# brudfors/UniRes

Hardware: AMD Instinct MI355X
Metric: cg_iters_per_sec (higher is better)
Workload: dtype f32; 1 GPU; cfg3_256c3_thick6z; channels=3, cg_iters_per_channel=20, cg_mode=fixed-iteration (tol=0), identity preconditioner, step=one y-update of one subject: C x (RHS + 20 CG iterations), channel_streams=True, channel_streams_setting=auto, parallelism=one subject per GPU, no data-path collective

## Files before the change

include/unires_hip.h:

```cpp
#ifndef UNIRES_HIP_H
#define UNIRES_HIP_H

#include <stdint.h>

#ifdef __cplusplus
extern "C" {
#endif

#define UNIRES_HIP_ABI_VERSION 1
#define UNIRES_MAX_TAPS 32

enum unires_status {
  UNIRES_OK = 0,
  UNIRES_ERR_NULL = 1,
  UNIRES_ERR_DIM = 2,
  UNIRES_ERR_ARG = 3,
  UNIRES_ERR_HIP = 4,
  UNIRES_ERR_ALLOC = 5,
  UNIRES_ERR_UNSUPPORTED = 6
};

enum unires_operator { UNIRES_OP_A = 0, UNIRES_OP_AT = 1, UNIRES_OP_ATA = 2 };

enum unires_regime {
  UNIRES_REGIME_IDENTITY = 0,
  UNIRES_REGIME_DENOISE = 1,
  UNIRES_REGIME_SUPERRES = 2
};

enum unires_cg_stop {
  UNIRES_STOP_RESIDUAL = 0,
  UNIRES_STOP_MAXGAIN = 1,
  UNIRES_STOP_MAXGAIN_RECURRED = 2,
  UNIRES_STOP_MAXGAIN_GUARDED = 3
};

enum unires_precond {
  UNIRES_PRECOND_IDENTITY = 0,
  UNIRES_PRECOND_JACOBI = 1,
  UNIRES_PRECOND_FFT = 2
};

const char *unires_last_error(void);
int unires_abi_version(void);


int unires_pull3d_affine(const float *src, const int32_t sdim[3], const float M[12], float *dst,
                         const int32_t gdim[3], float fov_tol, void *stream);

int unires_warp_label(const float *label, const int32_t ldim[3], const float M[12], float *dst,
                      const int32_t gdim[3], float fov_tol, void *stream);

int unires_pull3d_nearest(const float *src, const int32_t sdim[3], const float M[12], float *dst,
                          const int32_t gdim[3], float fov_tol, void *stream);

int unires_noise_hist(int32_t n_obs, const float *const *ptrs, const int64_t *sizes, const int32_t *ct,
                      uint32_t *counts, float *range, void *stream);

int unires_noise_fit(int32_t n_obs, const uint32_t *counts, const float *range, int32_t max_iter,
                     double *out, void *stream);

int unires_coreg_quantise(int32_t n_obs, const float *const *ptrs, const int64_t *sizes,
                          uint8_t *const *outs, uint32_t *counts, float *params, void *stream);

typedef struct {
  const uint8_t *G;
  const uint8_t *F;
  int32_t dim_g[3];
  int32_t dim_f[3];
  float M[12];
  float step[3];
} unires_coreg_job_t;

int unires_coreg_hist(int32_t n_jobs, const unires_coreg_job_t *jobs, uint64_t *hist, void *stream);

int unires_coreg_cost(int32_t n, const uint64_t *hist, int32_t cost_fun, double fwhm, double *work,
                      double *cost, void *stream);

int unires_pull_grad3d_affine(const float *src, const int32_t sdim[3], const float M[12],
                              float *dst3, const int32_t gdim[3], float fov_tol, void *stream);

int unires_push3d_affine(const float *src, const int32_t gdim[3], const float M[12], float *dst,
                         const int32_t ddim[3], float alpha, float fov_tol, int accumulate,
                         void *stream);

int unires_conv_down3d(const float *src, const int32_t sdim[3], const float *const taps[3],
                       const int32_t ntaps[3], const int32_t stride[3], float *dst,
                       const int32_t ddim[3], float scl, int32_t scl_dim, void *stream);

int unires_conv_up3d(const float *src, const int32_t sdim[3], const float *const taps[3],
                     const int32_t ntaps[3], const int32_t stride[3], float *dst,
                     const int32_t ddim[3], float scl, int32_t scl_dim, void *stream);

int unires_grad_fwd_zero(const float *src, const int32_t dim[3], const float vx[3], float *dst3,
                         void *stream);

int unires_div_fwd_zero(const float *src3, const int32_t dim[3], const float vx[3], float *dst,
                        void *stream);

int unires_dtd(const float *src, const int32_t dim[3], const float vx[3], float a, float c,
               float *dst, void *stream);

#define UNIRES_DIFF_FORWARD 0
#define UNIRES_DIFF_BACKWARD 1
#define UNIRES_DIFF_CENTRAL 2

int unires_grad_which(const float *src, const int32_t dim[3], const float vx[3], int32_t which,
                      float *dst3, void *stream);
int unires_div_which(const float *src3, const int32_t dim[3], const float vx[3], int32_t which,
                     float *dst, void *stream);
int unires_dtd_which(const float *src, const int32_t dim[3], const float vx[3], int32_t which, float a,
                     float c, float *dst, void *stream);


typedef struct unires_repeat {
  int32_t dim_x[3];
  int32_t dim_g[3];
  float M[12];
  int32_t ratio[3];
  int32_t ntaps[3];
  const float *taps[3];
  float scl;
  int32_t dim_thick;
  float tau;
} unires_repeat_t;

typedef struct unires_plan unires_plan_t;

int unires_plan_create(unires_plan_t **plan, const int32_t dim_y[3], const float vx_y[3],
                       int32_t regime, int32_t n_repeats, const unires_repeat_t *repeats,
                       float fov_tol);
int unires_plan_destroy(unires_plan_t *plan);
int unires_plan_set_repeat(unires_plan_t *plan, int32_t n, const unires_repeat_t *repeat);
int unires_plan_set_concurrency(unires_plan_t *plan, int32_t n_concurrent);
int unires_plan_set_diff(unires_plan_t *plan, int32_t which);
int unires_plan_set_missing(unires_plan_t *plan, int32_t n, const float *x, void *stream);
int unires_plan_set_slice_weights(unires_plan_t *plan, int32_t n, int32_t axis, const float *u_dev, void *stream);
int64_t unires_plan_workspace_bytes(const unires_plan_t *plan);
int unires_plan_repeat_info(const unires_plan_t *plan, int32_t n, int32_t info[8]);
int unires_orient_of(const float M[12], int32_t perm[3], int32_t flip[3]);
int unires_plan_time_matvecs(unires_plan_t *plan, int32_t on);
int unires_plan_matvec_time(unires_plan_t *plan, int32_t *launches, double *total_us);
int unires_plan_cg_ring(unires_plan_t *plan, int32_t k, int32_t *last);
int unires_plan_cg_ends(unires_plan_t *plan, int32_t *trimmed, int32_t *start_fused);

int unires_proj_apply(unires_plan_t *plan, int32_t n, int32_t op, const float *in, float *out,
                      void *stream);

int unires_ata_matvec(unires_plan_t *plan, float rho, float lam, const float *p, float *q,
                      double *dot_dev, void *stream);

int unires_rhs_assemble(unires_plan_t *plan, const float *const *x_ptrs, const float *w_c,
                        const float *z_c, float rho, float lam, float *b, void *stream);

int unires_atx_assemble(unires_plan_t *plan, const float *const *x_ptrs, float *atx,
                        void *stream);

int unires_rhs_from_atx(unires_plan_t *plan, const float *atx, const float *w_c,
                        const float *z_c, float rho, float lam, float *b, void *stream);

int unires_precond_build(unires_plan_t *plan, int32_t precond_mode, float rho, float lam,
                         float *m_out, void *stream);

int unires_precond_apply(unires_plan_t *plan, const float *in, float *out, void *stream);

int unires_cg_solve(unires_plan_t *plan, float rho, float lam, const float *b, float *x,
                    int32_t max_iter, double tol, int32_t stop_mode, int32_t precond_mode,
                    int32_t *iters_out, double *obj_trace, void *stream);

int unires_cg_solve_many(int32_t n, unires_plan_t *const *plans, const float *rho, const float *lam,
                         const float *const *b, float *const *x, int32_t max_iter, double tol,
                         int32_t stop_mode, int32_t precond_mode, int32_t *iters_out,
                         double *obj_trace, void *const *streams);


int unires_zw_update(const float *const *y_ptrs, const float *lam, int32_t n_channels,
                     const int32_t dim[3], const float vx[3], float rho, float alpha, float *z,
                     float *w, float *jtv, void *stream);

int unires_nll_prior(const float *const *y_ptrs, const float *lam, int32_t n_channels,
                     const int32_t dim[3], const float vx[3], double *out_dev, void *stream);

int unires_zw_update_which(const float *const *y_ptrs, const float *lam, int32_t n_channels,
                           const int32_t dim[3], const float vx[3], int32_t which, float rho, float alpha,
                           float *z, float *w, float *jtv, void *stream);
int unires_nll_prior_which(const float *const *y_ptrs, const float *lam, int32_t n_channels,
                           const int32_t dim[3], const float vx[3], int32_t which, double *out_dev,
                           void *stream);

int unires_masked_sse(const float *x, const float *ay, int64_t n, double *out_dev, void *stream);

int unires_slice_sums(const float *x, const float *ay, const int32_t dim[3], int32_t dim_thick, double *out_dev,
                      void *stream);

int unires_rigid_sums(const float *gr3, const float *diff, const float *ctc, const int32_t dim[3],
                      const float d_rigid[72], double *out_dev, void *stream);

int unires_clean_fov(float *y, const int32_t dim_y[3], const float M[12], const int32_t dim_x[3],
                     void *stream);

int unires_scaling_sums(const float *x, const float *ay, const int32_t dim[3], int32_t dim_thick,
                        double *out_dev, void *stream);

typedef struct unires_mark unires_mark_t;
int unires_mark_create(unires_mark_t **out);
int unires_mark_destroy(unires_mark_t *mark);
int unires_mark_signal(unires_mark_t *mark, uint64_t value, void *stream);
int unires_mark_read(const unires_mark_t *mark, uint64_t *value);

#ifdef __cplusplus
}
#endif
#endif
```

unires_amd/_lib.py:

```python
import ctypes as C
import os

_HERE = os.path.dirname(os.path.abspath(__file__))
LIB_PATH = os.environ.get('UNIRES_LIB') or os.path.join(_HERE, 'libunires_hip.so')

UNIRES_MAX_TAPS = 32
OP = {'A': 0, 'At': 1, 'AtA': 2}
REGIME_IDENTITY, REGIME_DENOISE, REGIME_SUPERRES = 0, 1, 2
STOP = {'e': 0, 'max_gain': 3, 'max_gain_guarded': 3, 'max_gain_fresh': 1, 'max_gain_recurred': 2}
PRECOND = {'none': 0, 'identity': 0, 'jacobi': 1, 'fft': 2}

c_i32x3 = C.c_int32 * 3
c_f32x3 = C.c_float * 3
c_f32x12 = C.c_float * 12
c_fptrx3 = C.POINTER(C.c_float) * 3


class Repeat(C.Structure):
    _fields_ = [('dim_x', c_i32x3), ('dim_g', c_i32x3), ('M', c_f32x12), ('ratio', c_i32x3),
                ('ntaps', c_i32x3), ('taps', c_fptrx3), ('scl', C.c_float),
                ('dim_thick', C.c_int32), ('tau', C.c_float)]


SIGNATURES = {
    'unires_last_error': (C.c_char_p, []),
    'unires_abi_version': (C.c_int, []),
    'unires_pull3d_affine': (C.c_int, [C.c_void_p, c_i32x3, c_f32x12, C.c_void_p, c_i32x3,
                                       C.c_float, C.c_void_p]),
    'unires_warp_label': (C.c_int, [C.c_void_p, c_i32x3, c_f32x12, C.c_void_p, c_i32x3,
                                    C.c_float, C.c_void_p]),
    'unires_pull3d_nearest': (C.c_int, [C.c_void_p, c_i32x3, c_f32x12, C.c_void_p, c_i32x3,
                                        C.c_float, C.c_void_p]),
    'unires_noise_hist': (C.c_int, [C.c_int32, C.POINTER(C.c_void_p), C.POINTER(C.c_int64),
                                    C.POINTER(C.c_int32), C.c_void_p, C.c_void_p, C.c_void_p]),
    'unires_noise_fit': (C.c_int, [C.c_int32, C.c_void_p, C.c_void_p, C.c_int32, C.c_void_p,
                                   C.c_void_p]),
    'unires_coreg_quantise': (C.c_int, [C.c_int32, C.POINTER(C.c_void_p), C.POINTER(C.c_int64),
                                        C.POINTER(C.c_void_p), C.c_void_p, C.c_void_p, C.c_void_p]),
    'unires_coreg_hist': (C.c_int, [C.c_int32, C.c_void_p, C.c_void_p, C.c_void_p]),
    'unires_coreg_cost': (C.c_int, [C.c_int32, C.c_void_p, C.c_int32, C.c_double, C.c_void_p,
                                    C.c_void_p, C.c_void_p]),
    'unires_pull_grad3d_affine': (C.c_int, [C.c_void_p, c_i32x3, c_f32x12, C.c_void_p, c_i32x3,
                                            C.c_float, C.c_void_p]),
    'unires_push3d_affine': (C.c_int, [C.c_void_p, c_i32x3, c_f32x12, C.c_void_p, c_i32x3,
                                       C.c_float, C.c_float, C.c_int, C.c_void_p]),
    'unires_conv_down3d': (C.c_int, [C.c_void_p, c_i32x3, c_fptrx3, c_i32x3, c_i32x3, C.c_void_p,
                                     c_i32x3, C.c_float, C.c_int32, C.c_void_p]),
    'unires_conv_up3d': (C.c_int, [C.c_void_p, c_i32x3, c_fptrx3, c_i32x3, c_i32x3, C.c_void_p,
                                   c_i32x3, C.c_float, C.c_int32, C.c_void_p]),
    'unires_grad_fwd_zero': (C.c_int, [C.c_void_p, c_i32x3, c_f32x3, C.c_void_p, C.c_void_p]),
    'unires_div_fwd_zero': (C.c_int, [C.c_void_p, c_i32x3, c_f32x3, C.c_void_p, C.c_void_p]),
    'unires_dtd': (C.c_int, [C.c_void_p, c_i32x3, c_f32x3, C.c_float, C.c_float, C.c_void_p,
                             C.c_void_p]),
    'unires_grad_which': (C.c_int, [C.c_void_p, c_i32x3, c_f32x3, C.c_int32, C.c_void_p, C.c_void_p]),
    'unires_div_which': (C.c_int, [C.c_void_p, c_i32x3, c_f32x3, C.c_int32, C.c_void_p, C.c_void_p]),
    'unires_dtd_which': (C.c_int, [C.c_void_p, c_i32x3, c_f32x3, C.c_int32, C.c_float, C.c_float, C.c_void_p,
                                   C.c_void_p]),
    'unires_plan_create': (C.c_int, [C.POINTER(C.c_void_p), c_i32x3, c_f32x3, C.c_int32,
                                     C.c_int32, C.POINTER(Repeat), C.c_float]),
    'unires_plan_destroy': (C.c_int, [C.c_void_p]),
    'unires_plan_set_repeat': (C.c_int, [C.c_void_p, C.c_int32, C.POINTER(Repeat)]),
    'unires_plan_set_concurrency': (C.c_int, [C.c_void_p, C.c_int32]),
    'unires_plan_set_diff': (C.c_int, [C.c_void_p, C.c_int32]),
    'unires_plan_set_missing': (C.c_int, [C.c_void_p, C.c_int32, C.c_void_p, C.c_void_p]),
    'unires_plan_set_slice_weights': (C.c_int, [C.c_void_p, C.c_int32, C.c_int32, C.c_void_p, C.c_void_p]),
    'unires_plan_workspace_bytes': (C.c_int64, [C.c_void_p]),
    'unires_orient_of': (C.c_int, [c_f32x12, c_i32x3, c_i32x3]),
    'unires_plan_repeat_info': (C.c_int, [C.c_void_p, C.c_int32, C.c_int32 * 8]),
    'unires_plan_time_matvecs': (C.c_int, [C.c_void_p, C.c_int32]),
    'unires_plan_matvec_time': (C.c_int, [C.c_void_p, C.POINTER(C.c_int32), C.POINTER(C.c_double)]),
    'unires_plan_cg_ring': (C.c_int, [C.c_void_p, C.c_int32, C.POINTER(C.c_int32)]),
    'unires_plan_cg_ends': (C.c_int, [C.c_void_p, C.POINTER(C.c_int32), C.POINTER(C.c_int32)]),
    'unires_proj_apply': (C.c_int, [C.c_void_p, C.c_int32, C.c_int32, C.c_void_p, C.c_void_p,
                                    C.c_void_p]),
    'unires_ata_matvec': (C.c_int, [C.c_void_p, C.c_float, C.c_float, C.c_void_p, C.c_void_p,
                                    C.c_void_p, C.c_void_p]),
    'unires_rhs_assemble': (C.c_int, [C.c_void_p, C.POINTER(C.c_void_p), C.c_void_p, C.c_void_p,
                                      C.c_float, C.c_float, C.c_void_p, C.c_void_p]),
    'unires_atx_assemble': (C.c_int, [C.c_void_p, C.POINTER(C.c_void_p), C.c_void_p, C.c_void_p]),
    'unires_rhs_from_atx': (C.c_int, [C.c_void_p, C.c_void_p, C.c_void_p, C.c_void_p, C.c_float,
                                      C.c_float, C.c_void_p, C.c_void_p]),
    'unires_precond_build': (C.c_int, [C.c_void_p, C.c_int32, C.c_float, C.c_float, C.c_void_p,
                                       C.c_void_p]),
    'unires_precond_apply': (C.c_int, [C.c_void_p, C.c_void_p, C.c_void_p, C.c_void_p]),
    'unires_cg_solve': (C.c_int, [C.c_void_p, C.c_float, C.c_float, C.c_void_p, C.c_void_p,
                                  C.c_int32, C.c_double, C.c_int32, C.c_int32,
                                  C.POINTER(C.c_int32), C.POINTER(C.c_double), C.c_void_p]),
    'unires_cg_solve_many': (C.c_int, [C.c_int32, C.POINTER(C.c_void_p), C.POINTER(C.c_float),
                                       C.POINTER(C.c_float), C.POINTER(C.c_void_p), C.POINTER(C.c_void_p),
                                       C.c_int32, C.c_double, C.c_int32, C.c_int32, C.POINTER(C.c_int32),
                                       C.POINTER(C.c_double), C.POINTER(C.c_void_p)]),
    'unires_zw_update': (C.c_int, [C.POINTER(C.c_void_p), C.POINTER(C.c_float), C.c_int32, c_i32x3,
                                   c_f32x3, C.c_float, C.c_float, C.c_void_p, C.c_void_p,
                                   C.c_void_p, C.c_void_p]),
    'unires_nll_prior': (C.c_int, [C.POINTER(C.c_void_p), C.POINTER(C.c_float), C.c_int32, c_i32x3,
                                   c_f32x3, C.c_void_p, C.c_void_p]),
    'unires_zw_update_which': (C.c_int, [C.POINTER(C.c_void_p), C.POINTER(C.c_float), C.c_int32, c_i32x3,
                                         c_f32x3, C.c_int32, C.c_float, C.c_float, C.c_void_p, C.c_void_p,
                                         C.c_void_p, C.c_void_p]),
    'unires_nll_prior_which': (C.c_int, [C.POINTER(C.c_void_p), C.POINTER(C.c_float), C.c_int32, c_i32x3,
                                         c_f32x3, C.c_int32, C.c_void_p, C.c_void_p]),
    'unires_scaling_sums': (C.c_int, [C.c_void_p, C.c_void_p, c_i32x3, C.c_int32, C.c_void_p,
                                      C.c_void_p]),
    'unires_rigid_sums': (C.c_int, [C.c_void_p, C.c_void_p, C.c_void_p, c_i32x3, C.c_float * 72,
                                    C.c_void_p, C.c_void_p]),
    'unires_clean_fov': (C.c_int, [C.c_void_p, c_i32x3, c_f32x12, c_i32x3, C.c_void_p]),
    'unires_masked_sse': (C.c_int, [C.c_void_p, C.c_void_p, C.c_int64, C.c_void_p, C.c_void_p]),
    'unires_slice_sums': (C.c_int, [C.c_void_p, C.c_void_p, c_i32x3, C.c_int32, C.c_void_p, C.c_void_p]),
    'unires_mark_create': (C.c_int, [C.POINTER(C.c_void_p)]),
    'unires_mark_destroy': (C.c_int, [C.c_void_p]),
    'unires_mark_signal': (C.c_int, [C.c_void_p, C.c_uint64, C.c_void_p]),
    'unires_mark_read': (C.c_int, [C.c_void_p, C.POINTER(C.c_uint64)]),
}

DIFF = {'forward': 0, 'backward': 1, 'central': 2}


def diff_code(which, arg='diff'):
    try:
        return DIFF[which]
    except (KeyError, TypeError):
        raise ValueError("%s must be 'forward', 'backward' or 'central', not %r" % (arg, which)) from None


_lib = None

_EXC = {1: ValueError, 2: ValueError, 3: ValueError, 4: RuntimeError, 5: MemoryError,
        6: NotImplementedError}


def load():
    global _lib
    if _lib is not None:
        return _lib
    if not os.path.exists(LIB_PATH):
        raise RuntimeError(
            'unires_amd: %s is missing. Build it with `python -c "import __graft_entry__ as g; '
            'g.build()"` (hipcc --offload-arch=gfx950). There is no CPU fallback.' % LIB_PATH)
    lib = C.CDLL(LIB_PATH)
    for name, (res, args) in SIGNATURES.items():
        fn = getattr(lib, name)
        fn.restype = res
        fn.argtypes = args
    if lib.unires_abi_version() != 1:
        raise RuntimeError('unires_amd: ABI version mismatch')
    _lib = lib
    return lib


def check(status):
    if status != 0:
        msg = load().unires_last_error().decode()
        raise _EXC.get(status, RuntimeError)(msg)


def i3(v):
    return c_i32x3(*[int(t) for t in v])


def f3(v):
    return c_f32x3(*[float(t) for t in v])


def f12(v):
    return c_f32x12(*[float(t) for t in v])
```

unires_amd/_plan.py:

```python
import ctypes as C

import numpy as np
import torch

from . import _lib
from ._lib import (REGIME_DENOISE, REGIME_IDENTITY, REGIME_SUPERRES, Repeat, check, f3, i3)
from ._ops import FOV_TOL, _ptr, _stream, _vol, on_device
from .spatial import _m12, voxel_size


def proj_matrix(po, method):
    if method == 'super-resolution':
        return torch.linalg.solve(po.mat_y, po.rigid.mm(po.mat_yx)), tuple(po.dim_yx)
    if method == 'denoising':
        return torch.linalg.solve(po.mat_y, po.rigid.mm(po.mat_x)), tuple(po.dim_x)
    raise ValueError('Undefined method')


def regime_of(method, do_proj):
    if method not in ('denoising', 'super-resolution'):
        raise ValueError('Undefined method')
    if not do_proj:
        return REGIME_IDENTITY
    return REGIME_SUPERRES if method == 'super-resolution' else REGIME_DENOISE
# ... 81 lines not shown
        check(self.lib.unires_plan_repeat_info(self._h, int(n), info))
        v = list(info)
        return dict(perm=tuple(v[:3]), flip=tuple((v[3] >> j) & 1 for j in range(3)), pull2=bool(v[4]),
                    splat2_axis=None if v[5] == 0 else v[5] - 2, shift=bool(v[6] & 1), separable=bool(v[7]),
                    fused=bool(v[6] & 2), masked=bool(v[6] & 4), weighted=bool(v[6] & 8))

    @on_device
    def time_matvecs(self, on=True):
        check(self.lib.unires_plan_time_matvecs(self._h, 2 if on == 2 else (1 if on else 0)))

    def cg_ring(self, k=0):
        last = C.c_int32(0)
        check(self.lib.unires_plan_cg_ring(self._h, int(k), C.byref(last)))
        return int(last.value)

    @on_device
    def matvec_time(self):
        n, us = C.c_int32(0), C.c_double(0.0)
        check(self.lib.unires_plan_matvec_time(self._h, C.byref(n), C.byref(us)))
        return int(n.value), float(us.value)

    @on_device
    def set_repeat(self, n, po, tau):
        keep = []
        r = _repeat_desc(po, tau, self.method, self.regime, keep)
        check(self.lib.unires_plan_set_repeat(self._h, n, C.byref(r)))

    @on_device
    def set_missing(self, n, dat):
        import weakref
        self._missing[n] = None
        if dat is None:
            check(self.lib.unires_plan_set_missing(self._h, int(n), None, _stream()))
            return
        d = _vol(dat, 'x')[0]
        if tuple(d.shape) != tuple(self.dims_x[n]):
            raise ValueError('unires_amd: observation shape mismatch')
        check(self.lib.unires_plan_set_missing(self._h, int(n), _ptr(d), _stream()))
        self._missing[n] = (weakref.ref(dat), dat._version)

    def sync_missing(self, x_dats):
        for n in range(self.n_repeats):
            if x_dats is None:
                if self._missing[n] is not None:
                    self.set_missing(n, None)
                continue
            t, key = x_dats[n], self._missing[n]
            if key is not None and key[0]() is t and key[1] == t._version:
                continue
            self.set_missing(n, t)

    @on_device
    def set_slice_weights(self, n, axis, w):
        import weakref
        n, axis = int(n), int(axis)
        if not 0 <= n < self.n_repeats:
            raise ValueError('unires_amd: repeat index out of range')
        if axis not in (0, 1, 2):
            raise ValueError('unires_amd: slice axis must be 0, 1 or 2')
        if w is not None and (not w.is_cuda or w.dtype != torch.float32
                              or tuple(w.shape) != (int(self.dims_x[n][axis]),)):
            raise ValueError('unires_amd: slice weights must be a float32 device tensor of shape (%d,)'
                             % int(self.dims_x[n][axis]))
        self._slice_w[n] = None
        self._atx = None
        if w is None:
            check(self.lib.unires_plan_set_slice_weights(self._h, n, axis, None, _stream()))
            return
        wc = w.contiguous()
        check(self.lib.unires_plan_set_slice_weights(self._h, int(n), axis, _ptr(wc), _stream()))
        self._slice_w[n] = (weakref.ref(w), w._version, axis)

    def sync_slice_weights(self, ws):
        for n in range(self.n_repeats):
            want = None if ws is None else ws[n]
            key = self._slice_w[n]
            if want is None:
                if key is not None:
                    self.set_slice_weights(n, key[2], None)
                continue
            axis, t = want
            if key is not None and key[0]() is t and key[1] == t._version and key[2] == int(axis):
                continue
            self.set_slice_weights(n, axis, t)

    def _slice_key(self):
        return tuple(None if k is None else (id(k[0]()), k[1]) for k in self._slice_w)

    def set_concurrency(self, n):
        n = max(1, int(n))
        if n != self._concurrency:
            check(self.lib.unires_plan_set_concurrency(self._h, n))
            self._concurrency = n

    def set_diff(self, diff):
        code = _lib.diff_code(diff, 'diff')
        if diff != self.diff:
            with torch.cuda.device(self.device):
                check(self.lib.unires_plan_set_diff(self._h, code))
            self.diff = diff

    def _y(self, t, name):
        v, _ = _vol(t, name)
        if tuple(v.shape) != self.dim_y:
            raise ValueError('unires_amd: %s has shape %s, expected %s'
                             % (name, tuple(v.shape), self.dim_y))
        return v

    @on_device
    def proj_apply(self, n, operator, dat):
        if operator not in _lib.OP:
            raise ValueError('Undefined operator')
        d, lead = _vol(dat)
        out_dim = self.dims_x[n] if operator == 'A' else self.dim_y
        in_dim = self.dims_x[n] if operator == 'At' else self.dim_y
        if tuple(d.shape) != tuple(in_dim):
            raise ValueError('unires_amd: input has shape %s, expected %s'
                             % (tuple(d.shape), tuple(in_dim)))
        out = torch.empty(out_dim, dtype=torch.float32, device=d.device)
        check(self.lib.unires_proj_apply(self._h, n, _lib.OP[operator], _ptr(d), _ptr(out),
                                         _stream()))
        return out.reshape(lead + tuple(out_dim))

    @on_device
    def matvec(self, p, rho, lam, out=None, dot=None):
        p = self._y(p, 'p')
        if out is None:
            out = torch.empty_like(p)
        check(self.lib.unires_ata_matvec(self._h, float(rho), float(lam), _ptr(p), _ptr(out),
                                         _ptr(dot) if dot is not None else None, _stream()))
        return out

    @on_device
    def rhs(self, x_dats, w_c, z_c, rho, lam, out=None):
        xs = [_vol(t, 'x')[0] for t in x_dats]
        for t, dx in zip(xs, self.dims_x):
            if tuple(t.shape) != tuple(dx):
                raise ValueError('unires_amd: observation shape mismatch')
        if len(xs) != self.n_repeats:
            raise ValueError('unires_amd: need one observation per repeat')
        for t in (w_c, z_c):
            if tuple(t.shape) != (3,) + self.dim_y or not t.is_cuda or t.dtype != torch.float32:
                raise ValueError('unires_amd: w/z must be (3,X,Y,Z) float32 device tensors')
        w_c, z_c = w_c.contiguous(), z_c.contiguous()
        if out is None:
            out = torch.empty(self.dim_y, dtype=torch.float32, device=w_c.device)
        ptrs = (C.c_void_p * len(xs))(*[t.data_ptr() for t in xs])
        check(self.lib.unires_rhs_assemble(self._h, ptrs, _ptr(w_c), _ptr(z_c), float(rho),
                                           float(lam), _ptr(out), _stream()))
        return out

    @on_device
    def rhs_cached(self, x_dats, w_c, z_c, rho, lam, out):
        xs = [_vol(t, 'x')[0] for t in x_dats]
        import weakref
        copied = any(v is not t and v.data_ptr() != t.data_ptr() for v, t in zip(xs, x_dats))
        key = None if copied else (tuple((id(t), t._version) for t in x_dats), self._slice_key())
        cache = getattr(self, '_atx', None)
        alive = cache is not None and all(r() is t for r, t in zip(cache[2], x_dats)) \
            and len(cache[2]) == len(x_dats)
        if cache is None or key is None or not alive or cache[0] != key:
            atx = cache[1] if cache is not None else torch.empty(self.dim_y, dtype=torch.float32,
                                                                 device=xs[0].device)
            ptrs = (C.c_void_p * len(xs))(*[t.data_ptr() for t in xs])
            check(self.lib.unires_atx_assemble(self._h, ptrs, _ptr(atx), _stream()))
            refs = [] if key is None else [weakref.ref(t) for t in x_dats]
            self._atx = cache = (key, atx, refs)
        w_c, z_c = w_c.contiguous(), z_c.contiguous()
        check(self.lib.unires_rhs_from_atx(self._h, _ptr(cache[1]), _ptr(w_c), _ptr(z_c),
                                           float(rho), float(lam), _ptr(out), _stream()))
        return out

    @on_device
    def precond_build(self, rho, lam, mode='jacobi', out=None):
        if mode not in _lib.PRECOND:
            raise ValueError('Undefined preconditioner')
        if out is not None:
            out = self._y(out, 'out')
        check(self.lib.unires_precond_build(self._h, _lib.PRECOND[mode], float(rho), float(lam),
                                            _ptr(out) if out is not None else None, _stream()))
        return out

    @on_device
    def precond_apply(self, v, out=None):
        v = self._y(v, 'v')
        if out is None:
            out = torch.empty_like(v)
        check(self.lib.unires_precond_apply(self._h, _ptr(v), _ptr(out), _stream()))
        return out

    @on_device
    def cg(self, b, x, rho, lam, max_iter=20, tolerance=1e-3, stop='max_gain', sync=True,
           precond='none'):
        if precond not in _lib.PRECOND:
            raise ValueError('Undefined preconditioner')
        pm = _lib.PRECOND[precond]
        b = self._y(b, 'b')
        if not x.is_contiguous():
            raise ValueError('unires_amd: cg updates x in place and needs it contiguous')
        self._y(x, 'x')
        s = stop if stop in _lib.STOP else stop[0].lower()
        mode = _lib.STOP[s] if s in _lib.STOP else (0 if s == 'e' else 3)
        max_iter = int(max_iter)
        if sync:
            it = C.c_int32(0)
            obj = (C.c_double * (min(max_iter, 4096) + 1))()
            check(self.lib.unires_cg_solve(self._h, float(rho), float(lam), _ptr(b), _ptr(x),
                                           int(max_iter), float(tolerance), mode, pm, C.byref(it),
                                           obj, _stream()))
            trace = _trace(list(obj), it.value) if tolerance else None
            return it.value, trace
        check(self.lib.unires_cg_solve(self._h, float(rho), float(lam), _ptr(b), _ptr(x),
                                       int(max_iter), float(tolerance), mode, pm, None, None,
                                       _stream()))
        return None


def _trace(ring, it):
    n = len(ring)
    if it < n:
        return ring[:it + 1]
    start = (it + 1) % n
    return ring[start:] + ring[:start]


def cg_many(plans, bs, xs, rho, lams, streams, max_iter=20, tolerance=1e-3, stop='max_gain', precond='none',
            sync=False):
    if precond not in _lib.PRECOND:
        raise ValueError('Undefined preconditioner')
    n = len(plans)
    lib = plans[0].lib
    s = stop if stop in _lib.STOP else stop[0].lower()
    mode = _lib.STOP[s] if s in _lib.STOP else (0 if s == 'e' else 3)
    for pl, b, x in zip(plans, bs, xs):
        pl._y(b, 'b')
        if not x.is_contiguous():
            raise ValueError('unires_amd: cg updates x in place and needs it contiguous')
        pl._y(x, 'x')
    max_iter = int(max_iter)
    nobj = min(max_iter, 4096) + 1
    it = (C.c_int32 * n)() if sync else None
    obj = (C.c_double * (n * nobj))() if sync else None
    with torch.cuda.device(plans[0].device):
        check(lib.unires_cg_solve_many(
            n, (C.c_void_p * n)(*[pl._h.value for pl in plans]), (C.c_float * n)(*[float(rho)] * n),
            (C.c_float * n)(*[float(v) for v in lams]), (C.c_void_p * n)(*[b.data_ptr() for b in bs]),
            (C.c_void_p * n)(*[x.data_ptr() for x in xs]), max_iter, float(tolerance), mode,
            _lib.PRECOND[precond], it, obj, (C.c_void_p * n)(*[st.cuda_stream for st in streams])))
    if not sync:
        return None
    return [(it[c], _trace(list(obj[c * nobj:(c + 1) * nobj]), it[c]) if tolerance else None) for c in range(n)]
```

unires_amd/_update.py:

```python
import ctypes as C

import torch

from . import _lib
from ._lib import check, f3, i3
from ._ops import _ptr, _stream, on_device
from ._host import Pacer
from ._plan import cg_many
from ._project import _channel_plan, _proj, _slice_axis
from .spatial import voxel_size


_PACERS = {}


def _admm_aux(y, sett):
    dim = (len(y), 3) + tuple(y[0].dim)
    z = torch.zeros(dim, dtype=torch.float32, device=sett.device)
    w = torch.zeros(dim, dtype=torch.float32, device=sett.device)
    return z, w


def _step_size(x, y, sett, verbose=False):
    rho = sett.rho
    if any(xn.ct for xc in x for xn in xc):
        rho = 1.0
    if rho is not None:
        return torch.tensor(rho, dtype=torch.float32)
    all_lam = torch.tensor([float(yc.lam) for yc in y], dtype=torch.float32)
    all_tau = torch.tensor([float(xn.tau) for xc in x for xn in xc], dtype=torch.float32)
    return sett.rho_scl * torch.sqrt(torch.mean(all_tau)) / torch.mean(all_lam)


def _diff(sett):
    diff = getattr(sett, 'diff', 'forward')
    _lib.diff_code(diff, 'sett.diff')
    return diff


def _mask_zeros(sett):
    return bool(getattr(sett, 'mask_zeros', False))


def _slice_robust(sett):
    return bool(getattr(sett, 'slice_robust', False))


class _Precond:

    def __init__(self, plan, M, mode):
        self.plan, self.M, self.mode = plan, M, mode

    def __call__(self, v):
        return v if self.M is None else v / self.M


@on_device
def _precond(x, y, rho, sett):
    if len(x) != 1:
        raise ValueError('CG pre-conditioning only supports one repeat per contrast.')
    plan = _channel_plan(x, y, sett.method, sett.do_proj, voxel_size(y.mat).float(), diff=_diff(sett),
                         mask_zeros=_mask_zeros(sett), weights=True)
    M = torch.empty(tuple(y.dim), dtype=torch.float32, device=y.dat.device)
    plan.precond_build(float(rho), float(y.lam), mode='jacobi', out=M)
    return _Precond(plan, M, 'jacobi')


@on_device
def _update_y(x, y, z, w, rho, tmp, sett, info=None):
    vx_y = voxel_size(y[0].mat).float()
    rho = float(rho)
    sync = info is not None
    C = len(x)
    concurrent = C > 1 and not sync and channel_streams_on(sett, y[0].dat)
    pre = getattr(sett, 'cgs_precond', 'none')
    if not concurrent:
        for c in range(C):
            plan = _channel_plan(x[c], y[c], sett.method, sett.do_proj, vx_y, diff=_diff(sett),
                                 mask_zeros=_mask_zeros(sett), weights=True)
            plan.set_concurrency(1)
            lam = float(y[c].lam)
            if getattr(sett, 'cache_atx', True) and not sync:
                plan.rhs_cached([xn.dat for xn in x[c]], w[c], z[c], rho, lam, out=tmp)
            else:
                plan.rhs([xn.dat for xn in x[c]], w[c], z[c], rho, lam, out=tmp)
            if pre in ('jacobi', 'fft'):
                plan.precond_build(rho, lam, mode=pre)
            res = plan.cg(tmp, y[c].dat, rho, lam, max_iter=sett.cgs_max_iter,
                          tolerance=sett.cgs_tol, stop=sett.cgs_stop, sync=sync, precond=pre)
            if sync:
                info.append(res)
        return y
    main = torch.cuda.current_stream()
    fetched = [_channel_plan(x[c], y[c], sett.method, sett.do_proj, vx_y, diff=_diff(sett),
                             mask_zeros=_mask_zeros(sett), weights=True) for c in range(C)]
    ready = torch.cuda.Event()
    ready.record(main)
    streams = _side_streams(y[0].dat.device, C)
    plans, bs = [], []
    for c in range(C):
        plan = fetched[c]
        plan.set_concurrency(C)
        lam = float(y[c].lam)
        b = tmp if c == 0 else plan.rhs_buffer(tmp)
        with torch.cuda.stream(streams[c]):
            streams[c].wait_event(ready)
            if getattr(sett, 'cache_atx', True):
                plan.rhs_cached([xn.dat for xn in x[c]], w[c], z[c], rho, lam, out=b)
            else:
                plan.rhs([xn.dat for xn in x[c]], w[c], z[c], rho, lam, out=b)
            if pre in ('jacobi', 'fft'):
                plan.precond_build(rho, lam, mode=pre)
        plans.append(plan)
        bs.append(b)
    cg_many(plans, bs, [yc.dat for yc in y], rho, [float(yc.lam) for yc in y], streams,
            max_iter=sett.cgs_max_iter, tolerance=sett.cgs_tol, stop=sett.cgs_stop, precond=pre)
    for c in range(C):
        main.wait_stream(streams[c])
    return y


CHANNEL_STREAMS_MAX_VOXELS = None


def channel_streams_on(sett, dat):
    cs = getattr(sett, 'channel_streams', 'auto')
    if cs == 'auto':
        return CHANNEL_STREAMS_MAX_VOXELS is None or dat.numel() < CHANNEL_STREAMS_MAX_VOXELS
    return bool(cs)


_STREAMS = {}


def _side_streams(device, n):
    key = (device.type, device.index)
    pool = _STREAMS.setdefault(key, [])
    while len(pool) < n:
        pool.append(torch.cuda.Stream(device=device))
    return pool[:n]


def _chan_args(y):
    for yc in y:
        if not yc.dat.is_cuda or yc.dat.dtype != torch.float32 or not yc.dat.is_contiguous():
            raise RuntimeError('unires_amd: y[c].dat must be contiguous float32 CUDA/HIP tensors')
    ptrs = (C.c_void_p * len(y))(*[yc.dat.data_ptr() for yc in y])
    lams = (C.c_float * len(y))(*[float(yc.lam) for yc in y])
    return ptrs, lams


@on_device
def _update_zw(y, z, w, rho, tmp, sett):
    for t in (z, w):
        if not t.is_cuda or t.dtype != torch.float32 or not t.is_contiguous() \
                or tuple(t.shape) != (len(y), 3) + tuple(y[0].dim):
            raise ValueError('unires_amd: z/w must be contiguous (C,3,X,Y,Z) float32 device tensors')
    if not tmp.is_contiguous() or tuple(tmp.shape) != tuple(y[0].dim):
        raise ValueError('unires_amd: tmp must be a contiguous (X,Y,Z) tensor')
    vx = [float(v) for v in voxel_size(y[0].mat).tolist()]
    ptrs, lams = _chan_args(y)
    diff = _lib.diff_code(_diff(sett), 'sett.diff')
    check(_lib.load().unires_zw_update_which(ptrs, lams, len(y), i3(y[0].dim), f3(vx), diff, float(rho),
                                             float(sett.alpha), _ptr(z), _ptr(w), _ptr(tmp), _stream()))
    return z, w, tmp


@on_device
def _slice_sums(x, y, sett):
    lib = _lib.load()
    out = {}
    for c in range(len(x)):
        for n, xn in enumerate(x[c]):
            if getattr(xn, 'slice_w', None) is None:
                continue
            Ay = _proj('A', y[c].dat, x[c], y[c], n=n, method=sett.method, do=sett.do_proj)
            xd = xn.dat.contiguous()
            a = _slice_axis(xn)
            sums = torch.empty(2 * int(xd.shape[a]), dtype=torch.float64, device=xd.device)
            check(lib.unires_slice_sums(_ptr(xd), _ptr(Ay), i3(xd.shape), a, _ptr(sums), _stream()))
            out[(c, n)] = sums
    return out


def slice_rule(sums, k):
    S = sums.numel() // 2
    sse, cnt = sums[:S], sums[S:]
    has = cnt > 0
    m = sse / cnt.clamp(min=1.0)
    K = has.sum()
    inf = torch.full_like(m, float('inf'))
    ranked = torch.where(has, m, inf).sort().values
    sig2 = ranked.gather(0, ((K + 1) // 2 - 1).clamp(min=0).reshape(1))[0]
    thr = (float(k) * float(k)) * sig2
    one = torch.ones_like(m)
    u = torch.where(has & (m > thr), thr / m, one)
    return torch.where((K > 0) & (sig2 > 0), u, one)


@on_device
def _update_slice_weights(x, y, sett, sums=None):
    sums = _slice_sums(x, y, sett) if sums is None else sums
    k = float(getattr(sett, 'slice_k', 3.0))
    for (c, n), s in sums.items():
        x[c][n].slice_w.copy_(slice_rule(s, k))
    return x


@on_device
def _compute_nll(x, y, sett, rho, sum_dtype=torch.float64, slice_sums=None):
    dev = y[0].dat.device
    if slice_sums is None:
        slice_sums = _slice_sums(x, y, sett)
    lib = _lib.load()
    vx = [float(v) for v in voxel_size(y[0].mat).tolist()]
    nll_xy = torch.zeros((), dtype=torch.float64, device=dev)
    sse = torch.zeros((), dtype=torch.float64, device=dev)
    for c in range(len(x)):
        for n in range(len(x[c])):
            if (c, n) in slice_sums:
                w, s = x[c][n].slice_w, slice_sums[(c, n)]
                nll_xy = nll_xy + 0.5 * float(x[c][n].tau) * (w.double() * s[:w.numel()]).sum()
                continue
            Ay = _proj('A', y[c].dat, x[c], y[c], n=n, method=sett.method, do=sett.do_proj)
            xd = x[c][n].dat.contiguous()
            check(lib.unires_masked_sse(_ptr(xd), _ptr(Ay), xd.numel(), _ptr(sse), _stream()))
            nll_xy = nll_xy + 0.5 * float(x[c][n].tau) * sse
    ptrs, lams = _chan_args(y)
    nll_y = torch.zeros((), dtype=torch.float64, device=dev)
    diff = _lib.diff_code(_diff(sett), 'sett.diff')
    check(lib.unires_nll_prior_which(ptrs, lams, len(y), i3(y[0].dim), f3(vx), diff, _ptr(nll_y), _stream()))
    return nll_xy + nll_y, nll_xy, nll_y


@on_device
def _update_scaling(x, y, sett, max_niter_gn=1, num_linesearch=4, verbose=0):
    from ._project import _apply_scaling
    if sett.method != 'super-resolution':
        raise ValueError('_update_scaling needs the super-resolution projection '
                         '(slice profile + slice scaling)')
    lib = _lib.load()
    dev = y[0].dat.device
    sll = torch.zeros((), dtype=torch.float64, device=dev)
    sums = torch.empty(5, dtype=torch.float64, device=dev)
    for c in range(len(x)):
        for n_x in range(len(x[c])):
            xn = x[c][n_x]
            if xn.ct:
                continue
            po = xn.po
            dim_thick, tau, scl = int(po.dim_thick), float(xn.tau), float(po.scl)
            plan = _channel_plan(x[c], y[c], sett.method, sett.do_proj)
            dat_x = xn.dat.contiguous()
            dat_y = plan.proj_apply(n_x, 'A', y[c].dat)

            def evaluate(ay):
                check(lib.unires_scaling_sums(_ptr(dat_x), _ptr(ay), i3(dat_x.shape), dim_thick,
                                              _ptr(sums), _stream()))
                return sums.tolist()

            ll = 0.0
            for _ in range(max_niter_gn):
                s = evaluate(dat_y)
                ll = 0.5 * tau * s[0]
                gr = tau * (s[1] - s[2])
                hes = tau * (s[3] + s[4])
                update = float(torch.tensor(gr, dtype=torch.float64) / torch.tensor(hes, dtype=torch.float64))
                old_scl, old_ll, armijo = scl, ll, 1.0
                if num_linesearch == 0:
# ... 36 lines not shown
```

unires_amd/csrc/api.hip:

```cpp
#include <float.h>
#include <math.h>
#include <string.h>

#include <map>
#include <mutex>
#include <new>

#include "admm.hpp"
#include "api_internal.hpp"
#include "conv.hpp"
#include "coreg.hpp"
#include "noise.hpp"
#include "pull.hpp"
#include "stencil.hpp"

using namespace unires;

thread_local std::string unires::g_err;

int unires::make_taps(const float *const taps[3], const int32_t ntaps[3], const int32_t stride[3], Taps &T) {
  memset(&T, 0, sizeof(T));
  for (int d = 0; d < 3; ++d) {
    if (ntaps[d] < 1 || ntaps[d] > UNIRES_MAX_TAPS)
      return fail(UNIRES_ERR_UNSUPPORTED, "ntaps must be in [1, UNIRES_MAX_TAPS]");
// ... 162 lines not shown
    int32_t ng[3];
    if (coreg_grid(J[o], ng) > (int64_t)INT32_MAX) return fail(UNIRES_ERR_DIM, "more than 2^31 - 1 sample points");
  }
  hipStream_t st = (hipStream_t)stream;
  HIP_TRY(hipMemsetAsync(hist, 0, (size_t)n_jobs * kCoregBins * kCoregBins * sizeof(uint64_t), st));
  for (int32_t o = 0; o < n_jobs; o += kCoregMaxJobs) {
    const int n = std::min<int32_t>(kCoregMaxJobs, n_jobs - o);
    launch_coreg_hist(n, J + o, hist + (size_t)o * kCoregBins * kCoregBins, st);
    CHECK_LAUNCH();
  }
  return UNIRES_OK;
}

extern "C" int unires_coreg_cost(int32_t n, const uint64_t *hist, int32_t cost_fun, double fwhm, double *work,
                                 double *cost, void *stream) {
  if (!hist || !work || !cost) return fail(UNIRES_ERR_NULL, "null argument");
  if (n < 1) return fail(UNIRES_ERR_ARG, "n must be >= 1");
  if (cost_fun < 0 || cost_fun > 2) return fail(UNIRES_ERR_ARG, "cost_fun must be 0 (nmi), 1 (mi) or 2 (ecc)");
  if (!(fwhm >= 0.0 && fwhm <= 16.0)) return fail(UNIRES_ERR_ARG, "fwhm must be in [0, 16]");
  const int R = (int)lround(2.0 * fwhm);
  double taps[2 * kCoregMaxTapRadius + 1];
  const double s = pow(fwhm / sqrt(8.0 * log(2.0)), 2) + DBL_EPSILON, w1 = 1.0 / sqrt(2.0 * s);
  double sum = 0.0;
  for (int k = -R; k <= R; ++k) {
    const double v = 0.5 * (erf(w1 * (k + 0.5)) - erf(w1 * (k - 0.5)));
    taps[k + R] = v > 0.0 ? v : 0.0;
    sum += taps[k + R];
  }
  for (int k = 0; k <= 2 * R; ++k) taps[k] /= sum;
  launch_coreg_cost(n, hist, cost_fun, taps, R, work, cost, (hipStream_t)stream);
  CHECK_LAUNCH();
  return UNIRES_OK;
}

extern "C" int unires_pull_grad3d_affine(const float *src, const int32_t sdim[3], const float M[12],
                                         float *dst3, const int32_t gdim[3], float fov_tol,
                                         void *stream) {
  if (!src || !dst3 || !sdim || !gdim || !M) return fail(UNIRES_ERR_NULL, "null argument");
  if (!dims_ok(sdim) || !dims_ok(gdim)) return fail(UNIRES_ERR_DIM, "bad dimensions");
  Affine A;
  memcpy(A.m, M, sizeof(A.m));
  launch_pull_grad(src, mk(sdim), A, dst3, mk(gdim), fov_tol, (hipStream_t)stream);
  CHECK_LAUNCH();
  return UNIRES_OK;
}

extern "C" int unires_push3d_affine(const float *src, const int32_t gdim[3], const float M[12],
                                    float *dst, const int32_t ddim[3], float alpha, float fov_tol,
                                    int accumulate, void *stream) {
  if (!src || !dst || !ddim || !gdim || !M) return fail(UNIRES_ERR_NULL, "null argument");
  if (!dims_ok(ddim) || !dims_ok(gdim)) return fail(UNIRES_ERR_DIM, "bad dimensions");
  Affine A;
  memcpy(A.m, M, sizeof(A.m));
  Affine Ainv;
  if (!invert_affine(A, Ainv)) return fail(UNIRES_ERR_ARG, "singular affine");
  PushSrc ps;
  memset(&ps, 0, sizeof(ps));
  ps.data = src;
  ps.gd = mk(gdim);
  ps.S = kNoScaling;
  PushEpilogue ep;
  ep.accumulate = accumulate ? 1 : 0;
  SplatSafety safe;
  splat_safety(A, safe.row_sep, safe.use_atomics);
  if (push_mode() == PushMode::kTile ||
      launch_splat(ps, A, Ainv, safe, alpha, fov_tol, ep, dst, mk(ddim), nullptr, (hipStream_t)stream))
    (void)launch_push_tile(ps, A, Ainv, safe, alpha, fov_tol, ep, dst, mk(ddim), nullptr,
                           (hipStream_t)stream);
  CHECK_LAUNCH();
  return UNIRES_OK;
}

extern "C" int unires_conv_down3d(const float *src, const int32_t sdim[3],
                                  const float *const taps[3], const int32_t ntaps[3],
                                  const int32_t stride[3], float *dst, const int32_t ddim[3],
                                  float scl, int32_t scl_dim, void *stream) {
  if (!src || !dst || !sdim || !ddim || !taps || !ntaps || !stride)
    return fail(UNIRES_ERR_NULL, "null argument");
  if (!dims_ok(sdim) || !dims_ok(ddim)) return fail(UNIRES_ERR_DIM, "bad dimensions");
  if (scl != 0.f && (scl_dim < 0 || scl_dim > 2)) return fail(UNIRES_ERR_ARG, "bad scl_dim");
  Taps T;
  int rc = make_taps(taps, ntaps, stride, T);
  if (rc) return rc;
  if ((rc = check_conv_dims(mk(sdim), mk(ddim), T))) return rc;
  launch_conv_down(src, mk(sdim), T, make_scaling(scl, scl_dim), dst, mk(ddim), nullptr,
                   (hipStream_t)stream);
  CHECK_LAUNCH();
  return UNIRES_OK;
}

extern "C" int unires_conv_up3d(const float *src, const int32_t sdim[3],
                                const float *const taps[3], const int32_t ntaps[3],
                                const int32_t stride[3], float *dst, const int32_t ddim[3],
                                float scl, int32_t scl_dim, void *stream) {
  if (!src || !dst || !sdim || !ddim || !taps || !ntaps || !stride)
    return fail(UNIRES_ERR_NULL, "null argument");
  if (!dims_ok(sdim) || !dims_ok(ddim)) return fail(UNIRES_ERR_DIM, "bad dimensions");
  if (scl != 0.f && (scl_dim < 0 || scl_dim > 2)) return fail(UNIRES_ERR_ARG, "bad scl_dim");
  Taps T;
  int rc = make_taps(taps, ntaps, stride, T);
  if (rc) return rc;
  if ((rc = check_conv_dims(mk(ddim), mk(sdim), T))) return rc;
  launch_conv_up(src, mk(sdim), T, make_scaling(scl, scl_dim), dst, mk(ddim), (hipStream_t)stream);
  CHECK_LAUNCH();
  return UNIRES_OK;
}

extern "C" int unires_grad_which(const float *src, const int32_t dim[3], const float vx[3], int32_t which,
                                 float *dst3, void *stream) {
  if (!src || !dst3 || !dim) return fail(UNIRES_ERR_NULL, "null argument");
  if (!dims_ok(dim)) return fail(UNIRES_ERR_DIM, "bad dimensions");
  if (!vx_ok(vx)) return fail(UNIRES_ERR_ARG, "voxel size must be positive");
  if (!diff_ok(which)) return fail(UNIRES_ERR_ARG, "which: forward (0), backward (1) or central (2)");
  launch_grad(src, mk(dim), vx, dst3, (hipStream_t)stream, which);
  CHECK_LAUNCH();
  return UNIRES_OK;
}
extern "C" int unires_grad_fwd_zero(const float *src, const int32_t dim[3], const float vx[3],
                                    float *dst3, void *stream) {
  return unires_grad_which(src, dim, vx, UNIRES_DIFF_FORWARD, dst3, stream);
}

extern "C" int unires_div_which(const float *src3, const int32_t dim[3], const float vx[3], int32_t which,
                                float *dst, void *stream) {
  if (!src3 || !dst || !dim) return fail(UNIRES_ERR_NULL, "null argument");
  if (!dims_ok(dim)) return fail(UNIRES_ERR_DIM, "bad dimensions");
  if (!vx_ok(vx)) return fail(UNIRES_ERR_ARG, "voxel size must be positive");
  if (!diff_ok(which)) return fail(UNIRES_ERR_ARG, "which: forward (0), backward (1) or central (2)");
  launch_div(src3, nullptr, 1.f, 0.f, mk(dim), vx, 1.f, nullptr, dst, (hipStream_t)stream, which);
  CHECK_LAUNCH();
  return UNIRES_OK;
}
extern "C" int unires_div_fwd_zero(const float *src3, const int32_t dim[3], const float vx[3],
                                   float *dst, void *stream) {
  return unires_div_which(src3, dim, vx, UNIRES_DIFF_FORWARD, dst, stream);
}

extern "C" int unires_dtd_which(const float *src, const int32_t dim[3], const float vx[3], int32_t which,
                                float a, float c, float *dst, void *stream) {
  if (!src || !dst || !dim) return fail(UNIRES_ERR_NULL, "null argument");
  if (!dims_ok(dim)) return fail(UNIRES_ERR_DIM, "bad dimensions");
  if (!vx_ok(vx)) return fail(UNIRES_ERR_ARG, "voxel size must be positive");
  if (!diff_ok(which)) return fail(UNIRES_ERR_ARG, "which: forward (0), backward (1) or central (2)");
  if (src == dst) return fail(UNIRES_ERR_ARG, "dtd cannot run in place");
  launch_dtd(src, mk(dim), vx, a, c, dst, nullptr, nullptr, nullptr, (hipStream_t)stream, which);
  CHECK_LAUNCH();
  return UNIRES_OK;
}
extern "C" int unires_dtd(const float *src, const int32_t dim[3], const float vx[3], float a,
                          float c, float *dst, void *stream) {
  return unires_dtd_which(src, dim, vx, UNIRES_DIFF_FORWARD, a, c, dst, stream);
}

static int check_channels(const float *const *y_ptrs, const float *lam, int32_t n) {
  if (!y_ptrs || !lam) return fail(UNIRES_ERR_NULL, "null argument");
  if (n < 1 || n > 4096) return fail(UNIRES_ERR_ARG, "channel count out of range");
  for (int c = 0; c < n; ++c)
    if (!y_ptrs[c]) return fail(UNIRES_ERR_NULL, "null channel pointer");
  return UNIRES_OK;
}

extern "C" int unires_zw_update_which(const float *const *y_ptrs, const float *lam, int32_t n_channels,
                                      const int32_t dim[3], const float vx[3], int32_t which, float rho,
                                      float alpha, float *z, float *w, float *jtv, void *stream) {
  int rc = check_channels(y_ptrs, lam, n_channels);
  if (rc) return rc;
  if (!diff_ok(which)) return fail(UNIRES_ERR_ARG, "which: forward (0), backward (1) or central (2)");
  if (!z || !w || !jtv || !dim) return fail(UNIRES_ERR_NULL, "null argument");
  if (!dims_ok(dim)) return fail(UNIRES_ERR_DIM, "bad dimensions");
  if (!vx_ok(vx)) return fail(UNIRES_ERR_ARG, "voxel size must be positive");
  if (!(rho > 0.f)) return fail(UNIRES_ERR_ARG, "rho must be positive");
  hipStream_t st = (hipStream_t)stream;
  const Dim3i d = mk(dim);
  launch_jtv_scale(y_ptrs, lam, n_channels, w, z, d, vx, rho, alpha, jtv, nullptr, nullptr, 0, st, which);
  const size_t n = d.numel();
  for (int c = 0; c < n_channels; ++c)
    launch_zw_update(y_ptrs[c], lam[c], jtv, z + (size_t)c * 3 * n, w + (size_t)c * 3 * n, d, vx,
                     rho, alpha, st, which);
  CHECK_LAUNCH();
  return UNIRES_OK;
}

extern "C" int unires_zw_update(const float *const *y_ptrs, const float *lam, int32_t n_channels,
                                const int32_t dim[3], const float vx[3], float rho, float alpha,
                                float *z, float *w, float *jtv, void *stream) {
  return unires_zw_update_which(y_ptrs, lam, n_channels, dim, vx, UNIRES_DIFF_FORWARD, rho, alpha, z, w, jtv, stream);
}

extern "C" int unires_nll_prior_which(const float *const *y_ptrs, const float *lam, int32_t n_channels,
                                      const int32_t dim[3], const float vx[3], int32_t which, double *out_dev,
                                      void *stream) {
  int rc = check_channels(y_ptrs, lam, n_channels);
  if (rc) return rc;
  if (!diff_ok(which)) return fail(UNIRES_ERR_ARG, "which: forward (0), backward (1) or central (2)");
  if (!out_dev || !dim) return fail(UNIRES_ERR_NULL, "null argument");
  if (!dims_ok(dim)) return fail(UNIRES_ERR_DIM, "bad dimensions");
  if (!vx_ok(vx)) return fail(UNIRES_ERR_ARG, "voxel size must be positive");
  hipStream_t st = (hipStream_t)stream;
  HIP_TRY(hipMemsetAsync(out_dev, 0, sizeof(double), st));
  float *acc = nullptr;
  if (n_channels > 8) {
    static std::mutex mu;
    static std::map<int, std::pair<float *, size_t>> scratch;
    int dev = 0;
    HIP_TRY(hipGetDevice(&dev));
    const size_t need = mk(dim).numel() * sizeof(float);
    std::lock_guard<std::mutex> lock(mu);
    auto &slot = scratch[dev];
    if (slot.second < need) {
      if (slot.first) {
        HIP_TRY(hipDeviceSynchronize());
        (void)hipFree(slot.first);
        slot = {nullptr, 0};
      }
      HIP_TRY(hipMalloc((void **)&slot.first, need));
      slot.second = need;
    }
    acc = slot.first;
  }
  double *part = nullptr;
  if ((rc = reduce_scratch(st, (size_t)jtv_scale_blocks(mk(dim)), &part))) return rc;
  launch_jtv_scale(y_ptrs, lam, n_channels, nullptr, nullptr, mk(dim), vx, 1.f, 1.f, acc, part, out_dev, 1, st, which);
  CHECK_LAUNCH();
  return UNIRES_OK;
}

extern "C" int unires_nll_prior(const float *const *y_ptrs, const float *lam, int32_t n_channels,
                                const int32_t dim[3], const float vx[3], double *out_dev,
                                void *stream) {
  return unires_nll_prior_which(y_ptrs, lam, n_channels, dim, vx, UNIRES_DIFF_FORWARD, out_dev, stream);
}

extern "C" int unires_scaling_sums(const float *x, const float *ay, const int32_t dim[3],
                                   int32_t dim_thick, double *out_dev, void *stream) {
  if (!x || !ay || !dim || !out_dev) return fail(UNIRES_ERR_NULL, "null argument");
  if (!dims_ok(dim)) return fail(UNIRES_ERR_DIM, "bad dims");
  if (dim_thick < 0 || dim_thick > 2) return fail(UNIRES_ERR_ARG, "bad dim_thick");
  hipStream_t st = (hipStream_t)stream;
  double *part = nullptr;
  if (int rc = reduce_scratch(st, 5 * (size_t)scaling_sums_blocks(mk(dim)), &part)) return rc;
  launch_scaling_sums(x, ay, mk(dim), dim_thick, part, out_dev, st);
  CHECK_LAUNCH();
  return UNIRES_OK;
}

extern "C" int unires_rigid_sums(const float *gr3, const float *diff, const float *ctc,
                                 const int32_t dim[3], const float d_rigid[72], double *out_dev,
                                 void *stream) {
  if (!gr3 || !diff || !dim || !d_rigid || !out_dev) return fail(UNIRES_ERR_NULL, "null argument");
  if (!dims_ok(dim)) return fail(UNIRES_ERR_DIM, "bad dims");
  hipStream_t st = (hipStream_t)stream;
  float D[6][12];
  memcpy(D, d_rigid, sizeof(D));
  double *part = nullptr;
  if (int rc = reduce_scratch(st, 27 * (size_t)rigid_sums_blocks(mk(dim)), &part)) return rc;
  launch_rigid_sums(gr3, diff, ctc, mk(dim), D, part, out_dev, st);
  CHECK_LAUNCH();
  return UNIRES_OK;
}

extern "C" int unires_clean_fov(float *y, const int32_t dim_y[3], const float M[12],
                                const int32_t dim_x[3], void *stream) {
  if (!y || !dim_y || !M || !dim_x) return fail(UNIRES_ERR_NULL, "null argument");
  if (!dims_ok(dim_y) || !dims_ok(dim_x)) return fail(UNIRES_ERR_DIM, "bad dims");
  Affine A;
  memcpy(A.m, M, sizeof(A.m));
  launch_clean_fov(y, mk(dim_y), A, mk(dim_x), (hipStream_t)stream);
  CHECK_LAUNCH();
  return UNIRES_OK;
}

extern "C" int unires_masked_sse(const float *x, const float *ay, int64_t n, double *out_dev,
                                 void *stream) {
  if (!x || !ay || !out_dev) return fail(UNIRES_ERR_NULL, "null argument");
  if (n < 1) return fail(UNIRES_ERR_DIM, "bad length");
  hipStream_t st = (hipStream_t)stream;
  double *part = nullptr;
  if (int rc = reduce_scratch(st, (size_t)masked_sse_blocks((size_t)n), &part)) return rc;
  launch_masked_sse(x, ay, (size_t)n, part, out_dev, st);
  CHECK_LAUNCH();
  return UNIRES_OK;
}

extern "C" int unires_slice_sums(const float *x, const float *ay, const int32_t dim[3], int32_t dim_thick,
                                 double *out_dev, void *stream) {
  if (!x || !ay || !dim || !out_dev) return fail(UNIRES_ERR_NULL, "null argument");
  if (!dims_ok(dim)) return fail(UNIRES_ERR_DIM, "bad dims");
  if (dim_thick < 0 || dim_thick > 2) return fail(UNIRES_ERR_ARG, "bad dim_thick");
  hipStream_t st = (hipStream_t)stream;
  double *part = nullptr;
  const size_t cols = 2 * (size_t)dim[dim_thick];
  if (int rc = reduce_scratch(st, cols * (size_t)slice_sums_parts(mk(dim), dim_thick), &part)) return rc;
  launch_slice_sums(x, ay, mk(dim), dim_thick, part, out_dev, st);
  CHECK_LAUNCH();
  return UNIRES_OK;
}

struct unires_mark {
  unsigned long long *host = nullptr;
  unsigned long long *dev = nullptr;
};

__global__ void k_mark(unsigned long long *w, unsigned long long v) {
  __hip_atomic_store(w, v, __ATOMIC_RELAXED, __HIP_MEMORY_SCOPE_SYSTEM);
}

// ... 41 lines not shown
```

unires_amd/csrc/api_cg.hip:

```cpp
#include <time.h>

#include <functional>

#include "api_internal.hpp"

using namespace unires;

static bool cg_start_fused_on() {
  static const bool on = !(getenv("UNIRES_CG_START_FUSED") && getenv("UNIRES_CG_START_FUSED")[0] == '0');
  return on;
}

static int cg_enqueue_start(unires_plan *pl, const CgSolve &s, unsigned long long *hostw, hipStream_t st) {
  const size_t ny = pl->dy.numel();
  const bool check = s.tol != 0.0;
  CgState *S = pl->state;
  const int gv = vec_num_blocks(ny);
  HIP_TRY(hipMemsetAsync(&S->done, 0, sizeof(int), st));
  const bool want_obj0 = check && s.stop != UNIRES_STOP_RESIDUAL;
  StartResidual res = {s.b, pl->r, pl->p, s.M, pl->part0, want_obj0 ? pl->part1 : nullptr, false};
  const bool ask = cg_start_fused_on() && !s.fft;
  int g0 = matvec(pl, s.rho, s.lam, s.x, pl->ap, nullptr, nullptr, st, nullptr, ask ? &res : nullptr);
  pl->last_fused = ask && res.served;
  if (!(ask && res.served)) {
    launch_residual_init(s.b, pl->ap, s.x, pl->r, pl->p, ny, pl->part0, want_obj0 ? pl->part1 : nullptr, s.M, st);
    g0 = gv;
  }
  if (s.fft) {
    if (fftpre_apply(pl->fft, pl->r, pl->fft.z, st)) return fail(UNIRES_ERR_HIP, "hipFFT execution failed");
    HIP_TRY(hipMemcpyAsync(pl->p, pl->fft.z, ny * sizeof(float), hipMemcpyDeviceToDevice, st));
    launch_dot(pl->r, pl->fft.z, ny, pl->part0, nullptr, st);
  }
  launch_sc_init(S, pl->part0, pl->part1, g0, s.stop, check ? 1 : 0, hostw, st);
  return UNIRES_OK;
}

static float *ring_slot(unires_plan *pl, int j) {
  return j == 0 ? pl->p : pl->ring + (size_t)(j - 1) * (align_up(pl->dy.numel() * 4) / 4);
}

static bool cg_trim_on() {
  static const bool on = !(getenv("UNIRES_CG_TRIM") && getenv("UNIRES_CG_TRIM")[0] == '0');
  return on;
}

static int cg_enqueue_iters(unires_plan *pl, const CgSolve &s, int k_first, int count, bool dev_k,
                            unsigned long long *hostw, hipStream_t st) {
  const size_t ny = pl->dy.numel();
  const bool check = s.tol != 0.0;
  const int ring = s.ring;
  CgState *S = pl->state;
  const int *done = &S->done;
  const int gv = vec_num_blocks(ny);
  if (ring > 1 && (check || s.fft || dev_k || ring > kMaxRing || ring - 1 > pl->ring_slots))
    return fail(UNIRES_ERR_ARG, "deferred iterate update outside its scope");
  const bool trim = cg_trim_on() && !check && !s.fft && !dev_k && k_first == 1 && count == s.max_iter;
  pl->last_trim = trim && count > 0;
  RingPtrs rp = {};
  for (int j = 0; j < ring && ring > 1; ++j) rp.p[j] = ring_slot(pl, j);
  for (int k = k_first; k < k_first + count; ++k) {
    const int kk = dev_k ? -1 : k;
    const int slot = ring > 1 ? (k - k_first) % ring : 0;
    float *p = ring > 1 ? ring_slot(pl, slot) : pl->p;
    hipEvent_t ev0 = nullptr, ev1 = nullptr;
    if (pl->timing && hipEventCreate(&ev0) == hipSuccess) {
      if (hipEventCreate(&ev1) == hipSuccess) {
        (void)hipEventRecord(ev0, st);
      } else {
        (void)hipEventDestroy(ev0);
        ev0 = nullptr;
      }
    }
    if (pl->twice) (void)matvec(pl, s.rho, s.lam, p, pl->ap, pl->part0, done, st);
    const int g = matvec(pl, s.rho, s.lam, p, pl->ap, pl->part0, done, st);
    if (ev0 && ev1) {
      (void)hipEventRecord(ev1, st);
      if (pl->tev.size() >= 65536) {
        (void)hipEventDestroy(pl->tev.front().first), (void)hipEventDestroy(pl->tev.front().second);
        pl->tev.erase(pl->tev.begin());
      }
      pl->tev.emplace_back(ev0, ev1);
    }
    const bool guarded = check && s.stop == UNIRES_STOP_MAXGAIN_GUARDED;
    const bool recur = check && (s.stop == UNIRES_STOP_MAXGAIN_RECURRED || guarded);
    int obj_kind = 0;
    if (check && s.stop == UNIRES_STOP_RESIDUAL) obj_kind = 1;
    if (recur) obj_kind = 2;
    const bool lazy_x = obj_kind == 0;
    if (trim && k == k_first + count - 1) {
      launch_sc_alpha(S, pl->part0, g, st, k);
      if (ring > 1)
        launch_update_x_flush(S, rp, slot + 1, ny, s.x, st);
      else
        launch_update_x(S, p, ny, s.x, st);
      break;
    }
    launch_sc_alpha(S, pl->part0, g, st);
    launch_update_xr(S, p, pl->ap, lazy_x ? nullptr : s.x, pl->r, s.b, ny, pl->part0,
                     recur ? pl->part1 : nullptr, s.M, st);
    if (s.fft) {
      if (fftpre_apply(pl->fft, pl->r, pl->fft.z, st)) return fail(UNIRES_ERR_HIP, "hipFFT execution failed");
      launch_dot(pl->r, pl->fft.z, ny, pl->part0, done, st);
    }
    if (guarded)
      launch_sc_beta_guarded(S, pl->part0, pl->part1, gv, kk, s.tol, hostw, st);
    else
      launch_sc_beta(S, pl->part0, pl->part1, gv, kk, obj_kind, s.tol, obj_kind ? hostw : nullptr, st);
    if (ring > 1 && (slot == ring - 1 || k == k_first + count - 1))
      launch_update_p_flush(S, pl->r, rp, slot + 1, ring_slot(pl, (slot + 1) % ring), ny, s.M, s.x, st);
    else if (ring > 1)
      launch_update_p_ring(S, pl->r, p, ring_slot(pl, slot + 1), slot, ny, s.M, st);
    else
      launch_update_p(S, s.fft ? pl->fft.z : pl->r, pl->p, ny, s.M, lazy_x ? s.x : nullptr, st);
    if (check && s.stop == UNIRES_STOP_MAXGAIN) {
      const int go = matvec(pl, s.rho, s.lam, s.x, pl->ax, pl->part1, done, st, s.b);
      launch_sc_obj(S, pl->part1, go, kk, s.tol, hostw, st);
    }
    if (guarded) {
      const int go = matvec(pl, s.rho, s.lam, s.x, pl->ax, pl->part1, &S->skip_fresh, st, s.b);
      launch_sc_obj_guarded(S, pl->part1, go, kk, s.tol, hostw, st);
    }
  }
  return UNIRES_OK;
}

static int cg_enqueue(unires_plan *pl, const CgSolve &s, hipStream_t st) {
  const int rc = cg_enqueue_start(pl, s, nullptr, st);
  if (rc) return rc;
  return cg_enqueue_iters(pl, s, 1, s.max_iter, false, nullptr, st);
}

static int cg_ring_prepare(unires_plan *pl, hipStream_t st) {
  static const int env_k = [] {
    const char *e = getenv("UNIRES_CG_RING");
    return e ? atoi(e) : 8;
  }();
  int want = pl->ring_req > 0 ? pl->ring_req : env_k;
  want = std::max(1, std::min(want, kMaxRing));
  if (want <= 1) return 1;
  if (!pl->ring_tried) {
    if (stream_capturing(st)) return 1;
    pl->ring_tried = true;
    const size_t slot = align_up(pl->dy.numel() * 4);
    size_t budget = 0;
    if (const char *e = getenv("UNIRES_CG_RING_MB")) {
      budget = (size_t)std::max(0.0, atof(e) * 1048576.0);
    } else {
      size_t free_b = 0, total_b = 0;
      if (hipMemGetInfo(&free_b, &total_b) == hipSuccess) budget = free_b / 8;
      (void)hipGetLastError();
    }
    const int n = (int)std::min<size_t>((size_t)(want - 1), budget / slot);
    if (n < 1) return 1;
    if (hipMalloc((void **)&pl->ring, (size_t)n * slot) != hipSuccess) {
      (void)hipGetLastError();
      pl->ring = nullptr;
      return 1;
    }
    pl->ring_slots = n;
  }
  return std::min(want, pl->ring_slots + 1);
}

struct CgRun {
  unires_plan *pl = nullptr;
  CgSolve s;
  hipStream_t st = nullptr;
  int enqueued = 0;
  unsigned gen = 0;
  bool finished = false;
  bool use_graph = false;
};

static void cg_resync_gen(unires_plan *pl) {
  (void)hipDeviceSynchronize();
  (void)hipGetLastError();
  unsigned g = pl->cg_gen;
  if (pl->state && hipMemcpy(&g, &pl->state->gen, sizeof(g), hipMemcpyDeviceToHost) == hipSuccess) pl->cg_gen = g;
  (void)hipGetLastError();
}

static int cg_chunk_env() {
  static const int v = [] {
    const char *e = getenv("UNIRES_CG_CHUNK");
    return e ? atoi(e) : 2;
  }();
  return v;
}
static int cg_chunk_size() { return std::max(1, std::min(cg_chunk_env(), 64)); }

static int capture_graph(hipStream_t st, hipGraphExec_t *exec, const std::function<int()> &body) {
  *exec = nullptr;
  if (hipStreamBeginCapture(st, hipStreamCaptureModeThreadLocal) != hipSuccess) {
    (void)hipGetLastError();
    return -1;
  }
  const int rc = body();
  hipGraph_t graph = nullptr;
  const hipError_t ce = hipStreamEndCapture(st, &graph);
  if (rc) {
    if (graph) (void)hipGraphDestroy(graph);
    return rc;
  }
  if (ce != hipSuccess || !graph) return fail(UNIRES_ERR_HIP, "hipStreamEndCapture failed");
  const hipError_t ge = hipGraphInstantiate(exec, graph, nullptr, nullptr, 0);
  (void)hipGraphDestroy(graph);
  if (ge != hipSuccess) {
    *exec = nullptr;
    return fail(UNIRES_ERR_HIP, "hipGraphInstantiate failed");
  }
  return UNIRES_OK;
}

static int cg_run_enqueue_chunk(CgRun &R) {
  unires_plan *pl = R.pl;
  const int n = std::min(R.s.chunk, R.s.max_iter - R.enqueued);
  if (n <= 0) return UNIRES_OK;
  if (R.use_graph && n == R.s.chunk && pl->cg_chunk_exec) {
    HIP_TRY(hipGraphLaunch(pl->cg_chunk_exec, R.st));
  } else {
    const int rc = cg_enqueue_iters(pl, R.s, R.enqueued + 1, n, true, pl->progress_dev, R.st);
    if (rc) return rc;
  }
  R.enqueued += n;
  return UNIRES_OK;
}

static int cg_run_start_impl(CgRun &R) {
  unires_plan *pl = R.pl;
  if (!pl->progress) {
    HIP_TRY(hipHostMalloc((void **)&pl->progress, 64, hipHostMallocMapped));
    *pl->progress = 0ull;
    HIP_TRY(hipHostGetDevicePointer((void **)&pl->progress_dev, (void *)pl->progress, 0));
  }
  R.gen = ++pl->cg_gen;
  R.enqueued = 0;
  R.finished = false;
  CgSolve key = R.s;
  key.max_iter = 0;
  key.pre = R.s.M ? UNIRES_PRECOND_JACOBI : UNIRES_PRECOND_IDENTITY;
  if (R.use_graph && !(pl->cg_start_exec && pl->cg_chunk_exec && pl->cg_chunk_key.same_graph(key))) {
    drop_cg_chunk_graphs(pl);
    int rc = capture_graph(R.st, &pl->cg_start_exec, [&] { return cg_enqueue_start(pl, R.s, pl->progress_dev, R.st); });
    if (rc > 0) return rc;
    if (rc == 0)
      rc = capture_graph(R.st, &pl->cg_chunk_exec, [&] {
        return cg_enqueue_iters(pl, R.s, 1, R.s.chunk, true, pl->progress_dev, R.st);
      });
    if (rc > 0) return rc;
    if (rc < 0 || !pl->cg_start_exec || !pl->cg_chunk_exec) {
      drop_cg_chunk_graphs(pl);
      R.use_graph = false;
    } else {
      pl->cg_chunk_key = key;
      pl->chunk_fused = pl->last_fused;
    }
  }
  pl->last_trim = 0;
  if (R.use_graph) {
    pl->last_fused = pl->chunk_fused;
    HIP_TRY(hipGraphLaunch(pl->cg_start_exec, R.st));
  } else {
    const int rc = cg_enqueue_start(pl, R.s, pl->progress_dev, R.st);
    if (rc) return rc;
  }
  int rc = cg_run_enqueue_chunk(R);
  if (!rc) rc = cg_run_enqueue_chunk(R);
  if (rc) return rc;
  if (R.enqueued >= R.s.max_iter) R.finished = true;
  pl->last_trim = 0;
  return UNIRES_OK;
}

static int cg_run_start(CgRun &R) {
  const int rc = cg_run_start_impl(R);
  if (rc) cg_resync_gen(R.pl);
  return rc;
}

static int cg_run_poll(CgRun &R) {
  if (R.finished) return UNIRES_OK;
  const unsigned long long w = __atomic_load_n(R.pl->progress, __ATOMIC_ACQUIRE);
  if ((unsigned)(w >> 32) != R.gen) return UNIRES_OK;
  if (w & 0x80000000ull) {
    R.finished = true;
    return UNIRES_OK;
  }
  const int iters = (int)(w & 0x7fffffffull);
  while (!R.finished && iters >= R.enqueued - R.s.chunk) {
    const int rc = cg_run_enqueue_chunk(R);
    if (rc) return rc;
    if (R.enqueued >= R.s.max_iter) R.finished = true;
  }
  return UNIRES_OK;
}

static int cg_runs_drive(std::vector<CgRun> &runs) {
  unsigned spins = 0;
  for (;;) {
    bool all = true;
    for (CgRun &R : runs) {
      if (R.finished) continue;
      const int rc = cg_run_poll(R);
      if (rc) return rc;
      all = all && R.finished;
    }
    if (all) return UNIRES_OK;
    if (++spins > 256) {
      const struct timespec nap = {0, 50000};
      (void)nanosleep(&nap, nullptr);
    }
    if ((spins <= 256 && (spins & 0xff) == 0) || (spins > 256 && (spins & 0x1ff) == 0)) {
      for (CgRun &R : runs) {
        if (R.finished) continue;
        const hipError_t q = hipStreamQuery(R.st);
        if (q == hipSuccess) {
          const int before = R.enqueued;
          const int rc = cg_run_poll(R);
          if (rc) return rc;
          if (!R.finished && R.enqueued == before)
            return fail(UNIRES_ERR_HIP, "chunked CG: the stream drained without the expected progress");
        } else if (q != hipErrorNotReady) {
          g_err = std::string("chunked CG: ") + hipGetErrorString(q);
          return UNIRES_ERR_HIP;
        }
      }
    }
  }
}

static int cg_check_args(unires_plan *plan, float rho, float lam, const float *b, float *x, int32_t max_iter,
                         double tol, int32_t stop_mode, int32_t precond_mode) {
  if (!plan || !b || !x) return fail(UNIRES_ERR_NULL, "null argument");
  if (b == x) return fail(UNIRES_ERR_ARG, "b and x must not alias");
  if (max_iter < 0) return fail(UNIRES_ERR_ARG, "max_iter out of range");
  if (max_iter > kMaxCgIter && !(tol > 0.0))
    return fail(UNIRES_ERR_ARG, "max_iter beyond 4096 needs a tolerance (the solve is then enqueued in chunks)");
  if (stop_mode < 0 || stop_mode > 3) return fail(UNIRES_ERR_ARG, "bad stop mode");
  if (precond_mode < UNIRES_PRECOND_IDENTITY || precond_mode > UNIRES_PRECOND_FFT)
    return fail(UNIRES_ERR_UNSUPPORTED, "preconditioner modes: identity (0), Jacobi (1), FFT (2)");
  if (precond_mode != UNIRES_PRECOND_IDENTITY &&
      (!plan->prec_ready || plan->prec_mode != precond_mode || plan->prec_rho != rho ||
       plan->prec_lam != lam))
    return fail(UNIRES_ERR_ARG, "call unires_precond_build with this mode, rho and lam first");
  if (!(tol >= 0.0)) return fail(UNIRES_ERR_ARG, "tolerance must be >= 0");
  return UNIRES_OK;
}

static bool cg_graphs_on() {
  static const bool on = !(getenv("UNIRES_CG_GRAPH") && getenv("UNIRES_CG_GRAPH")[0] == '0');
  return on;
}

static bool cg_chunked(double tol, int max_iter) {
  const bool off = cg_chunk_env() == 0;
  return tol != 0.0 && max_iter > 0 && (!off || max_iter > kMaxCgIter);
}

static CgSolve cg_describe(const unires_plan *pl, float rho, float lam, const float *b, float *x, int max_iter,
                           double tol, int stop_mode, int precond_mode) {
  CgSolve s;
  s.b = b, s.x = x, s.rho = rho, s.lam = lam, s.max_iter = max_iter, s.stop = stop_mode, s.pre = precond_mode;
  s.tol = tol;
  s.M = precond_mode == UNIRES_PRECOND_JACOBI ? pl->precM : nullptr;
  s.fft = precond_mode == UNIRES_PRECOND_FFT;
  return s;
}

static CgRun cg_make_run(unires_plan *pl, CgSolve s, hipStream_t st) {
  CgRun R;
  R.pl = pl, R.s = s, R.st = st;
  R.s.chunk = cg_chunk_size();
  R.use_graph = cg_graphs_on() && !s.fft && !pl->timing;
  return R;
}

static int cg_read_back(unires_plan *pl, int max_iter, double tol, int32_t *iters_out, double *obj_trace,
                        hipStream_t st) {
  CgState *S = pl->state;
  int it = 0;
  HIP_TRY(hipMemcpyAsync(&it, &S->iters, sizeof(int), hipMemcpyDeviceToHost, st));
  if (obj_trace && tol != 0.0)
    HIP_TRY(hipMemcpyAsync(obj_trace, S->obj, sizeof(double) * (size_t)(std::min(max_iter, kMaxCgIter) + 1),
                           hipMemcpyDeviceToHost, st));
  HIP_TRY(hipStreamSynchronize(st));
  *iters_out = it;
  return UNIRES_OK;
}

extern "C" int unires_cg_solve(unires_plan_t *plan, float rho, float lam, const float *b, float *x,
                               int32_t max_iter, double tol, int32_t stop_mode,
                               int32_t precond_mode, int32_t *iters_out, double *obj_trace,
                               void *stream) {
  int rc = cg_check_args(plan, rho, lam, b, x, max_iter, tol, stop_mode, precond_mode);
  if (rc) return rc;
  hipStream_t st = (hipStream_t)stream;
  unires_plan *pl = plan;
  CgSolve s = cg_describe(pl, rho, lam, b, x, max_iter, tol, stop_mode, precond_mode);
  mark_use(pl, st);

  if (stream_capturing(st) && tol != 0.0 && max_iter > kMaxCgIter)
    return fail(UNIRES_ERR_ARG, "a solve with a tolerance and more than 4096 iterations cannot join a stream capture "
                                "(it is fed to the device chunk by chunk, following its progress)");
  if (cg_chunked(tol, max_iter) && !(stream_capturing(st) && max_iter <= kMaxCgIter)) {
    pl->last_ring = 1;
    std::vector<CgRun> runs(1, cg_make_run(pl, s, st));
    if ((rc = cg_run_start(runs[0]))) return rc;
    if ((rc = cg_runs_drive(runs))) return rc;
    mark_use(pl, st);
    CHECK_LAUNCH();
    return iters_out ? cg_read_back(pl, max_iter, tol, iters_out, obj_trace, st) : UNIRES_OK;
  }
  ++pl->cg_gen;
  s.ring = tol == 0.0 && !s.fft && max_iter > 0 ? cg_ring_prepare(pl, st) : 1;
  pl->last_ring = s.ring;

  const bool graphable = cg_graphs_on() && !s.fft && max_iter > 0 && !pl->timing;
  if (graphable && pl->cg_exec && pl->cg_key.same_graph(s)) {
    pl->last_trim = pl->graph_trim, pl->last_fused = pl->graph_fused;
    HIP_TRY(hipGraphLaunch(pl->cg_exec, st));
  } else {
    if (graphable && pl->cg_exec) drop_cg_graph(pl);
    rc = graphable ? capture_graph(st, &pl->cg_exec, [&] { return cg_enqueue(pl, s, st); }) : -1;
    if (rc > 0) {
      cg_resync_gen(pl);
      return rc;
    }
    if (rc == 0) {
      pl->cg_key = s;
      pl->graph_trim = pl->last_trim, pl->graph_fused = pl->last_fused;
      if (hipGraphLaunch(pl->cg_exec, st) != hipSuccess) {
        cg_resync_gen(pl);
        return fail(UNIRES_ERR_HIP, "hipGraphLaunch failed");
      }
    } else if ((rc = cg_enqueue(pl, s, st))) {
      cg_resync_gen(pl);
      return rc;
    }
  }
  mark_use(pl, st);
  CHECK_LAUNCH();
  return iters_out ? cg_read_back(pl, max_iter, tol, iters_out, obj_trace, st) : UNIRES_OK;
}

extern "C" int unires_cg_solve_many(int32_t n, unires_plan_t *const *plans, const float *rho, const float *lam,
                                    const float *const *b, float *const *x, int32_t max_iter, double tol,
                                    int32_t stop_mode, int32_t precond_mode, int32_t *iters_out,
                                    double *obj_trace, void *const *streams) {
  if (n < 1 || !plans || !rho || !lam || !b || !x || !streams) return fail(UNIRES_ERR_NULL, "null argument");
  for (int c = 0; c < n; ++c) {
    const int rc = cg_check_args(plans[c], rho[c], lam[c], b[c], x[c], max_iter, tol, stop_mode, precond_mode);
    if (rc) return rc;
    for (int d = 0; d < c; ++d)
      if (plans[d] == plans[c]) return fail(UNIRES_ERR_ARG, "one plan per solve");
  }
  bool capturing = false;
  for (int c = 0; c < n; ++c) capturing = capturing || stream_capturing((hipStream_t)streams[c]);
  if (capturing && tol != 0.0 && max_iter > kMaxCgIter)
    return fail(UNIRES_ERR_ARG, "a solve with a tolerance and more than 4096 iterations cannot join a stream capture "
                                "(it is fed to the device chunk by chunk, following its progress)");
  for (int c = 0; c < n; ++c) mark_use(plans[c], (hipStream_t)streams[c]);
  if (!cg_chunked(tol, max_iter) || (capturing && max_iter <= kMaxCgIter)) {
    for (int c = 0; c < n; ++c) {
      const int rc = unires_cg_solve(plans[c], rho[c], lam[c], b[c], x[c], max_iter, tol, stop_mode, precond_mode,
                                     nullptr, nullptr, streams[c]);
      if (rc) return rc;
    }
  } else {
    std::vector<CgRun> runs;
    for (int c = 0; c < n; ++c) plans[c]->last_ring = 1;
    for (int c = 0; c < n; ++c)
      runs.push_back(cg_make_run(plans[c], cg_describe(plans[c], rho[c], lam[c], b[c], x[c], max_iter, tol, stop_mode,
                                                       precond_mode), (hipStream_t)streams[c]));
    for (CgRun &R : runs) {
      const int rc = cg_run_start(R);
      if (rc) return rc;
    }
    const int rc = cg_runs_drive(runs);
    if (rc) return rc;
    for (int c = 0; c < n; ++c) mark_use(plans[c], (hipStream_t)streams[c]);
    CHECK_LAUNCH();
  }
  if (iters_out)
    for (int c = 0; c < n; ++c) {
      const int rc = cg_read_back(plans[c], max_iter, tol, iters_out + c,
                                  obj_trace ? obj_trace + (size_t)c * (std::min(max_iter, kMaxCgIter) + 1) : nullptr,
                                  (hipStream_t)streams[c]);
      if (rc) return rc;
    }
  return UNIRES_OK;
}
```

unires_amd/csrc/api_internal.hpp:

```cpp
#pragma once
#include <math.h>
#include <stdlib.h>
#include <string.h>

#include <algorithm>
#include <string>
#include <utility>
#include <vector>

#include "../../include/unires_hip.h"
#include "ata1.hpp"
#include "cg.hpp"
#include "fftpre.hpp"
#include "fused.hpp"
#include "mask.hpp"
#include "orient.hpp"
#include "pull2.hpp"
#include "shift.hpp"
#include "slice.hpp"
#include "splat2.hpp"

namespace unires {

extern thread_local std::string g_err;

inline int fail(int code, const char *msg) {
  g_err = msg;
  return code;
}

#define HIP_TRY(expr)                                                               \
  do {                                                                              \
    hipError_t e_ = (expr);                                                         \
    if (e_ != hipSuccess) {                                                         \
      unires::g_err = std::string(#expr) + ": " + hipGetErrorString(e_);            \
      return UNIRES_ERR_HIP;                                                        \
    }                                                                               \
  } while (0)

#define CHECK_LAUNCH()                                                              \
  do {                                                                              \
    hipError_t e_ = hipGetLastError();                                              \
    if (e_ != hipSuccess) {                                                         \
      unires::g_err = std::string("kernel launch: ") + hipGetErrorString(e_);       \
      return UNIRES_ERR_HIP;                                                        \
    }                                                                               \
  } while (0)

inline bool dims_ok(const int32_t d[3]) {
  return d[0] > 0 && d[1] > 0 && d[2] > 0 && d[0] <= 65535 &&
         (long long)d[0] * d[1] * d[2] < (1ll << 40);
}
inline bool vx_ok(const float vx[3]) { return vx && vx[0] > 0 && vx[1] > 0 && vx[2] > 0; }
inline Dim3i mk(const int32_t d[3]) { return Dim3i{d[0], d[1], d[2]}; }
inline size_t align_up(size_t v) { return (v + 255) & ~(size_t)255; }

int make_taps(const float *const taps[3], const int32_t ntaps[3], const int32_t stride[3], Taps &T);
int check_conv_dims(const Dim3i &hi, const Dim3i &lo, const Taps &T);
bool invert_affine(const Affine &A, Affine &out);

inline Scaling make_scaling(float scl, int dim) {
  if (scl == 0.f) return kNoScaling;
  return Scaling{expf(scl), expf(-scl), dim};
}

enum class PushMode { kDefault, kTile, kNoSchedule };
inline PushMode push_mode() {
  static const PushMode mode = [] {
    const char *e = getenv("UNIRES_PUSH");
    return !e ? PushMode::kDefault : !strcmp(e, "tile") ? PushMode::kTile : PushMode::kNoSchedule;
  }();
  return mode;
}

struct RepeatDesc {
  Orient orient;
  bool oriented = false;
  Dim3i dim_xu;
  Dim3i dim_x, dim_g;
  Affine A;
  Taps T;
  float scl;
  int dim_thick;
  float tau;
  Dim3i dim_gf;
  Affine Af, Afinv;
  Taps Tf;
  SplatSafety safe;
  bool sep = false;
  bool sep0 = false;
  bool hyb = false;
  bool hybf = false;
  Taps Tz, Txy;
  Dim3i dim_h;
};

struct RepeatTables {
  SplatSched sched;
  float *ctab_dev[2] = {nullptr, nullptr};
  int ctab_n = 0, ctab_cap = 0;
  unsigned ctab_step = 1, src_stride = 1;
  float *xytab_dev[2] = {nullptr, nullptr};
  int xytab_cap[2] = {0, 0};
  PullPlan pplan;
  ShiftPlan shift;
  F1Sched f1;
};

struct RepeatMask {
  bool masked = false;
  uint8_t *mask_u = nullptr, *mask_c = nullptr;
  size_t mask_cap = 0;
};

struct RepeatWeights {
  bool weighted = false;
  float *w_dev = nullptr;
  int w_axis = 0;
  size_t w_cap = 0;
};

struct Repeat : RepeatDesc, RepeatTables, RepeatMask, RepeatWeights {
  const uint8_t *mask() const { return oriented ? mask_c : mask_u; }
  bool mid() const { return masked || weighted; }
  int w_caxis() const {
    for (int j = 0; j < 3; ++j)
      if (orient.perm[j] == w_axis) return j;
    return w_axis;
  }
  bool w_flip() const { return orient.flip[w_caxis()] != 0; }
};

struct CgSolve {
  const float *b = nullptr;
  float *x = nullptr;
  float rho = 0.f, lam = 0.f;
  int max_iter = -1, stop = -1, pre = -1;
  double tol = -1.0;
  int ring = 1;
  int chunk = 0;
  const float *M = nullptr;
  bool fft = false;
  bool same_graph(const CgSolve &o) const {
    return b == o.b && x == o.x && rho == o.rho && lam == o.lam && max_iter == o.max_iter && stop == o.stop &&
           pre == o.pre && ring == o.ring && chunk == o.chunk && tol == o.tol;
  }
};

}

struct unires_plan {
  unires::Dim3i dy;
  float vx[3];
  int regime;
  float fov_tol;
  int diff = UNIRES_DIFF_FORWARD;
  std::vector<unires::Repeat> reps;
  char *ws = nullptr;
  size_t ws_bytes = 0;
  float *r = nullptr, *p = nullptr, *ap = nullptr, *ax = nullptr;
  bool timing = false;
  bool twice = false;
  std::vector<std::pair<hipEvent_t, hipEvent_t>> tev;
  float *gbuf = nullptr;
  float *gbuf2 = nullptr;
  float *xbuf = nullptr;
  float *xperm = nullptr;
  double *part0 = nullptr, *part1 = nullptr;
  unires::CgState *state = nullptr;
  size_t cap_g = 0, cap_x = 0;
  unires::CgSolve cg_key;
  hipGraphExec_t cg_exec = nullptr;
  unires::CgSolve cg_chunk_key;
  hipGraphExec_t cg_start_exec = nullptr, cg_chunk_exec = nullptr;
  unsigned long long *progress = nullptr, *progress_dev = nullptr;
  unsigned cg_gen = 0;
  float *precM = nullptr;
  float *ring = nullptr;
  int ring_slots = 0;
  bool ring_tried = false;
  int ring_req = 0;
  int last_ring = 1;
  int last_trim = 0, last_fused = 0, graph_trim = 0, graph_fused = 0, chunk_fused = 0;
  unires::FftPre fft;
  float prec_rho = 0.f, prec_lam = 0.f;
  int prec_mode = UNIRES_PRECOND_IDENTITY;
  bool prec_ready = false;
  hipEvent_t last_use = nullptr;
  std::vector<hipStream_t> use_streams;
  bool captured_use = false;
  int concurrency = 1;
  int cap_s2 = 0, cap_f1 = 0;
};

namespace unires {

bool stream_capturing(hipStream_t st);
void mark_use(unires_plan *pl, hipStream_t st);
void await_use(unires_plan *pl);
void drop_cg_chunk_graphs(unires_plan *pl);
void drop_cg_graph(unires_plan *pl);

struct StartResidual {
  const float *b;
  float *r, *p;
  const float *M;
  double *partials;
  double *obj_partials;
  bool served;
};
int matvec(unires_plan *pl, float rho, float lam, const float *p, float *q, double *part, const int *done,
           hipStream_t st, const float *objb = nullptr, StartResidual *res = nullptr);

}
```

unires_amd/csrc/api_operator.hip:

```cpp
#include "aligned.hpp"
#include "api_internal.hpp"
#include "conv.hpp"
#include "pull.hpp"
#include "stencil.hpp"

using namespace unires;

static PushSrc push_src(const Repeat &R, const float *data, bool convup, float scl) {
  PushSrc src;
  src.data = data;
  src.convup = convup ? 1 : 0;
  src.xd = R.dim_x;
  src.gd = convup ? R.dim_gf : R.dim_g;
  src.T = R.Tf;
  src.S = make_scaling(scl, R.dim_thick);
  return src;
}

static Scaling scaling_z(const Scaling &S) { return S.dim == 2 ? S : kNoScaling; }
static Scaling scaling_xy(const Scaling &S) { return S.dim == 2 ? kNoScaling : S; }

static void forward(unires_plan *pl, const Repeat &R, const float *in, const Scaling &S, float *out,
                    const int *done, hipStream_t st) {
  if (pl->regime == UNIRES_REGIME_DENOISE) {
// ... 219 lines not shown
}

int unires::matvec(unires_plan *pl, float rho, float lam, const float *p, float *q, double *part, const int *done,
                   hipStream_t st, const float *objb, StartResidual *res) {
  if (res) res->served = false;
  const float c = rho * (lam * lam);
  float wr[3], wq[3];
  for (int d = 0; d < 3; ++d) {
    const float v2 = pl->vx[d] * pl->vx[d];
    wr[d] = c * (1.f / v2), wq[d] = c / v2;
  }
  if (pl->regime == UNIRES_REGIME_IDENTITY) {
    float a0 = 0.f;
    for (const Repeat &R : pl->reps) a0 += R.tau;
    return stencil_close(pl, c, wr, wq, a0, false, p, q, part, done, st, objb);
  }
  const bool fwd = !diff_nonforward(pl->diff);
  const float zero[3] = {0.f, 0.f, 0.f};
  const float *kw = fwd ? wr : zero;
  double *kpart = fwd ? part : nullptr;
  const float *kobjb = fwd ? objb : nullptr;
  const size_t nrep = pl->reps.size();
  const auto one_kernel = [&]() -> int {
    const Repeat &R = pl->reps[0];
    if (nrep != 1 || no_aligned() || R.mid()) return -1;
    const auto shift = [&] {
      return launch_ata_shift(R.shift, p, q, pl->dy, R.Af, R.tau, 0.f, kw[0], kw[1], kw[2], kpart, kobjb, done, st);
    };
    if (shift_fast(R.shift, pl->dy) && !shift()) return kpart ? shift_blocks(pl->dy) : 0;
    if (!launch_ata_aligned(p, q, pl->dy, R.dim_gf, R.dim_x, R.Tf, make_scaling(2.f * R.scl, R.dim_thick), R.Af, R.tau,
                            0.f, kw[0], kw[1], kw[2], kpart, kobjb, done, st))
      return kpart ? aligned_blocks(pl->dy) : 0;
    if (!shift()) return kpart ? shift_blocks(pl->dy) : 0;
    return -1;
  };
  const bool ask = res && fwd && !part && !objb;
  int npart = one_kernel();
  if (npart < 0) {
    npart = 0;
    for (size_t n = 0; n < nrep; ++n) {
      const Repeat &R = pl->reps[n];
      PushEpilogue ep;
      ep.accumulate = n > 0;
      if (fwd) {
        ep.p = p;
        if (n == 0) ep.cx = wq[0], ep.cy = wq[1], ep.cz = wq[2];
        if (n + 1 == nrep) ep.partials = part, ep.objb = objb;
        if (n + 1 == nrep && ask)
          ep.partials = res->partials, ep.res_obj = res->obj_partials, ep.res_b = res->b, ep.res_r = res->r,
          ep.res_p = res->p, ep.res_M = res->M;
      }
      npart = ata_apply(pl, R, p, R.tau, ep, true, q, done, st, n + 1 == nrep && ask ? &res->served : nullptr);
    }
  }
  return fwd ? npart : stencil_close(pl, c, wr, wq, 0.f, true, p, q, part, done, st, objb);
}

extern "C" int unires_ata_matvec(unires_plan_t *plan, float rho, float lam, const float *p,
                                 float *q, double *dot_dev, void *stream) {
  if (!plan || !p || !q) return fail(UNIRES_ERR_NULL, "null argument");
  if (p == q) return fail(UNIRES_ERR_ARG, "matvec cannot run in place");
  hipStream_t st = (hipStream_t)stream;
  mark_use(plan, st);
  const int g = matvec(plan, rho, lam, p, q, dot_dev ? plan->part0 : nullptr, nullptr, st);
  if (dot_dev) launch_sum_to(plan->part0, g, dot_dev, st);
  CHECK_LAUNCH();
  return UNIRES_OK;
}

extern "C" int unires_precond_build(unires_plan_t *plan, int32_t precond_mode, float rho,
                                    float lam, float *m_out, void *stream) {
  if (!plan) return fail(UNIRES_ERR_NULL, "null plan");
  if (precond_mode == UNIRES_PRECOND_IDENTITY) {
    plan->prec_ready = false;
    return UNIRES_OK;
  }
  if (plan->prec_ready && plan->prec_mode == precond_mode && plan->prec_rho == rho && plan->prec_lam == lam &&
      !m_out)
    return UNIRES_OK;
  if (precond_mode != UNIRES_PRECOND_JACOBI && precond_mode != UNIRES_PRECOND_FFT)
    return fail(UNIRES_ERR_UNSUPPORTED, "preconditioner modes: identity (0), Jacobi (1), FFT (2)");
  hipStream_t st = (hipStream_t)stream;
  mark_use(plan, st);
  const size_t ny = plan->dy.numel();
  if (precond_mode == UNIRES_PRECOND_FFT) {
    if (int rc = fftpre_setup(plan->fft, plan->dy, plan->diff))
      return fail(rc == 2 ? UNIRES_ERR_ALLOC : UNIRES_ERR_HIP, "hipFFT plan / buffer creation failed");
    FftPre &F = plan->fft;
    double a = 0.0;
    if (plan->regime == UNIRES_REGIME_IDENTITY) {
      for (const Repeat &R : plan->reps) a += R.tau;
    } else {
      launch_fill(1.f, plan->ax, ny, st);
      for (size_t n = 0; n < plan->reps.size(); ++n) {
        const Repeat &R = plan->reps[n];
        const PushSrc src = ata_forward(plan, R, plan->ax, nullptr, st);
        PushEpilogue ep;
        ep.accumulate = n > 0;
        push_any(plan, src, R, R.tau, ep, F.z, nullptr, st);
      }
      launch_dot(F.z, plan->ax, ny, plan->part0, nullptr, st);
      launch_sum_to(plan->part0, vec_num_blocks(ny), &plan->state->rz, st);
      HIP_TRY(hipMemcpyAsync(&a, &plan->state->rz, sizeof(double), hipMemcpyDeviceToHost, st));
      HIP_TRY(hipStreamSynchronize(st));
      a /= (double)ny;
    }
    if (!(a > 0.0)) return fail(UNIRES_ERR_ARG, "data term has an empty diagonal");
    F.a = (float)a;
    for (int d = 0; d < 3; ++d) F.c[d] = rho * (lam * lam) / (plan->vx[d] * plan->vx[d]);
    if (m_out) return fail(UNIRES_ERR_ARG, "m_out is only defined for the Jacobi diagonal");
    CHECK_LAUNCH();
    plan->prec_rho = rho, plan->prec_lam = lam, plan->prec_mode = precond_mode, plan->prec_ready = true;
    return UNIRES_OK;
  }
  if (plan->reps.size() != 1)
    return fail(UNIRES_ERR_ARG, "CG pre-conditioning only supports one repeat per contrast.");
  if (!plan->precM) HIP_TRY(hipMalloc((void **)&plan->precM, ny * sizeof(float)));
  const Repeat &R = plan->reps[0];
  float c = 0.f;
  for (int d = 0; d < 3; ++d) c += 1.f / (plan->vx[d] * plan->vx[d]);
  c = 2.f * rho * (lam * lam) * c;
  if (plan->regime == UNIRES_REGIME_IDENTITY) {
    launch_fill(R.tau + c, plan->precM, ny, st);
  } else {
    launch_fill(1.f, plan->ax, ny, st);
    const PushSrc src = ata_forward(plan, R, plan->ax, nullptr, st);
    push_any(plan, src, R, 1.f, PushEpilogue(), plan->precM, nullptr, st);
    launch_scale_shift(R.tau, c, plan->precM, ny, st);
  }
  if (m_out)
    HIP_TRY(hipMemcpyAsync(m_out, plan->precM, ny * sizeof(float), hipMemcpyDeviceToDevice, st));
  CHECK_LAUNCH();
  plan->prec_rho = rho, plan->prec_lam = lam, plan->prec_mode = precond_mode, plan->prec_ready = true;
  return UNIRES_OK;
}

extern "C" int unires_precond_apply(unires_plan_t *plan, const float *in, float *out, void *stream) {
  if (!plan || !in || !out) return fail(UNIRES_ERR_NULL, "null argument");
  if (in == out) return fail(UNIRES_ERR_ARG, "precond_apply cannot run in place");
  hipStream_t st = (hipStream_t)stream;
  mark_use(plan, st);
  const size_t ny = plan->dy.numel();
  if (!plan->prec_ready || plan->prec_mode == UNIRES_PRECOND_IDENTITY) {
    HIP_TRY(hipMemcpyAsync(out, in, ny * sizeof(float), hipMemcpyDeviceToDevice, st));
  } else if (plan->prec_mode == UNIRES_PRECOND_FFT) {
    if (fftpre_apply(plan->fft, in, out, st)) return fail(UNIRES_ERR_HIP, "hipFFT execution failed");
  } else {
    launch_div(in, plan->precM, out, ny, st);
  }
  CHECK_LAUNCH();
  return UNIRES_OK;
}

extern "C" int unires_rhs_assemble(unires_plan_t *plan, const float *const *x_ptrs,
                                   const float *w_c, const float *z_c, float rho, float lam,
                                   float *b, void *stream) {
  if (!plan || !x_ptrs || !w_c || !z_c || !b) return fail(UNIRES_ERR_NULL, "null argument");
  for (size_t n = 0; n < plan->reps.size(); ++n)
    if (!x_ptrs[n]) return fail(UNIRES_ERR_NULL, "null observation pointer");
  hipStream_t st = (hipStream_t)stream;
  mark_use(plan, st);
  launch_div(w_c, z_c, 1.f, -rho, plan->dy, plan->vx, -lam, nullptr, b, st, plan->diff);
  for (size_t n = 0; n < plan->reps.size(); ++n)
    at_accumulate(plan, plan->reps[n], x_ptrs[n], b, plan->reps[n].tau, true, st, true);
  CHECK_LAUNCH();
  return UNIRES_OK;
}

extern "C" int unires_atx_assemble(unires_plan_t *plan, const float *const *x_ptrs, float *atx,
                                   void *stream) {
  if (!plan || !x_ptrs || !atx) return fail(UNIRES_ERR_NULL, "null argument");
  for (size_t n = 0; n < plan->reps.size(); ++n)
    if (!x_ptrs[n]) return fail(UNIRES_ERR_NULL, "null observation pointer");
  hipStream_t st = (hipStream_t)stream;
  mark_use(plan, st);
  if (plan->regime == UNIRES_REGIME_IDENTITY)
    HIP_TRY(hipMemsetAsync(atx, 0, plan->dy.numel() * sizeof(float), st));
  for (size_t n = 0; n < plan->reps.size(); ++n)
    at_accumulate(plan, plan->reps[n], x_ptrs[n], atx, plan->reps[n].tau,
                  n > 0 || plan->regime == UNIRES_REGIME_IDENTITY, st, true);
  CHECK_LAUNCH();
  return UNIRES_OK;
}

extern "C" int unires_rhs_from_atx(unires_plan_t *plan, const float *atx, const float *w_c,
                                   const float *z_c, float rho, float lam, float *b,
                                   void *stream) {
  if (!plan || !atx || !w_c || !z_c || !b) return fail(UNIRES_ERR_NULL, "null argument");
  launch_div(w_c, z_c, 1.f, -rho, plan->dy, plan->vx, -lam, atx, b, (hipStream_t)stream, plan->diff);
  CHECK_LAUNCH();
  return UNIRES_OK;
}
```

unires_amd/csrc/api_plan.hip:

```cpp
#include <stdio.h>
#include <time.h>

#include <new>

#include "api_internal.hpp"

using namespace unires;

static void drop_timing(unires_plan *pl) {
  for (auto &e : pl->tev) (void)hipEventDestroy(e.first), (void)hipEventDestroy(e.second);
  pl->tev.clear();
}

bool unires::stream_capturing(hipStream_t st) {
  hipStreamCaptureStatus cs = hipStreamCaptureStatusNone;
  if (hipStreamIsCapturing(st, &cs) != hipSuccess) {
    (void)hipGetLastError();
    return false;
  }
  return cs != hipStreamCaptureStatusNone;
}

void unires::mark_use(unires_plan *pl, hipStream_t st) {
  if (stream_capturing(st)) {
// ... 298 lines not shown
static void free_tables(RepeatTables &R) {
  splat2_free(R.sched);
  pull2_free(R.pplan);
  shift_free(R.shift);
  ata1_free(R.f1);
  for (int v = 0; v < 2; ++v) {
    if (R.ctab_dev[v]) (void)hipFree(R.ctab_dev[v]), R.ctab_dev[v] = nullptr;
    if (R.xytab_dev[v]) (void)hipFree(R.xytab_dev[v]), R.xytab_dev[v] = nullptr;
    R.xytab_cap[v] = 0;
  }
  R.ctab_n = R.ctab_cap = 0;
}

static void free_mask(RepeatMask &R) {
  if (R.mask_u) (void)hipFree(R.mask_u);
  if (R.mask_c) (void)hipFree(R.mask_c);
  R.mask_u = R.mask_c = nullptr;
  R.mask_cap = 0, R.masked = false;
}

static void free_weights(RepeatWeights &R) {
  if (R.w_dev) (void)hipFree(R.w_dev);
  R.w_dev = nullptr;
  R.w_cap = 0, R.weighted = false;
}

static int canonical_mask(Repeat &R, hipStream_t st) {
  if (!R.masked || !R.oriented) return UNIRES_OK;
  if (!R.mask_c && hipMalloc((void **)&R.mask_c, R.mask_cap) != hipSuccess) {
    R.mask_c = nullptr;
    return fail(UNIRES_ERR_ALLOC, "hipMalloc mask");
  }
  launch_mask_permute(R.mask_u, R.orient, R.dim_xu, R.mask_c, st);
  return UNIRES_OK;
}

extern "C" int unires_plan_create(unires_plan_t **plan, const int32_t dim_y[3],
                                  const float vx_y[3], int32_t regime, int32_t n_repeats,
                                  const unires_repeat_t *repeats, float fov_tol) {
  if (!plan || !dim_y) return fail(UNIRES_ERR_NULL, "null argument");
  *plan = nullptr;
  if (!dims_ok(dim_y)) return fail(UNIRES_ERR_DIM, "bad dim_y");
  if (!vx_ok(vx_y)) return fail(UNIRES_ERR_ARG, "voxel size must be positive");
  if (regime < 0 || regime > 2) return fail(UNIRES_ERR_ARG, "Undefined method");
  if (n_repeats < 1 || !repeats) return fail(UNIRES_ERR_ARG, "need at least one repeat");
  unires_plan *pl = new (std::nothrow) unires_plan();
  if (!pl) return fail(UNIRES_ERR_ALLOC, "host allocation failed");
  pl->dy = mk(dim_y);
  memcpy(pl->vx, vx_y, sizeof(pl->vx));
  pl->regime = regime;
  pl->fov_tol = fov_tol;
  pl->reps.resize(n_repeats);
  bool need_sep = false;
  for (int n = 0; n < n_repeats; ++n) {
    if (int rc = fill_repeat(pl, &repeats[n], pl->reps[n])) {
      unires_plan_destroy(pl);
      return rc;
    }
    if (regime != UNIRES_REGIME_IDENTITY) {
      pl->cap_g = std::max(pl->cap_g, pl->reps[n].dim_g.numel());
      pl->cap_x = std::max(pl->cap_x, pl->reps[n].dim_x.numel());
    }
    need_sep = need_sep || (regime == UNIRES_REGIME_SUPERRES && (pl->reps[n].sep || pl->reps[n].hyb));
  }
  const size_t ny = pl->dy.numel();
  size_t off = 0;
  auto carve = [&](size_t bytes) {
    size_t o = off;
    off += align_up(bytes);
    return o;
  };
  const size_t o_r = carve(ny * 4), o_p = carve(ny * 4), o_ap = carve(ny * 4), o_ax = carve(ny * 4);
  const size_t o_g = carve(pl->cap_g * 4), o_x = carve(pl->cap_x * 4), o_xp = carve(pl->cap_x * 4);
  const size_t o_g2 = carve(need_sep ? pl->cap_g * 4 : 0);
  const size_t o_p0 = carve(kMaxPartials * 8), o_p1 = carve(kMaxPartials * 8);
  const size_t o_st = carve(sizeof(CgState));
  pl->ws_bytes = off;
  hipError_t e = hipMalloc((void **)&pl->ws, pl->ws_bytes);
  if (e != hipSuccess) {
    g_err = std::string("hipMalloc workspace: ") + hipGetErrorString(e);
    pl->ws = nullptr;
    unires_plan_destroy(pl);
    return UNIRES_ERR_ALLOC;
  }
  pl->r = (float *)(pl->ws + o_r);
  pl->p = (float *)(pl->ws + o_p);
  pl->ap = (float *)(pl->ws + o_ap);
  pl->ax = (float *)(pl->ws + o_ax);
  pl->gbuf = (float *)(pl->ws + o_g);
  pl->xbuf = (float *)(pl->ws + o_x);
  pl->xperm = (float *)(pl->ws + o_xp);
  pl->gbuf2 = need_sep ? (float *)(pl->ws + o_g2) : nullptr;
  pl->part0 = (double *)(pl->ws + o_p0);
  pl->part1 = (double *)(pl->ws + o_p1);
  pl->state = (CgState *)(pl->ws + o_st);
  e = hipMemset(pl->state, 0, sizeof(CgState));
  if (e != hipSuccess) {
    g_err = std::string("hipMemset: ") + hipGetErrorString(e);
    unires_plan_destroy(pl);
    return UNIRES_ERR_HIP;
  }
  for (Repeat &R : pl->reps)
    if (int rc = build_repeat_kernels(pl, R)) {
      unires_plan_destroy(pl);
      return rc;
    }
  *plan = pl;
  return UNIRES_OK;
}

extern "C" int unires_plan_destroy(unires_plan_t *plan) {
  if (!plan) return UNIRES_OK;
  if (plan->ws) (void)hipFree(plan->ws);
  if (plan->precM) (void)hipFree(plan->precM);
  if (plan->ring) (void)hipFree(plan->ring);
  if (plan->cg_exec) (void)hipGraphExecDestroy(plan->cg_exec);
  if (plan->cg_start_exec) (void)hipGraphExecDestroy(plan->cg_start_exec);
  if (plan->cg_chunk_exec) (void)hipGraphExecDestroy(plan->cg_chunk_exec);
  if (plan->progress) (void)hipHostFree(plan->progress);
  if (plan->last_use) (void)hipEventDestroy(plan->last_use);
  drop_timing(plan);
  fftpre_destroy(plan->fft);
  for (Repeat &R : plan->reps) free_tables(R), free_mask(R), free_weights(R);
  delete plan;
  return UNIRES_OK;
}

extern "C" int unires_plan_time_matvecs(unires_plan_t *plan, int32_t on) {
  if (!plan) return fail(UNIRES_ERR_NULL, "null argument");
  const bool twice = on == 2;
  if (twice != plan->twice) drop_cg_graph(plan);
  plan->twice = twice;
  plan->timing = on == 1;
  if (!plan->timing) drop_timing(plan);
  return UNIRES_OK;
}

extern "C" int unires_plan_cg_ring(unires_plan_t *plan, int32_t k, int32_t *last) {
  if (!plan) return fail(UNIRES_ERR_NULL, "null argument");
  if (k < 0) return fail(UNIRES_ERR_ARG, "ring size must be >= 0");
  if (k > 0) {
    const int v = std::min<int>(k, kMaxRing);
    if (v != plan->ring_req) drop_cg_graph(plan);
    plan->ring_req = v;
  }
  if (last) *last = plan->last_ring;
  return UNIRES_OK;
}

extern "C" int unires_plan_cg_ends(unires_plan_t *plan, int32_t *trimmed, int32_t *start_fused) {
  if (!plan) return fail(UNIRES_ERR_NULL, "null argument");
  if (trimmed) *trimmed = plan->last_trim;
  if (start_fused) *start_fused = plan->last_fused;
  return UNIRES_OK;
}

extern "C" int unires_plan_matvec_time(unires_plan_t *plan, int32_t *launches, double *total_us) {
  if (!plan || !launches || !total_us) return fail(UNIRES_ERR_NULL, "null argument");
  *launches = 0, *total_us = 0.0;
  for (auto &e : plan->tev) {
    float ms = 0.f;
    HIP_TRY(hipEventSynchronize(e.second));
    HIP_TRY(hipEventElapsedTime(&ms, e.first, e.second));
    *total_us += 1e3 * (double)ms;
    ++*launches;
  }
  drop_timing(plan);
  return UNIRES_OK;
}

static bool same_but_scaling(const RepeatDesc &a, const RepeatDesc &b) {
  auto taps_equal = [](const Taps &p, const Taps &q) {
    for (int d = 0; d < 3; ++d) {
      if (p.n[d] != q.n[d] || p.s[d] != q.s[d]) return false;
      for (int t = 0; t < p.n[d]; ++t)
        if (p.t[d][t] != q.t[d][t]) return false;
    }
    return true;
  };
  return !memcmp(&a.A, &b.A, sizeof(Affine)) && taps_equal(a.T, b.T) && !memcmp(&a.Af, &b.Af, sizeof(Affine)) &&
         taps_equal(a.Tf, b.Tf) && !memcmp(&a.dim_x, &b.dim_x, sizeof(Dim3i)) &&
         !memcmp(&a.dim_g, &b.dim_g, sizeof(Dim3i)) && !memcmp(&a.dim_gf, &b.dim_gf, sizeof(Dim3i)) &&
         !memcmp(&a.dim_xu, &b.dim_xu, sizeof(Dim3i)) && !memcmp(&a.orient, &b.orient, sizeof(Orient)) &&
         a.oriented == b.oriented && a.dim_thick == b.dim_thick && (a.scl != 0.f) == (b.scl != 0.f) &&
         a.sep0 == b.sep0;
}

extern "C" int unires_plan_set_repeat(unires_plan_t *plan, int32_t n,
                                      const unires_repeat_t *repeat) {
  if (!plan || !repeat) return fail(UNIRES_ERR_NULL, "null argument");
  if (n < 0 || n >= (int)plan->reps.size()) return fail(UNIRES_ERR_ARG, "repeat index");
  RepeatDesc tmp;
  int rc = fill_repeat(plan, repeat, tmp, plan->reps[n].mid());
  if (rc) return rc;
  if (plan->reps[n].masked && memcmp(&tmp.dim_xu, &plan->reps[n].dim_xu, sizeof(Dim3i)))
    return fail(UNIRES_ERR_DIM, "a masked repeat keeps its observation's dims (clear the mask first)");
  if (plan->reps[n].weighted && memcmp(&tmp.dim_xu, &plan->reps[n].dim_xu, sizeof(Dim3i)))
    return fail(UNIRES_ERR_DIM, "a weighted repeat keeps its observation's dims (clear the weights first)");
  if (plan->regime != UNIRES_REGIME_IDENTITY &&
      (tmp.dim_g.numel() > plan->cap_g || tmp.dim_x.numel() > plan->cap_x))
    return fail(UNIRES_ERR_DIM, "new repeat exceeds the plan's workspace");
  if (plan->regime == UNIRES_REGIME_SUPERRES && (tmp.sep || tmp.hyb) && !plan->gbuf2)
    return fail(UNIRES_ERR_DIM, "new repeat needs the separable-conv scratch the plan was built without");
  await_use(plan);
  drop_cg_graph(plan);
  plan->prec_ready = false;
  Repeat &R = plan->reps[n];
  static const bool no_fast = getenv("UNIRES_SET_REPEAT_FULL") != nullptr;
  const bool same = !no_fast && same_but_scaling(tmp, R);
  static const bool verbose = getenv("UNIRES_SET_REPEAT_VERBOSE") != nullptr;
  if (verbose) fprintf(stderr, "[set_repeat] %s (scl %g -> %g)\n", same ? "scaling only" : "full rebuild", (double)R.scl, (double)tmp.scl);
  if (same) {
    R.scl = tmp.scl, R.tau = tmp.tau;
    rc = build_sched(plan, R, true);
    if (!rc) build_shift(plan, R);
    return rc;
  }
  static_cast<RepeatDesc &>(R) = tmp;
  R.ctab_n = 0;
  sched_set_thorough(false);
  rc = build_repeat_kernels(plan, R);
  sched_set_thorough(true);
  if (!rc && R.masked && R.oriented) {
    rc = canonical_mask(R, nullptr);
    if (!rc) HIP_TRY(hipStreamSynchronize(nullptr));
  }
  return rc;
}

static int refamily(unires_plan *pl, Repeat &R) {
  const bool hyb = R.hyb, hybf = R.hybf, sep = R.sep;
  choose_family(pl, R, R.mid());
  if (hyb == R.hyb && hybf == R.hybf && sep == R.sep) return UNIRES_OK;
  R.ctab_n = 0;
  return build_repeat_kernels(pl, R);
}

extern "C" int unires_plan_set_missing(unires_plan_t *plan, int32_t n, const float *x, void *stream) {
  if (!plan) return fail(UNIRES_ERR_NULL, "null plan");
  if (n < 0 || n >= (int)plan->reps.size()) return fail(UNIRES_ERR_ARG, "repeat index");
  if (plan->regime == UNIRES_REGIME_IDENTITY)
    return fail(UNIRES_ERR_UNSUPPORTED,
                "regime A = I has no x-space intermediate to mask: build the plan in the denoising regime with the "
                "identity affine");
  Repeat &R = plan->reps[n];
  if (!x && !R.masked) return UNIRES_OK;
  hipStream_t st = (hipStream_t)stream;
  await_use(plan);
  drop_cg_graph(plan);
  plan->prec_ready = false;
  const bool was = R.masked, was_mid = R.mid();
  if (x) {
    const size_t nx = R.dim_xu.numel();
    if (R.mask_cap < nx) {
      free_mask(R);
      if (was_mid != R.mid()) (void)refamily(plan, R);
      if (hipMalloc((void **)&R.mask_u, nx) != hipSuccess) {
        R.mask_u = nullptr;
        return fail(UNIRES_ERR_ALLOC, "hipMalloc mask");
      }
      R.mask_cap = nx;
    }
    if (R.oriented && !R.mask_c && hipMalloc((void **)&R.mask_c, R.mask_cap) != hipSuccess) {
      R.mask_c = nullptr;
      return fail(UNIRES_ERR_ALLOC, "hipMalloc mask");
    }
    mark_use(plan, st);
    launch_mask_build(x, Orient(), R.dim_xu, R.mask_u, st);
    R.masked = true;
    (void)canonical_mask(R, st);
  } else {
    R.masked = false;
  }
  if (was_mid != R.mid()) {
    if (int rc = refamily(plan, R)) {
      R.masked = was;
      (void)refamily(plan, R);
      return rc;
    }
  }
  CHECK_LAUNCH();
  return UNIRES_OK;
}

extern "C" int unires_plan_set_slice_weights(unires_plan_t *plan, int32_t n, int32_t axis, const float *u_dev,
                                             void *stream) {
  if (!plan) return fail(UNIRES_ERR_NULL, "null plan");
  if (n < 0 || n >= (int)plan->reps.size()) return fail(UNIRES_ERR_ARG, "repeat index");
  if (axis < 0 || axis > 2) return fail(UNIRES_ERR_ARG, "slice axis: 0, 1 or 2");
  if (plan->regime == UNIRES_REGIME_IDENTITY)
    return fail(UNIRES_ERR_UNSUPPORTED,
                "regime A = I has no x-space intermediate to weight: build the plan in the denoising regime with the "
                "identity affine");
  Repeat &R = plan->reps[n];
  if (!u_dev && !R.weighted) return UNIRES_OK;
  hipStream_t st = (hipStream_t)stream;
  const bool was = R.weighted, was_mid = R.mid();
  const int was_axis = R.w_axis;
  const bool values_only = u_dev && was && axis == R.w_axis;
  plan->prec_ready = false;
  if (!values_only) {
    await_use(plan);
    drop_cg_graph(plan);
  }
  if (u_dev) {
    const int du[3] = {R.dim_xu.x, R.dim_xu.y, R.dim_xu.z};
// ... 86 lines not shown
```

unires_amd/csrc/cg.hip:

```cpp
#include "cg.hpp"

namespace unires {

static inline int vec_blocks(size_t n) {
  size_t b = (n / 4 + kBlock - 1) / kBlock;
  if (b < 1) b = 1;
  const size_t cap = 4096;
  return (int)(b < cap ? b : cap);
}

#define GRID_STRIDE_VEC4(n)                                                   \
  const size_t n4 = (n) / 4;                                                  \
  const size_t stride = (size_t)gridDim.x * blockDim.x;                       \
  const size_t tid0 = (size_t)blockIdx.x * blockDim.x + threadIdx.x

__device__ __forceinline__ float4 ld4(const float *p, size_t i) {
  return reinterpret_cast<const float4 *>(p)[i];
}
__device__ __forceinline__ void st4(float *p, size_t i, float4 v) {
  reinterpret_cast<float4 *>(p)[i] = v;
}
typedef float f4v __attribute__((ext_vector_type(4)));
__device__ __forceinline__ float4 ld4_stream(const float *p, size_t i) {
#ifdef UNIRES_CG_X_PLAIN
  return ld4(p, i);
#else
  const f4v v = __builtin_nontemporal_load(reinterpret_cast<const f4v *>(p) + i);
  return make_float4(v.x, v.y, v.z, v.w);
#endif
}
__device__ __forceinline__ void st4_stream(float *p, size_t i, float4 v) {
#ifdef UNIRES_CG_X_PLAIN
  st4(p, i, v);
#else
  __builtin_nontemporal_store(f4v{v.x, v.y, v.z, v.w}, reinterpret_cast<f4v *>(p) + i);
#endif
}


__device__ __forceinline__ float4 zval4(float4 r, const float *__restrict__ M, size_t i) {
  if (!M) return r;
  const float4 m = ld4(M, i);
  return make_float4(__fdiv_rn(r.x, m.x), __fdiv_rn(r.y, m.y), __fdiv_rn(r.z, m.z),
                     __fdiv_rn(r.w, m.w));
}
__device__ __forceinline__ float zval1(float r, const float *__restrict__ M, size_t i) {
  return M ? __fdiv_rn(r, M[i]) : r;
}

__global__ void __launch_bounds__(kBlock)
    k_residual_init(const float *__restrict__ b, const float *__restrict__ ax,
                    const float *__restrict__ x, float *__restrict__ r, float *__restrict__ p,
                    size_t n, double *__restrict__ part_rr, double *__restrict__ part_obj,
                    const float *__restrict__ M) {
  GRID_STRIDE_VEC4(n);
  double rr = 0.0, ob = 0.0;
  for (size_t i = tid0; i < n4; i += stride) {
    const float4 vb = ld4(b, i), va = ld4(ax, i);
    float4 vr;
    vr.x = __fsub_rn(vb.x, va.x);
    vr.y = __fsub_rn(vb.y, va.y);
    vr.z = __fsub_rn(vb.z, va.z);
    vr.w = __fsub_rn(vb.w, va.w);
    st4(r, i, vr);
    const float4 vz = zval4(vr, M, i);
    st4(p, i, vz);
    rr += (double)__fmul_rn(vr.x, vz.x) + (double)__fmul_rn(vr.y, vz.y) +
          (double)__fmul_rn(vr.z, vz.z) + (double)__fmul_rn(vr.w, vz.w);
    if (part_obj) {
      const float4 vx = ld4(x, i);
      ob += (double)obj_term(va.x, vb.x, vx.x) + (double)obj_term(va.y, vb.y, vx.y) +
            (double)obj_term(va.z, vb.z, vx.z) + (double)obj_term(va.w, vb.w, vx.w);
    }
  }
  for (size_t i = n4 * 4 + tid0; i < n; i += stride) {
    const float vr = __fsub_rn(b[i], ax[i]);
    r[i] = vr;
    const float vz = zval1(vr, M, i);
    p[i] = vz;
    rr += (double)__fmul_rn(vr, vz);
    if (part_obj) ob += (double)obj_term(ax[i], b[i], x[i]);
  }
  const double t = block_sum(rr);
  if (threadIdx.x == 0) part_rr[blockIdx.x] = t;
  if (part_obj) {
    const double t2 = block_sum(ob);
    if (threadIdx.x == 0) part_obj[blockIdx.x] = t2;
  }
}

__global__ void __launch_bounds__(kBlock)
    k_dot(const float *__restrict__ a, const float *__restrict__ b, size_t n,
          double *__restrict__ part, const int *__restrict__ done) {
  if (done && *done) return;
  GRID_STRIDE_VEC4(n);
  double acc = 0.0;
  for (size_t i = tid0; i < n4; i += stride) {
    const float4 va = ld4(a, i), vb = ld4(b, i);
    acc += (double)__fmul_rn(va.x, vb.x) + (double)__fmul_rn(va.y, vb.y) +
           (double)__fmul_rn(va.z, vb.z) + (double)__fmul_rn(va.w, vb.w);
  }
  for (size_t i = n4 * 4 + tid0; i < n; i += stride) acc += (double)__fmul_rn(a[i], b[i]);
  const double t = block_sum(acc);
  if (threadIdx.x == 0) part[blockIdx.x] = t;
}

template <bool XUPD>
__global__ void __launch_bounds__(kBlock)
    k_update_xr(const CgState *__restrict__ st, const float *__restrict__ p,
                const float *__restrict__ ap, float *__restrict__ x, float *__restrict__ r,
                const float *__restrict__ b, size_t n, double *__restrict__ part_rr,
                double *__restrict__ part_obj, const float *__restrict__ M) {
  if (st->done) return;
  const float alpha = (float)st->alpha;
  GRID_STRIDE_VEC4(n);
  double rr = 0.0, ob = 0.0;
  for (size_t i = tid0; i < n4; i += stride) {
    const float4 va = ld4(ap, i);
    float4 vx = make_float4(0.f, 0.f, 0.f, 0.f), vr = ld4(r, i);
    if (XUPD) {
      const float4 vp = ld4(p, i);
      vx = ld4(x, i);
      vx.x = __fadd_rn(vx.x, __fmul_rn(alpha, vp.x));
      vx.y = __fadd_rn(vx.y, __fmul_rn(alpha, vp.y));
      vx.z = __fadd_rn(vx.z, __fmul_rn(alpha, vp.z));
      vx.w = __fadd_rn(vx.w, __fmul_rn(alpha, vp.w));
      st4(x, i, vx);
    }
    vr.x = __fsub_rn(vr.x, __fmul_rn(alpha, va.x));
    vr.y = __fsub_rn(vr.y, __fmul_rn(alpha, va.y));
    vr.z = __fsub_rn(vr.z, __fmul_rn(alpha, va.z));
    vr.w = __fsub_rn(vr.w, __fmul_rn(alpha, va.w));
    st4(r, i, vr);
    const float4 vz = zval4(vr, M, i);
    rr += (double)__fmul_rn(vr.x, vz.x) + (double)__fmul_rn(vr.y, vz.y) +
          (double)__fmul_rn(vr.z, vz.z) + (double)__fmul_rn(vr.w, vz.w);
    if (XUPD && part_obj) {
      const float4 vb = ld4(b, i);
      ob += (double)__fmul_rn(vx.x, __fadd_rn(vb.x, vr.x)) +
            (double)__fmul_rn(vx.y, __fadd_rn(vb.y, vr.y)) +
            (double)__fmul_rn(vx.z, __fadd_rn(vb.z, vr.z)) +
            (double)__fmul_rn(vx.w, __fadd_rn(vb.w, vr.w));
    }
  }
  for (size_t i = n4 * 4 + tid0; i < n; i += stride) {
    float vx = 0.f;
    if (XUPD) {
      vx = __fadd_rn(x[i], __fmul_rn(alpha, p[i]));
      x[i] = vx;
    }
    const float vr = __fsub_rn(r[i], __fmul_rn(alpha, ap[i]));
    r[i] = vr;
    rr += (double)__fmul_rn(vr, zval1(vr, M, i));
    if (XUPD && part_obj) ob += (double)__fmul_rn(vx, __fadd_rn(b[i], vr));
  }
  const double t = block_sum(rr);
  if (threadIdx.x == 0) part_rr[blockIdx.x] = t;
  if (XUPD && part_obj) {
    const double t2 = block_sum(ob);
    if (threadIdx.x == 0) part_obj[blockIdx.x] = t2;
  }
}

template <bool XUPD>
__global__ void __launch_bounds__(kBlock)
    k_update_p(const CgState *__restrict__ st, const float *__restrict__ r, float *__restrict__ p,
               size_t n, const float *__restrict__ M, float *__restrict__ x) {
  if (st->done) return;
  const float beta = (float)st->beta, alpha = (float)st->alpha;
  GRID_STRIDE_VEC4(n);
  for (size_t i = tid0; i < n4; i += stride) {
    const float4 vr = zval4(ld4(r, i), M, i);
    float4 vp = ld4(p, i);
    if (XUPD) {
      float4 vx = ld4_stream(x, i);
      vx.x = __fadd_rn(vx.x, __fmul_rn(alpha, vp.x));
      vx.y = __fadd_rn(vx.y, __fmul_rn(alpha, vp.y));
      vx.z = __fadd_rn(vx.z, __fmul_rn(alpha, vp.z));
      vx.w = __fadd_rn(vx.w, __fmul_rn(alpha, vp.w));
      st4_stream(x, i, vx);
    }
    vp.x = __fadd_rn(__fmul_rn(beta, vp.x), vr.x);
    vp.y = __fadd_rn(__fmul_rn(beta, vp.y), vr.y);
    vp.z = __fadd_rn(__fmul_rn(beta, vp.z), vr.z);
    vp.w = __fadd_rn(__fmul_rn(beta, vp.w), vr.w);
    st4(p, i, vp);
  }
  for (size_t i = n4 * 4 + tid0; i < n; i += stride) {
    const float vp = p[i];
    if (XUPD) x[i] = __fadd_rn(x[i], __fmul_rn(alpha, vp));
    p[i] = __fadd_rn(__fmul_rn(beta, vp), zval1(r[i], M, i));
  }
}


__global__ void __launch_bounds__(kBlock)
    k_update_p_ring(CgState *__restrict__ st, const float *__restrict__ r, const float *__restrict__ p_in,
                    float *__restrict__ p_out, int slot, size_t n, const float *__restrict__ M) {
  const int done = st->done;
  if (blockIdx.x == 0 && threadIdx.x == 0) st->ahist[slot] = st->alpha, st->committed[slot] = done ? 0 : 1;
  if (done) return;
  const float beta = (float)st->beta;
  GRID_STRIDE_VEC4(n);
  for (size_t i = tid0; i < n4; i += stride) {
    const float4 vz = zval4(ld4(r, i), M, i);
    float4 vp = ld4_stream(p_in, i);
    vp.x = __fadd_rn(__fmul_rn(beta, vp.x), vz.x);
    vp.y = __fadd_rn(__fmul_rn(beta, vp.y), vz.y);
    vp.z = __fadd_rn(__fmul_rn(beta, vp.z), vz.z);
    vp.w = __fadd_rn(__fmul_rn(beta, vp.w), vz.w);
    st4(p_out, i, vp);
  }
  for (size_t i = n4 * 4 + tid0; i < n; i += stride)
    p_out[i] = __fadd_rn(__fmul_rn(beta, p_in[i]), zval1(r[i], M, i));
}

template <bool PUPD>
__global__ void __launch_bounds__(kBlock)
    k_update_p_flush(CgState *__restrict__ st, const float *__restrict__ r, RingPtrs ring, int m, float *p_out,
                     size_t n, const float *__restrict__ M, float *__restrict__ x) {
  const int done = st->done;
  const float beta = PUPD ? (float)st->beta : 0.f;
  float a[kMaxRing];
  bool c[kMaxRing];
  bool any = false;
#pragma unroll
  for (int j = 0; j < kMaxRing; ++j) {
    c[j] = false, a[j] = 0.f;
    if (j < m - 1) c[j] = st->committed[j] != 0, a[j] = (float)st->ahist[j];
    if (j == m - 1) c[j] = !done, a[j] = (float)st->alpha;
    any = any || c[j];
  }
  if (!any) return;
  GRID_STRIDE_VEC4(n);
  for (size_t i = tid0; i < n4; i += stride) {
    float4 vz = make_float4(0.f, 0.f, 0.f, 0.f);
    if (PUPD && !done) vz = zval4(ld4(r, i), M, i);
    float4 vx = ld4_stream(x, i);
    float4 vp[kMaxRing];
#pragma unroll
    for (int j = 0; j < kMaxRing; ++j)
      if (c[j]) vp[j] = ld4_stream(ring.p[j], i);
#pragma unroll
    for (int j = 0; j < kMaxRing; ++j) {
      if (!c[j]) continue;
      vx.x = __fadd_rn(vx.x, __fmul_rn(a[j], vp[j].x));
      vx.y = __fadd_rn(vx.y, __fmul_rn(a[j], vp[j].y));
      vx.z = __fadd_rn(vx.z, __fmul_rn(a[j], vp[j].z));
      vx.w = __fadd_rn(vx.w, __fmul_rn(a[j], vp[j].w));
      if (PUPD && j == m - 1) {
        float4 b = vp[j];
        b.x = __fadd_rn(__fmul_rn(beta, b.x), vz.x);
        b.y = __fadd_rn(__fmul_rn(beta, b.y), vz.y);
        b.z = __fadd_rn(__fmul_rn(beta, b.z), vz.z);
        b.w = __fadd_rn(__fmul_rn(beta, b.w), vz.w);
        st4(p_out, i, b);
      }
    }
    st4_stream(x, i, vx);
  }
  for (size_t i = n4 * 4 + tid0; i < n; i += stride) {
    float vx = x[i], own = 0.f;
#pragma unroll
    for (int j = 0; j < kMaxRing; ++j) {
      if (!c[j]) continue;
      const float pj = ring.p[j][i];
      vx = __fadd_rn(vx, __fmul_rn(a[j], pj));
      if (j == m - 1) own = pj;
    }
    x[i] = vx;
    if (PUPD && !done) p_out[i] = __fadd_rn(__fmul_rn(beta, own), zval1(r[i], M, i));
  }
}

__global__ void __launch_bounds__(kBlock)
    k_update_x(const CgState *__restrict__ st, const float *__restrict__ p, size_t n, float *__restrict__ x) {
  if (st->done) return;
  const float alpha = (float)st->alpha;
  GRID_STRIDE_VEC4(n);
  for (size_t i = tid0; i < n4; i += stride) {
    const float4 vp = ld4_stream(p, i);
    float4 vx = ld4_stream(x, i);
    vx.x = __fadd_rn(vx.x, __fmul_rn(alpha, vp.x));
    vx.y = __fadd_rn(vx.y, __fmul_rn(alpha, vp.y));
    vx.z = __fadd_rn(vx.z, __fmul_rn(alpha, vp.z));
    vx.w = __fadd_rn(vx.w, __fmul_rn(alpha, vp.w));
    st4_stream(x, i, vx);
  }
  for (size_t i = n4 * 4 + tid0; i < n; i += stride) x[i] = __fadd_rn(x[i], __fmul_rn(alpha, p[i]));
}

__global__ void __launch_bounds__(kBlock)
    k_axpy(float a, const float *__restrict__ x, float *__restrict__ y, size_t n) {
  const size_t stride = (size_t)gridDim.x * blockDim.x;
  for (size_t i = (size_t)blockIdx.x * blockDim.x + threadIdx.x; i < n; i += stride)
    y[i] = fmaf(a, x[i], y[i]);
}

__device__ __forceinline__ double sum_partials(const double *part, int g) {
  double v = 0.0;
  int i = threadIdx.x;
  for (; i + 7 * kBlock < g; i += 8 * kBlock) {
    double t[8];
#pragma unroll
    for (int u = 0; u < 8; ++u) t[u] = part[i + u * kBlock];
// ... 44 lines not shown
  const double gain = (prev - obj) / (st->obj_max - st->obj_min);
  if (fabs(gain) < tol) st->done = 1;
  if (!isfinite(obj)) st->done = 1;
}

__global__ void __launch_bounds__(kBlock)
    k_sc_init(CgState *st, const double *part_rr, const double *part_obj, int g, int mode,
              int check, unsigned long long *hostw) {
  const double rr = sum_partials(part_rr, g);
  double ob = 0.0;
  if (check && mode != UNIRES_STOP_RESIDUAL) ob = sum_partials(part_obj, g);
  if (threadIdx.x == 0) {
    st->rz = rr;
    st->rzpp[0] = rr;
    st->rzpp[1] = rr;
    st->done = 0;
    st->iters = 0;
    st->alpha = 0.0;
    st->beta = 0.0;
    st->gen += 1u;
    if (check) record_obj(st, 0, mode == UNIRES_STOP_RESIDUAL ? sqrt(rr) : 0.5 * ob, 0.0);
    st->skip_fresh = 1, st->fresh_prev_ok = 1, st->rec_prev = 0.5 * ob, st->fresh_prev = 0.5 * ob, st->gain_rec = 0.0;
    publish(st, hostw);
  }
}

__global__ void __launch_bounds__(kBlock) k_sc_alpha(CgState *st, const double *part_pap, int g, int iters_end) {
  PartLoad L;
  part_issue(part_pap, g, L);
  const int done = st->done;
  const double rz = st->rz;
  const double pap = part_finish(part_pap, g, L);
  if (threadIdx.x == 0 && !done) {
    st->pAp = pap;
    st->alpha = rz / pap;
    if (iters_end > 0) st->iters = iters_end;
  }
}

__global__ void __launch_bounds__(kBlock)
    k_sc_beta(CgState *st, const double *part_rr, const double *part_obj, int g, int k,
              int obj_kind, double tol, unsigned long long *hostw) {
  PartLoad Lr, Lo;
  part_issue(part_rr, g, Lr);
  if (obj_kind == 2) part_issue(part_obj, g, Lo);
  const int done = st->done, iters = st->iters;
  const double rz0 = st->rz;
  if (k < 0) k = iters + 1;
  const double rr = part_finish(part_rr, g, Lr);
  double ob = 0.0;
  if (obj_kind == 2) ob = part_finish(part_obj, g, Lo);
  if (threadIdx.x == 0 && !done) {
    st->rz = rr;
    st->rzpp[k & 1] = rr;
    st->beta = rr / rz0;
    st->iters = k;
    if (obj_kind == 1) record_obj(st, k, sqrt(rr), tol);
    if (obj_kind == 2) record_obj(st, k, -0.5 * ob, tol);
    publish(st, hostw);
  }
}

__global__ void __launch_bounds__(kBlock)
    k_sc_obj(CgState *st, const double *part_obj, int g, int k, double tol, unsigned long long *hostw) {
  PartLoad L;
  part_issue(part_obj, g, L);
  const int done = st->done, iters = st->iters;
  if (k < 0) k = iters;
  const double ob = part_finish(part_obj, g, L);
  if (threadIdx.x == 0 && !done) {
    record_obj(st, k, 0.5 * ob, tol);
    publish(st, hostw);
  }
}

constexpr double kGuardHi = 4.0, kGuardLo = 0.5, kGuardNear = 1.5;
__global__ void __launch_bounds__(kBlock)
    k_sc_beta_guarded(CgState *st, const double *part_rr, const double *part_obj, int g, int k, double tol,
                      unsigned long long *hostw) {
  PartLoad Lr, Lo;
  part_issue(part_rr, g, Lr);
  part_issue(part_obj, g, Lo);
  const int done = st->done, iters = st->iters;
  const double rz0 = st->rz;
  if (k < 0) k = iters + 1;
  const double rr = part_finish(part_rr, g, Lr);
  const double ob = part_finish(part_obj, g, Lo);
  if (threadIdx.x == 0 && !done) {
    constexpr int kRing = kMaxCgIter + 1;
    st->rz = rr;
    st->rzpp[k & 1] = rr;
    st->beta = rr / rz0;
    st->iters = k;
    const double rec = -0.5 * ob;
    st->obj[k % kRing] = rec;
    st->obj_max = fmax(st->obj_max, rec);
    st->obj_min = fmin(st->obj_min, rec);
    const double gain = (st->rec_prev - rec) / (st->obj_max - st->obj_min);
    const double gain_before = fabs(st->gain_rec);
    st->gain_rec = gain;
    st->rec_prev = rec;
    double hi = kGuardHi;
    if (gain_before > 0.0 && isfinite(gain_before) && isfinite(gain)) {
      const double rho = fabs(gain) / gain_before;
      hi = fmin(kGuardHi, fmax(kGuardNear, kGuardNear / fmax(rho, 1e-6)));
    }
    const bool far = fabs(gain) >= hi * tol;
    const bool under = fabs(gain) < kGuardLo * tol;
    st->skip_fresh = (far || under) ? 1 : 0;
    if (far) st->fresh_prev_ok = 0;
    if (under) st->done = 1;
    if (!isfinite(rec)) st->done = 1, st->skip_fresh = 1;
    publish(st, hostw);
  }
}

__global__ void __launch_bounds__(kBlock)
    k_sc_obj_guarded(CgState *st, const double *part_obj, int g, int k, double tol, unsigned long long *hostw) {
  PartLoad L;
  part_issue(part_obj, g, L);
  const int done = st->done, skip = st->skip_fresh, iters = st->iters;
  if (k < 0) k = iters;
  const double ob = part_finish(part_obj, g, L);
  if (threadIdx.x == 0 && !done && !skip) {
    constexpr int kRing = kMaxCgIter + 1;
    const double fresh = 0.5 * ob;
    st->obj[k % kRing] = fresh;
    st->obj_max = fmax(st->obj_max, fresh);
    st->obj_min = fmin(st->obj_min, fresh);
    const double gain = st->fresh_prev_ok ? (st->fresh_prev - fresh) / (st->obj_max - st->obj_min) : st->gain_rec;
    st->fresh_prev = fresh, st->fresh_prev_ok = 1;
    if (fabs(gain) < tol || !isfinite(fresh)) st->done = 1, st->skip_fresh = 1;
    publish(st, hostw);
  }
}

__global__ void __launch_bounds__(kBlock) k_sum_to(const double *part, int g, double *out) {
  const double v = sum_partials(part, g);
  if (threadIdx.x == 0) *out = v;
}

int vec_num_blocks(size_t n) { return vec_blocks(n); }

void launch_residual_init(const float *b, const float *ax, const float *x, float *r, float *p,
                          size_t n, double *part_rr, double *part_obj, const float *M,
                          hipStream_t st) {
  hipLaunchKernelGGL(k_residual_init, dim3(vec_blocks(n)), dim3(kBlock), 0, st, b, ax, x, r, p, n,
                     part_rr, part_obj, M);
}
void launch_dot(const float *a, const float *b, size_t n, double *part, const int *done,
                hipStream_t st) {
  hipLaunchKernelGGL(k_dot, dim3(vec_blocks(n)), dim3(kBlock), 0, st, a, b, n, part, done);
}
void launch_update_xr(const CgState *s, const float *p, const float *ap, float *x, float *r,
                      const float *b, size_t n, double *part_rr, double *part_obj,
                      const float *M, hipStream_t st) {
  if (x)
    hipLaunchKernelGGL(k_update_xr<true>, dim3(vec_blocks(n)), dim3(kBlock), 0, st, s, p, ap, x, r, b,
                       n, part_rr, part_obj, M);
  else
    hipLaunchKernelGGL(k_update_xr<false>, dim3(vec_blocks(n)), dim3(kBlock), 0, st, s, p, ap, x, r,
                       b, n, part_rr, part_obj, M);
}
void launch_update_p(const CgState *s, const float *r, float *p, size_t n, const float *M, float *x,
                     hipStream_t st) {
  if (x)
    hipLaunchKernelGGL(k_update_p<true>, dim3(vec_blocks(n)), dim3(kBlock), 0, st, s, r, p, n, M, x);
  else
    hipLaunchKernelGGL(k_update_p<false>, dim3(vec_blocks(n)), dim3(kBlock), 0, st, s, r, p, n, M, x);
}
void launch_update_p_ring(CgState *s, const float *r, const float *p_in, float *p_out, int slot, size_t n,
                          const float *M, hipStream_t st) {
  hipLaunchKernelGGL(k_update_p_ring, dim3(vec_blocks(n)), dim3(kBlock), 0, st, s, r, p_in, p_out, slot, n, M);
}
void launch_update_p_flush(CgState *s, const float *r, const RingPtrs &ring, int m, float *p_out, size_t n,
                           const float *M, float *x, hipStream_t st) {
  hipLaunchKernelGGL(k_update_p_flush<true>, dim3(vec_blocks(n)), dim3(kBlock), 0, st, s, r, ring, m, p_out, n, M, x);
}
void launch_update_x_flush(CgState *s, const RingPtrs &ring, int m, size_t n, float *x, hipStream_t st) {
  hipLaunchKernelGGL(k_update_p_flush<false>, dim3(vec_blocks(n)), dim3(kBlock), 0, st, s, (const float *)nullptr, ring, m,
                     (float *)nullptr, n, (const float *)nullptr, x);
}
void launch_update_x(const CgState *s, const float *p, size_t n, float *x, hipStream_t st) {
  hipLaunchKernelGGL(k_update_x, dim3(vec_blocks(n)), dim3(kBlock), 0, st, s, p, n, x);
}
__global__ void __launch_bounds__(kBlock) k_scale_shift(float a, float c, float *__restrict__ y, size_t n) {
  const size_t stride = (size_t)gridDim.x * blockDim.x;
  for (size_t i = (size_t)blockIdx.x * blockDim.x + threadIdx.x; i < n; i += stride)
    y[i] = __fadd_rn(__fmul_rn(a, y[i]), c);
}
void launch_scale_shift(float a, float c, float *y, size_t n, hipStream_t st) {
  hipLaunchKernelGGL(k_scale_shift, dim3(vec_blocks(n) * 4 > 4096 ? 4096 : vec_blocks(n) * 4),
                     dim3(kBlock), 0, st, a, c, y, n);
}
__global__ void __launch_bounds__(kBlock) k_fill(float v, float *__restrict__ y, size_t n) {
  const size_t stride = (size_t)gridDim.x * blockDim.x;
  for (size_t i = (size_t)blockIdx.x * blockDim.x + threadIdx.x; i < n; i += stride) y[i] = v;
}
void launch_fill(float v, float *y, size_t n, hipStream_t st) {
  hipLaunchKernelGGL(k_fill, dim3(vec_blocks(n) * 4 > 4096 ? 4096 : vec_blocks(n) * 4), dim3(kBlock), 0,
                     st, v, y, n);
}
__global__ void __launch_bounds__(kBlock)
    k_divide(const float *__restrict__ a, const float *__restrict__ m, float *__restrict__ y, size_t n) {
  const size_t stride = (size_t)gridDim.x * blockDim.x;
  for (size_t i = (size_t)blockIdx.x * blockDim.x + threadIdx.x; i < n; i += stride)
    y[i] = __fdiv_rn(a[i], m[i]);
}
void launch_div(const float *a, const float *m, float *y, size_t n, hipStream_t st) {
  hipLaunchKernelGGL(k_divide, dim3(vec_blocks(n) * 4 > 4096 ? 4096 : vec_blocks(n) * 4), dim3(kBlock), 0,
                     st, a, m, y, n);
}
void launch_axpy(float a, const float *x, float *y, size_t n, hipStream_t st) {
  hipLaunchKernelGGL(k_axpy, dim3(vec_blocks(n) * 4 > 4096 ? 4096 : vec_blocks(n) * 4),
                     dim3(kBlock), 0, st, a, x, y, n);
}
void launch_sc_init(CgState *s, const double *part_rr, const double *part_obj, int g, int mode,
                    int check, unsigned long long *hostw, hipStream_t st) {
  hipLaunchKernelGGL(k_sc_init, dim3(1), dim3(kBlock), 0, st, s, part_rr, part_obj, g, mode,
                     check, hostw);
}
void launch_sc_alpha(CgState *s, const double *part, int g, hipStream_t st, int iters_end) {
  hipLaunchKernelGGL(k_sc_alpha, dim3(1), dim3(kBlock), 0, st, s, part, g, iters_end);
}
void launch_sc_beta(CgState *s, const double *part_rr, const double *part_obj, int g, int k,
                    int obj_kind, double tol, unsigned long long *hostw, hipStream_t st) {
  hipLaunchKernelGGL(k_sc_beta, dim3(1), dim3(kBlock), 0, st, s, part_rr, part_obj, g, k,
                     obj_kind, tol, hostw);
}
void launch_sc_obj(CgState *s, const double *part, int g, int k, double tol, unsigned long long *hostw,
                   hipStream_t st) {
  hipLaunchKernelGGL(k_sc_obj, dim3(1), dim3(kBlock), 0, st, s, part, g, k, tol, hostw);
}
void launch_sc_beta_guarded(CgState *s, const double *part_rr, const double *part_obj, int g, int k, double tol,
                            unsigned long long *hostw, hipStream_t st) {
  hipLaunchKernelGGL(k_sc_beta_guarded, dim3(1), dim3(kBlock), 0, st, s, part_rr, part_obj, g, k, tol, hostw);
}
void launch_sc_obj_guarded(CgState *s, const double *part, int g, int k, double tol, unsigned long long *hostw,
                           hipStream_t st) {
  hipLaunchKernelGGL(k_sc_obj_guarded, dim3(1), dim3(kBlock), 0, st, s, part, g, k, tol, hostw);
}
void launch_sum_to(const double *part, int g, double *out, hipStream_t st) {
  hipLaunchKernelGGL(k_sum_to, dim3(1), dim3(kBlock), 0, st, part, g, out);
}

}
```

unires_amd/csrc/cg.hpp:

```cpp
#pragma once
#include "common.hpp"

namespace unires {

constexpr int kMaxCgIter = 4096;
constexpr int kMaxRing = 8;

struct CgState {
  double rz, pAp, alpha, beta, obj_max, obj_min;
  int done, iters;
  unsigned gen, pad_;
  double rzpp[2];
  double obj[kMaxCgIter + 1];
  int skip_fresh;
  int fresh_prev_ok;
  double rec_prev, fresh_prev, gain_rec;
  double ahist[kMaxRing];
  int committed[kMaxRing];
};
struct RingPtrs {
  const float *p[kMaxRing];
};

__host__ __device__ inline unsigned long long cg_progress_word(unsigned gen, int done, int iters) {
  return ((unsigned long long)gen << 32) | (done ? 0x80000000ull : 0ull) | (unsigned)(iters & 0x7fffffff);
}

int vec_num_blocks(size_t n);
void launch_residual_init(const float *b, const float *ax, const float *x, float *r, float *p,
                          size_t n, double *part_rr, double *part_obj, const float *M,
                          hipStream_t st);
void launch_dot(const float *a, const float *b, size_t n, double *part, const int *done,
                hipStream_t st);
void launch_update_xr(const CgState *s, const float *p, const float *ap, float *x, float *r,
                      const float *b, size_t n, double *part_rr, double *part_obj, const float *M,
                      hipStream_t st);
void launch_update_p(const CgState *s, const float *r, float *p, size_t n, const float *M, float *x,
                     hipStream_t st);
void launch_update_p_ring(CgState *s, const float *r, const float *p_in, float *p_out, int slot, size_t n,
                          const float *M, hipStream_t st);
void launch_update_p_flush(CgState *s, const float *r, const RingPtrs &ring, int m, float *p_out, size_t n,
                           const float *M, float *x, hipStream_t st);
void launch_update_x_flush(CgState *s, const RingPtrs &ring, int m, size_t n, float *x, hipStream_t st);
void launch_update_x(const CgState *s, const float *p, size_t n, float *x, hipStream_t st);
void launch_scale_shift(float a, float c, float *y, size_t n, hipStream_t st);
void launch_fill(float v, float *y, size_t n, hipStream_t st);
void launch_div(const float *a, const float *m, float *y, size_t n, hipStream_t st);
void launch_axpy(float a, const float *x, float *y, size_t n, hipStream_t st);
void launch_sc_init(CgState *s, const double *part_rr, const double *part_obj, int g, int mode,
                    int check, unsigned long long *hostw, hipStream_t st);
void launch_sc_alpha(CgState *s, const double *part, int g, hipStream_t st, int iters_end = 0);
void launch_sc_beta(CgState *s, const double *part_rr, const double *part_obj, int g, int k,
                    int obj_kind, double tol, unsigned long long *hostw, hipStream_t st);
void launch_sc_obj(CgState *s, const double *part, int g, int k, double tol, unsigned long long *hostw,
                   hipStream_t st);
void launch_sc_beta_guarded(CgState *s, const double *part_rr, const double *part_obj, int g, int k, double tol,
                            unsigned long long *hostw, hipStream_t st);
void launch_sc_obj_guarded(CgState *s, const double *part, int g, int k, double tol, unsigned long long *hostw,
                           hipStream_t st);
void launch_sum_to(const double *part, int g, double *out, hipStream_t st);

}
```

unires_amd/csrc/stencil.hip:

```cpp
#include <stdlib.h>

#include <algorithm>

#include "stencil.hpp"

namespace unires {

#ifndef UNIRES_FLAT_VECS
#define UNIRES_FLAT_VECS 1
#endif
constexpr int kFlatVecs = UNIRES_FLAT_VECS;
constexpr int kFlatChunk = kBlock * 4 * kFlatVecs;

struct FlatArgs {
  const float *p;
  float *q;
  const float *objb;
  double *partials;
  unsigned n, nz, ny, nynz;
  float inv_nz, inv_ny;
  unsigned head;
  unsigned nvec;
  unsigned nchunk;
  float a0, cx, cy, cz;
// ... 325 lines not shown
      FlatVec L;
      L.cc = cur.cc, L.xm = prev.cc, L.xp = next.cc, L.ym = cur.ym, L.yp = cur.yp, L.ob = cur.ob, L.edge = cur.edge;
      if (M.dbg & 2) {
        const f4 o = cur.cc + prev.cc + next.cc + cur.ym + cur.yp;
        if (valid) __builtin_amdgcn_raw_buffer_store_b128(__builtin_bit_cast(u4, o), rq, bo, 0, kAuxNt);
        bo += pstep;
        return;
      }
      if (y_inside && vx > 0u && vx + 1u < M.nx)
        flat_vec<false, DOT, OBJ>(A, L, lane, bo >> 2, k0, j0, valid, rq, dot);
      else
        flat_vec<true, DOT, OBJ>(A, L, lane, bo >> 2, k0, j0, valid, rq, dot);
      bo += pstep;
    };
    Plane P0, P1, P2, P3;
    P0.cc = f4{0.f, 0.f, 0.f, 0.f};
    if (xa > 0u) P0.cc = ld4_fast(rp, bo - pstep);
    P1.cc = ld4_fast(rp, bo);
    load_rest(bo, xa == 0u, P1);
    P2.cc = ld4_fast(rp, bo + pstep);
    for (unsigned vx = xa; vx < xb; vx += 4u) {
      step(P0, P1, P2, P3, vx);
      if (vx + 1u < xb) step(P1, P2, P3, P0, vx + 1u);
      if (vx + 2u < xb) step(P2, P3, P0, P1, vx + 2u);
      if (vx + 3u < xb) step(P3, P0, P1, P2, vx + 3u);
      else break;
    }
  }
  if (tail_wg) {
    const unsigned tl = nynz - 4u * M.nvp, ntail = M.nx * tl;
    const Dim3i dd{(int)M.nx, (int)A.ny, (int)nz};
    for (unsigned i = tid; i < ntail; i += kBlock) {
      const unsigned x = i / tl, idx = x * nynz + 4u * M.nvp + (i - x * tl);
      const unsigned line = idx / nz, k = idx - line * nz, j = line - x * A.ny;
      float pc;
      const float st = dtd_at(A.p, idx, (int)x, (int)j, (int)k, dd, A.cx, A.cy, A.cz, pc);
      matvec_emit(A.q, idx, A.a0 * pc + st, pc, OBJ ? A.objb : nullptr, DOT, dot);
    }
  }
  if (DOT || OBJ) {
    const double tot = block_sum(dot);
    if (tid == 0) A.partials[blockIdx.x] = tot;
  }
}

static bool flat_m_geometry(Dim3i dd, FlatMArgs &M) {
  static const int mode = getenv("UNIRES_FLAT_MARCH") ? atoi(getenv("UNIRES_FLAT_MARCH")) : 0;
  if (mode == 0) return false;
  const unsigned long long nynz = (unsigned long long)dd.y * dd.z;
  if (nynz < 4u * kWave || dd.x < 4 || nynz >= (1u << 24)) return false;
  M.nx = (unsigned)dd.x, M.nvp = (unsigned)(nynz / 4u), M.ncw = (M.nvp + kWave - 1u) / kWave;
  static const int tasks = getenv("UNIRES_FLAT_TASKS") ? atoi(getenv("UNIRES_FLAT_TASKS")) : 2048;
  unsigned long long xr = mode > 0 ? (unsigned long long)mode : ((unsigned long long)M.nx * M.ncw + tasks - 1) / tasks;
  xr = std::max<unsigned long long>(mode > 0 ? 2 : 4, std::min<unsigned long long>(xr, M.nx));
  if (mode <= 0 && xr < M.nx && (xr * nynz * 4u) % (1u << 20) == 0) ++xr;
  M.xr = (unsigned)xr, M.nxr = (M.nx + M.xr - 1u) / M.xr;
  return true;
}

static int flat_m_blocks(const FlatMArgs &M) {
  const unsigned long long nb = ((unsigned long long)M.ncw * M.nxr + (kBlock / kWave) - 1) / (kBlock / kWave);
  return (int)std::min<unsigned long long>(nb, 4096) + 1;
}

static int flat_grid(unsigned nchunk) {
  static const unsigned cap = getenv("UNIRES_FLAT_BLOCKS") ? (unsigned)atoi(getenv("UNIRES_FLAT_BLOCKS")) : 4096u;
  if (nchunk < 1) return 1;
  const unsigned per = (nchunk + cap - 1) / cap;
  return (int)((nchunk + per - 1) / per);
}

int dtd_flat_blocks(Dim3i dd, int which) {
  FlatMArgs M;
  if (!diff_nonforward(which) && flat_m_geometry(dd, M)) return flat_m_blocks(M);
  const size_t n = dd.numel();
  return flat_grid((unsigned)((n / 4 * 4 + kFlatChunk - 1) / kFlatChunk));
}

static bool flat_args(const float *p, float *q, Dim3i dd, float a0, float cx, float cy, float cz, double *partials,
                      const float *objb, FlatArgs &A) {
  const size_t n = dd.numel();
  if (dd.z < 4 || n >= (1ull << 29) || n < 64 || (objb && !partials)) return false;
  if ((size_t)dd.z + kFlatChunk >= (1u << 24) || (size_t)dd.y + kFlatChunk >= (1u << 24)) return false;
  A.p = p, A.q = q, A.objb = objb, A.partials = partials;
  A.n = (unsigned)n, A.nz = (unsigned)dd.z, A.ny = (unsigned)dd.y, A.nynz = (unsigned)dd.y * (unsigned)dd.z;
  A.inv_nz = 1.f / (float)dd.z, A.inv_ny = 1.f / (float)dd.y;
  A.head = (unsigned)(((16u - (unsigned)((uintptr_t)q & 15u)) & 15u) / 4u);
  A.nvec = (A.n - A.head) / 4u;
  A.nchunk = (A.nvec * 4u + kFlatChunk - 1u) / (unsigned)kFlatChunk;
  A.a0 = a0, A.cx = cx, A.cy = cy, A.cz = cz;
  return true;
}

static void flat_ranges(FlatArgs &A, unsigned G) {
  A.nx = G >= 8u ? 8u : 1u, A.per_xcd = G / A.nx, A.rem = G % A.nx;
  for (unsigned x = 0, before = 0; x <= A.nx; ++x) {
    A.cb[x] = (unsigned)((unsigned long long)A.nchunk * before / G);
    before += A.per_xcd + (x < A.rem ? 1u : 0u);
  }
}

template <class L>
static void by_epilogue(const double *partials, const float *objb, L &&launch) {
  if (objb)
    launch(std::true_type(), std::true_type());
  else if (partials)
    launch(std::true_type(), std::false_type());
  else
    launch(std::false_type(), std::false_type());
}

int launch_dtd_flat(int which, bool accumulate, const float *p, float *q, Dim3i dd, float a0, float cx, float cy,
                    float cz, double *partials, const float *objb, const int *done, hipStream_t st) {
  const bool fwd = !diff_nonforward(which);
  FlatArgs A;
  if (!flat_args(p, q, dd, a0, cx, cy, cz, partials, objb, A) || (fwd && accumulate)) return 1;
  const dim3 block(kBlock);
  FlatMArgs M;
  if (fwd && flat_m_geometry(dd, M)) {
    M.F = A;
    static const int fdbg = getenv("UNIRES_FLAT_DBG") ? atoi(getenv("UNIRES_FLAT_DBG")) : 0;
    M.dbg = fdbg;
    const dim3 grid(flat_m_blocks(M));
    by_epilogue(partials, objb, [&](auto DOT, auto OBJ) {
      hipLaunchKernelGGL((k_dtd_flat_m<DOT(), OBJ()>), grid, block, 0, st, M, done);
    });
    return 0;
  }
  const unsigned G = (unsigned)dtd_flat_blocks(dd, which);
  flat_ranges(A, G);
  const dim3 grid(G);
  if (fwd) {
    by_epilogue(partials, objb, [&](auto DOT, auto OBJ) {
      hipLaunchKernelGGL((k_dtd_flat<DOT(), OBJ()>), grid, block, 0, st, A, done);
    });
    return 0;
  }
  by_diff(which, [&](auto Wc) {
    constexpr int W = decltype(Wc)::value;
    if constexpr (W != kDiffForward) {
      if (accumulate)
        by_epilogue(partials, objb, [&](auto DOT, auto OBJ) {
          hipLaunchKernelGGL((k_dtd_flat_w<W, true, DOT(), OBJ()>), grid, block, 0, st, A, done);
        });
      else
        by_epilogue(partials, objb, [&](auto DOT, auto OBJ) {
          hipLaunchKernelGGL((k_dtd_flat_w<W, false, DOT(), OBJ()>), grid, block, 0, st, A, done);
        });
    }
  });
  return 0;
}

}
```

unires_amd/csrc/stencil.hpp:

```cpp
#pragma once
#include "common.hpp"

namespace unires {

int dtd_flat_blocks(Dim3i dd, int which);
int launch_dtd_flat(int which, bool accumulate, const float *p, float *q, Dim3i dd, float a0, float cx, float cy,
                    float cz, double *partials, const float *objb, const int *done, hipStream_t st);

void launch_grad(const float *src, Dim3i d, const float vx[3], float *dst3, hipStream_t st, int which = kDiffForward);
void launch_div(const float *ua, const float *ub, float ca, float cb, Dim3i d, const float vx[3],
                float scale, const float *add, float *dst, hipStream_t st, int which = kDiffForward);
int dtd_num_blocks(Dim3i d);
void launch_dtd(const float *src, Dim3i d, const float vx[3], float a, float c, float *dst,
                double *partials, const float *objb, const int *done, hipStream_t st, int which = kDiffForward,
                bool accumulate = false);

}
```

Measured before the change: 5263 cg_iters/s.

## Fuse RHS assembly into CG start with one-pass divergence-residual kernel

Adds a combined RHS+CG solve entry point (single and multi-stream) used when the tolerance is zero. The RHS divergence of w/z, the optional A^T x add, the initial residual b - Ax0, preconditioning and the r·z dot are computed in one vectorised stencil kernel inside the CG start. This removes separate RHS launches, the b buffer write/read and the per-channel Python round trips. In exchange it needs a new code path with alignment and dim%4 constraints, and it falls back to separate kernels otherwise.

```diff
diff --git a/include/unires_hip.h b/include/unires_hip.h
--- a/include/unires_hip.h
+++ b/include/unires_hip.h
@@ -109,6 +109,10 @@
                       float *dst3, void *stream);
 int unires_div_which(const float *src3, const int32_t dim[3], const float vx[3], int32_t which,
                      float *dst, void *stream);
+int unires_rhs_residual(const float *ua, const float *ub, float ca, float cb, const int32_t dim[3],
+                        const float vx[3], int32_t which, float scale, const float *add, int32_t add_after, const float *q,
+                        const float *m, float *r, float *p, float *b, double *partials, int32_t one_pass,
+                        int32_t *n_partials, void *stream);
 int unires_dtd_which(const float *src, const int32_t dim[3], const float vx[3], int32_t which, float a,
                      float c, float *dst, void *stream);
 
@@ -143,6 +147,10 @@
 int unires_plan_matvec_time(unires_plan_t *plan, int32_t *launches, double *total_us);
 int unires_plan_cg_ring(unires_plan_t *plan, int32_t k, int32_t *last);
 int unires_plan_cg_ends(unires_plan_t *plan, int32_t *trimmed, int32_t *start_fused);
+#define UNIRES_START_SEPARATE 0
+#define UNIRES_START_PUSH 1
+#define UNIRES_START_RHS 2
+int unires_plan_cg_start(unires_plan_t *plan, int32_t *start, int32_t *r0_once);
 
 int unires_proj_apply(unires_plan_t *plan, int32_t n, int32_t op, const float *in, float *out,
                       void *stream);
@@ -172,6 +180,17 @@
                          const float *const *b, float *const *x, int32_t max_iter, double tol,
                          int32_t stop_mode, int32_t precond_mode, int32_t *iters_out,
                          double *obj_trace, void *const *streams);
+
+int unires_plan_rhs_cg_solve(unires_plan_t *plan, const float *const *x_ptrs, const float *atx, const float *w_c,
+                             const float *z_c, float rho, float lam, float *b, float *x, int32_t max_iter, double tol,
+                             int32_t stop_mode, int32_t precond_mode, int32_t *iters_out, double *obj_trace,
+                             void *stream);
+int unires_plan_rhs_cg_solve_many(int32_t n, unires_plan_t *const *plans, const float *const *const *x_ptrs,
+                                  const float *const *atx,
+                                  const float *const *w_c, const float *const *z_c, const float *rho,
+                                  const float *lam, float *const *b, float *const *x, int32_t max_iter,
+                                  double tol, int32_t stop_mode, int32_t precond_mode, int32_t *iters_out,
+                                  double *obj_trace, void *const *streams);
 
 
 int unires_zw_update(const float *const *y_ptrs, const float *lam, int32_t n_channels,
diff --git a/unires_amd/_lib.py b/unires_amd/_lib.py
--- a/unires_amd/_lib.py
+++ b/unires_amd/_lib.py
@@ -56,6 +56,10 @@
     'unires_div_which': (C.c_int, [C.c_void_p, c_i32x3, c_f32x3, C.c_int32, C.c_void_p, C.c_void_p]),
     'unires_dtd_which': (C.c_int, [C.c_void_p, c_i32x3, c_f32x3, C.c_int32, C.c_float, C.c_float, C.c_void_p,
                                    C.c_void_p]),
+    'unires_rhs_residual': (C.c_int, [C.c_void_p, C.c_void_p, C.c_float, C.c_float, c_i32x3, c_f32x3, C.c_int32,
+                                      C.c_float, C.c_void_p, C.c_int32, C.c_void_p, C.c_void_p, C.c_void_p,
+                                      C.c_void_p, C.c_void_p, C.c_void_p, C.c_int32, C.POINTER(C.c_int32),
+                                      C.c_void_p]),
     'unires_plan_create': (C.c_int, [C.POINTER(C.c_void_p), c_i32x3, c_f32x3, C.c_int32,
                                      C.c_int32, C.POINTER(Repeat), C.c_float]),
     'unires_plan_destroy': (C.c_int, [C.c_void_p]),
@@ -90,6 +94,16 @@
                                        C.POINTER(C.c_float), C.POINTER(C.c_void_p), C.POINTER(C.c_void_p),
                                        C.c_int32, C.c_double, C.c_int32, C.c_int32, C.POINTER(C.c_int32),
                                        C.POINTER(C.c_double), C.POINTER(C.c_void_p)]),
+    'unires_plan_cg_start': (C.c_int, [C.c_void_p, C.POINTER(C.c_int32), C.POINTER(C.c_int32)]),
+    'unires_plan_rhs_cg_solve': (C.c_int, [C.c_void_p, C.POINTER(C.c_void_p), C.c_void_p, C.c_void_p, C.c_void_p,
+                                           C.c_float, C.c_float,
+                                           C.c_void_p, C.c_void_p, C.c_int32, C.c_double, C.c_int32, C.c_int32,
+                                           C.POINTER(C.c_int32), C.POINTER(C.c_double), C.c_void_p]),
+    'unires_plan_rhs_cg_solve_many': (C.c_int, [C.c_int32, C.POINTER(C.c_void_p), C.POINTER(C.POINTER(C.c_void_p)),
+                                                C.POINTER(C.c_void_p), C.POINTER(C.c_void_p), C.POINTER(C.c_void_p), C.POINTER(C.c_float),
+                                                C.POINTER(C.c_float), C.POINTER(C.c_void_p), C.POINTER(C.c_void_p),
+                                                C.c_int32, C.c_double, C.c_int32, C.c_int32, C.POINTER(C.c_int32),
+                                                C.POINTER(C.c_double), C.POINTER(C.c_void_p)]),
     'unires_zw_update': (C.c_int, [C.POINTER(C.c_void_p), C.POINTER(C.c_float), C.c_int32, c_i32x3,
                                    c_f32x3, C.c_float, C.c_float, C.c_void_p, C.c_void_p,
                                    C.c_void_p, C.c_void_p]),
diff --git a/unires_amd/_plan.py b/unires_amd/_plan.py
--- a/unires_amd/_plan.py
+++ b/unires_amd/_plan.py
@@ -257,6 +257,14 @@
 
     @on_device
     def rhs_cached(self, x_dats, w_c, z_c, rho, lam, out):
+        atx = self.atx_cached(x_dats)
+        w_c, z_c = w_c.contiguous(), z_c.contiguous()
+        check(self.lib.unires_rhs_from_atx(self._h, _ptr(atx), _ptr(w_c), _ptr(z_c),
+                                           float(rho), float(lam), _ptr(out), _stream()))
+        return out
+
+    @on_device
+    def atx_cached(self, x_dats):
         xs = [_vol(t, 'x')[0] for t in x_dats]
         import weakref
         copied = any(v is not t and v.data_ptr() != t.data_ptr() for v, t in zip(xs, x_dats))
@@ -271,10 +279,44 @@
             check(self.lib.unires_atx_assemble(self._h, ptrs, _ptr(atx), _stream()))
             refs = [] if key is None else [weakref.ref(t) for t in x_dats]
             self._atx = cache = (key, atx, refs)
-        w_c, z_c = w_c.contiguous(), z_c.contiguous()
-        check(self.lib.unires_rhs_from_atx(self._h, _ptr(cache[1]), _ptr(w_c), _ptr(z_c),
-                                           float(rho), float(lam), _ptr(out), _stream()))
-        return out
+        return cache[1]
+
+    @on_device
+    def _observations(self, x_dats):
+        xs = [_vol(t, 'x')[0] for t in x_dats]
+        if len(xs) != self.n_repeats:
+            raise ValueError('unires_amd: need one observation per repeat')
+        for t, dx in zip(xs, self.dims_x):
+            if tuple(t.shape) != tuple(dx):
+                raise ValueError('unires_amd: observation shape mismatch')
+        return xs, (C.c_void_p * len(xs))(*[t.data_ptr() for t in xs])
+
+    @on_device
+    def rhs_cg(self, x_dats, w_c, z_c, rho, lam, b, x, max_iter=20, tolerance=0.0, stop='max_gain', sync=False,
+               precond='none', cached=True):
+        if precond not in _lib.PRECOND:
+            raise ValueError('Undefined preconditioner')
+        atx = self.atx_cached(x_dats) if cached else None
+        xs, xp = (None, None) if cached else self._observations(x_dats)
+        w_c, z_c, b = _wz(self, w_c), _wz(self, z_c), self._y(b, 'b')
+        if not x.is_contiguous() or not b.is_contiguous():
+            raise ValueError('unires_amd: cg updates x in place and needs it and b contiguous')
+        self._y(x, 'x')
+        max_iter = int(max_iter)
+        it = C.c_int32(0) if sync else None
+        obj = (C.c_double * (min(max_iter, 4096) + 1))() if sync else None
+        check(self.lib.unires_plan_rhs_cg_solve(self._h, xp, _ptr(atx) if cached else None, _ptr(w_c), _ptr(z_c),
+                                                float(rho), float(lam),
+                                                _ptr(b), _ptr(x), max_iter, float(tolerance), _stop_mode(stop),
+                                                _lib.PRECOND[precond], C.byref(it) if sync else None, obj, _stream()))
+        if not sync:
+            return None
+        return it.value, (_trace(list(obj), it.value) if tolerance else None)
+
+    def cg_start(self):
+        s, o = C.c_int32(-1), C.c_int32(-1)
+        check(self.lib.unires_plan_cg_start(self._h, C.byref(s), C.byref(o)))
+        return int(s.value), bool(o.value)
 
     @on_device
     def precond_build(self, rho, lam, mode='jacobi', out=None):
@@ -319,6 +361,48 @@
                                        int(max_iter), float(tolerance), mode, pm, None, None,
                                        _stream()))
         return None
+
+
+def _stop_mode(stop):
+    s = stop if stop in _lib.STOP else stop[0].lower()
+    return _lib.STOP[s] if s in _lib.STOP else (0 if s == 'e' else 3)
+
+
+def _wz(plan, t):
+    if tuple(t.shape) != (3,) + plan.dim_y or not t.is_cuda or t.dtype != torch.float32:
+        raise ValueError('unires_amd: w/z must be (3,X,Y,Z) float32 device tensors')
+    return t.contiguous()
+
+
+def rhs_cg_many(plans, x_dats, ws, zs, bs, xs, rho, lams, streams, max_iter=20, tolerance=0.0, stop='max_gain',
+                precond='none', cached=True):
+    if precond not in _lib.PRECOND:
+        raise ValueError('Undefined preconditioner')
+    n = len(plans)
+    lib = plans[0].lib
+    atx, obs, keep = [], [], []
+    for c, pl in enumerate(plans):
+        if cached:
+            with torch.cuda.stream(streams[c]):
+                atx.append(pl.atx_cached(x_dats[c]))
+        else:
+            obs.append(pl._observations(x_dats[c]))
+        keep.append((_wz(pl, ws[c]), _wz(pl, zs[c])))
+        pl._y(bs[c], 'b')
+        pl._y(xs[c], 'x')
+        if not xs[c].is_contiguous() or not bs[c].is_contiguous():
+            raise ValueError('unires_amd: cg updates x in place and needs it and b contiguous')
+    vp = C.c_void_p * n
+    with torch.cuda.device(plans[0].device):
+        check(lib.unires_plan_rhs_cg_solve_many(
+            n, vp(*[pl._h.value for pl in plans]),
+            None if cached else (C.POINTER(C.c_void_p) * n)(*[C.cast(xp, C.POINTER(C.c_void_p)) for _, xp in obs]),
+            vp(*[t.data_ptr() for t in atx]) if cached else None,
+            vp(*[w.data_ptr() for w, _ in keep]), vp(*[z.data_ptr() for _, z in keep]),
+            (C.c_float * n)(*[float(rho)] * n), (C.c_float * n)(*[float(v) for v in lams]),
+            vp(*[b.data_ptr() for b in bs]), vp(*[x.data_ptr() for x in xs]), int(max_iter), float(tolerance),
+            _stop_mode(stop), _lib.PRECOND[precond], None, None, vp(*[st.cuda_stream for st in streams])))
+    return None
 
 
 def _trace(ring, it):
diff --git a/unires_amd/_update.py b/unires_amd/_update.py
--- a/unires_amd/_update.py
+++ b/unires_amd/_update.py
@@ -6,7 +6,7 @@
 from ._lib import check, f3, i3
 from ._ops import _ptr, _stream, on_device
 from ._host import Pacer
-from ._plan import cg_many
+from ._plan import cg_many, rhs_cg_many
 from ._project import _channel_plan, _proj, _slice_axis
 from .spatial import voxel_size
 
@@ -74,12 +74,20 @@
     C = len(x)
     concurrent = C > 1 and not sync and channel_streams_on(sett, y[0].dat)
     pre = getattr(sett, 'cgs_precond', 'none')
+    one_call = sett.cgs_tol == 0
+    cached = bool(getattr(sett, 'cache_atx', True))
     if not concurrent:
         for c in range(C):
             plan = _channel_plan(x[c], y[c], sett.method, sett.do_proj, vx_y, diff=_diff(sett),
                                  mask_zeros=_mask_zeros(sett), weights=True)
             plan.set_concurrency(1)
             lam = float(y[c].lam)
+            if one_call and not sync:
+                if pre in ('jacobi', 'fft'):
+                    plan.precond_build(rho, lam, mode=pre)
+                plan.rhs_cg([xn.dat for xn in x[c]], w[c], z[c], rho, lam, tmp, y[c].dat, max_iter=sett.cgs_max_iter,
+                            tolerance=sett.cgs_tol, stop=sett.cgs_stop, precond=pre, cached=cached)
+                continue
             if getattr(sett, 'cache_atx', True) and not sync:
                 plan.rhs_cached([xn.dat for xn in x[c]], w[c], z[c], rho, lam, out=tmp)
             else:
@@ -105,7 +113,10 @@
         b = tmp if c == 0 else plan.rhs_buffer(tmp)
         with torch.cuda.stream(streams[c]):
             streams[c].wait_event(ready)
-            if getattr(sett, 'cache_atx', True):
+            if one_call:
+                if cached:
+                    plan.atx_cached([xn.dat for xn in x[c]])
+            elif getattr(sett, 'cache_atx', True):
                 plan.rhs_cached([xn.dat for xn in x[c]], w[c], z[c], rho, lam, out=b)
             else:
                 plan.rhs([xn.dat for xn in x[c]], w[c], z[c], rho, lam, out=b)
@@ -113,8 +124,13 @@
                 plan.precond_build(rho, lam, mode=pre)
         plans.append(plan)
         bs.append(b)
-    cg_many(plans, bs, [yc.dat for yc in y], rho, [float(yc.lam) for yc in y], streams,
-            max_iter=sett.cgs_max_iter, tolerance=sett.cgs_tol, stop=sett.cgs_stop, precond=pre)
+    if one_call:
+        rhs_cg_many(plans, [[xn.dat for xn in xc] for xc in x], list(w), list(z), bs, [yc.dat for yc in y], rho,
+                    [float(yc.lam) for yc in y], streams, max_iter=sett.cgs_max_iter, tolerance=sett.cgs_tol,
+                    stop=sett.cgs_stop, precond=pre, cached=cached)
+    else:
+        cg_many(plans, bs, [yc.dat for yc in y], rho, [float(yc.lam) for yc in y], streams,
+                max_iter=sett.cgs_max_iter, tolerance=sett.cgs_tol, stop=sett.cgs_stop, precond=pre)
     for c in range(C):
         main.wait_stream(streams[c])
     return y
diff --git a/unires_amd/csrc/api.hip b/unires_amd/csrc/api.hip
--- a/unires_amd/csrc/api.hip
+++ b/unires_amd/csrc/api.hip
@@ -338,6 +338,32 @@
   return unires_dtd_which(src, dim, vx, UNIRES_DIFF_FORWARD, a, c, dst, stream);
 }
 
+extern "C" int unires_rhs_residual(const float *ua, const float *ub, float ca, float cb, const int32_t dim[3],
+                                   const float vx[3], int32_t which, float scale, const float *add, int32_t add_after,
+                                   const float *q,
+                                   const float *m, float *r, float *p, float *b, double *partials, int32_t one_pass,
+                                   int32_t *n_partials, void *stream) {
+  if (!ua || !dim || !q || !p || !partials) return fail(UNIRES_ERR_NULL, "null argument");
+  if (!dims_ok(dim)) return fail(UNIRES_ERR_DIM, "bad dimensions");
+  if (!vx_ok(vx)) return fail(UNIRES_ERR_ARG, "voxel size must be positive");
+  if (!diff_ok(which)) return fail(UNIRES_ERR_ARG, "which: forward (0), backward (1) or central (2)");
+  hipStream_t st = (hipStream_t)stream;
+  const Dim3i d = mk(dim);
+  const int g = vec_num_blocks(d.numel());
+  if (n_partials) *n_partials = g;
+  if (one_pass) {
+    if (launch_rhs_residual(which, ua, ub, ca, cb, d, vx, scale, add, add_after != 0, q, m, r, p, b, partials, g, st))
+      return fail(UNIRES_ERR_UNSUPPORTED, "the one-pass form needs dim[2] % 4 == 0 and 16-byte aligned pointers");
+  } else {
+    if (!r || !b) return fail(UNIRES_ERR_NULL, "the separate kernels store r and b");
+    launch_div(ua, ub, ca, cb, d, vx, scale, add_after ? nullptr : add, b, st, which);
+    if (add && add_after) launch_axpy(1.f, add, b, d.numel(), st);
+    launch_residual_init(b, q, nullptr, r, p, d.numel(), partials, nullptr, m, st);
+  }
+  CHECK_LAUNCH();
+  return UNIRES_OK;
+}
+
 static int check_channels(const float *const *y_ptrs, const float *lam, int32_t n) {
   if (!y_ptrs || !lam) return fail(UNIRES_ERR_NULL, "null argument");
   if (n < 1 || n > 4096) return fail(UNIRES_ERR_ARG, "channel count out of range");
diff --git a/unires_amd/csrc/api_cg.hip b/unires_amd/csrc/api_cg.hip
--- a/unires_amd/csrc/api_cg.hip
+++ b/unires_amd/csrc/api_cg.hip
@@ -3,6 +3,7 @@
 #include <functional>
 
 #include "api_internal.hpp"
+#include "stencil.hpp"
 
 using namespace unires;
 
@@ -17,11 +18,32 @@
   CgState *S = pl->state;
   const int gv = vec_num_blocks(ny);
   HIP_TRY(hipMemsetAsync(&S->done, 0, sizeof(int), st));
+  pl->last_r0_once = 0;
+  if (s.rhs_w) {
+    if (check || s.fft) return fail(UNIRES_ERR_ARG, "right-hand side inside the start outside its scope");
+    const bool once = !s.M;
+    const float *add = s.rhs_x ? s.rhs_b : s.rhs_add;
+    const bool flat = rhs_residual_serves(pl->dy, {s.rhs_w, s.rhs_z, add, pl->ap, s.M, pl->r, pl->p});
+    if (flat) {
+      pl->last_fused = 0;
+      if (s.rhs_x) rhs_data_term(pl, &s.rhs_x, s.rhs_b, false, st);
+      (void)matvec(pl, s.rho, s.lam, s.x, pl->ap, nullptr, nullptr, st);
+      if (launch_rhs_residual(pl->diff, s.rhs_w, s.rhs_z, 1.f, -s.rho, pl->dy, pl->vx, -s.lam, add, s.rhs_x != nullptr,
+                              pl->ap, s.M, once ? nullptr : pl->r, pl->p, nullptr, pl->part0, gv, st))
+        return fail(UNIRES_ERR_ARG, "right-hand side pass outside its domain");
+      pl->last_start = UNIRES_START_RHS, pl->last_r0_once = once ? 1 : 0;
+      launch_sc_init(S, pl->part0, pl->part1, gv, s.stop, 0, hostw, st);
+      return UNIRES_OK;
+    }
+    launch_div(s.rhs_w, s.rhs_z, 1.f, -s.rho, pl->dy, pl->vx, -s.lam, s.rhs_add, s.rhs_b, st, pl->diff);
+    if (s.rhs_x) rhs_data_term(pl, &s.rhs_x, s.rhs_b, true, st);
+  }
   const bool want_obj0 = check && s.stop != UNIRES_STOP_RESIDUAL;
   StartResidual res = {s.b, pl->r, pl->p, s.M, pl->part0, want_obj0 ? pl->part1 : nullptr, false};
   const bool ask = cg_start_fused_on() && !s.fft;
   int g0 = matvec(pl, s.rho, s.lam, s.x, pl->ap, nullptr, nullptr, st, nullptr, ask ? &res : nullptr);
   pl->last_fused = ask && res.served;
+  pl->last_start = pl->last_fused ? UNIRES_START_PUSH : UNIRES_START_SEPARATE;
   if (!(ask && res.served)) {
     launch_residual_init(s.b, pl->ap, s.x, pl->r, pl->p, ny, pl->part0, want_obj0 ? pl->part1 : nullptr, s.M, st);
     g0 = gv;
@@ -45,7 +67,7 @@
 }
 
 static int cg_enqueue_iters(unires_plan *pl, const CgSolve &s, int k_first, int count, bool dev_k,
-                            unsigned long long *hostw, hipStream_t st) {
+                            unsigned long long *hostw, hipStream_t st, bool r0_once = false) {
   const size_t ny = pl->dy.numel();
   const bool check = s.tol != 0.0;
   const int ring = s.ring;
@@ -56,6 +78,8 @@
     return fail(UNIRES_ERR_ARG, "deferred iterate update outside its scope");
   const bool trim = cg_trim_on() && !check && !s.fft && !dev_k && k_first == 1 && count == s.max_iter;
   pl->last_trim = trim && count > 0;
+  if (r0_once && (dev_k || k_first != 1 || s.M))
+    return fail(UNIRES_ERR_ARG, "residual stored once outside its scope");
   RingPtrs rp = {};
   for (int j = 0; j < ring && ring > 1; ++j) rp.p[j] = ring_slot(pl, j);
   for (int k = k_first; k < k_first + count; ++k) {
@@ -96,7 +120,8 @@
       break;
     }
     launch_sc_alpha(S, pl->part0, g, st);
-    launch_update_xr(S, p, pl->ap, lazy_x ? nullptr : s.x, pl->r, s.b, ny, pl->part0,
+    const float *r_in = r0_once && k == 1 ? pl->p : pl->r;
+    launch_update_xr(S, p, pl->ap, lazy_x ? nullptr : s.x, r_in, pl->r, s.b, ny, pl->part0,
                      recur ? pl->part1 : nullptr, s.M, st);
     if (s.fft) {
       if (fftpre_apply(pl->fft, pl->r, pl->fft.z, st)) return fail(UNIRES_ERR_HIP, "hipFFT execution failed");
@@ -127,7 +152,7 @@
 static int cg_enqueue(unires_plan *pl, const CgSolve &s, hipStream_t st) {
   const int rc = cg_enqueue_start(pl, s, nullptr, st);
   if (rc) return rc;
-  return cg_enqueue_iters(pl, s, 1, s.max_iter, false, nullptr, st);
+  return cg_enqueue_iters(pl, s, 1, s.max_iter, false, nullptr, st, pl->last_r0_once != 0);
 }
 
 static int cg_ring_prepare(unires_plan *pl, hipStream_t st) {
@@ -259,6 +284,7 @@
   pl->last_trim = 0;
   if (R.use_graph) {
     pl->last_fused = pl->chunk_fused;
+    pl->last_start = pl->chunk_fused ? UNIRES_START_PUSH : UNIRES_START_SEPARATE, pl->last_r0_once = 0;
     HIP_TRY(hipGraphLaunch(pl->cg_start_exec, R.st));
   } else {
     const int rc = cg_enqueue_start(pl, R.s, pl->progress_dev, R.st);
@@ -388,15 +414,29 @@
   return UNIRES_OK;
 }
 
-extern "C" int unires_cg_solve(unires_plan_t *plan, float rho, float lam, const float *b, float *x,
-                               int32_t max_iter, double tol, int32_t stop_mode,
-                               int32_t precond_mode, int32_t *iters_out, double *obj_trace,
-                               void *stream) {
+static bool cg_rhs_fused_on() {
+  static const bool on = !(getenv("UNIRES_CG_RHS_FUSED") && getenv("UNIRES_CG_RHS_FUSED")[0] == '0');
+  return on;
+}
+
+struct CgRhs {
+  const float *atx, *x, *w, *z;
+};
+
+static bool cg_rhs_in_start(const unires_plan *pl, bool from_x, int max_iter, double tol, int precond_mode) {
+  if (from_x && (pl->reps.size() != 1 || pl->regime == UNIRES_REGIME_IDENTITY)) return false;
+  return cg_rhs_fused_on() && tol == 0.0 && max_iter > 0 && precond_mode != UNIRES_PRECOND_FFT;
+}
+
+static int cg_solve(unires_plan_t *plan, float rho, float lam, const float *b, float *x, int32_t max_iter, double tol,
+                    int32_t stop_mode, int32_t precond_mode, int32_t *iters_out, double *obj_trace, void *stream,
+                    const CgRhs *rhs) {
   int rc = cg_check_args(plan, rho, lam, b, x, max_iter, tol, stop_mode, precond_mode);
   if (rc) return rc;
   hipStream_t st = (hipStream_t)stream;
   unires_plan *pl = plan;
   CgSolve s = cg_describe(pl, rho, lam, b, x, max_iter, tol, stop_mode, precond_mode);
+  if (rhs) s.rhs_w = rhs->w, s.rhs_z = rhs->z, s.rhs_add = rhs->atx, s.rhs_x = rhs->x, s.rhs_b = const_cast<float *>(b);
   mark_use(pl, st);
 
   if (stream_capturing(st) && tol != 0.0 && max_iter > kMaxCgIter)
@@ -418,6 +458,7 @@
   const bool graphable = cg_graphs_on() && !s.fft && max_iter > 0 && !pl->timing;
   if (graphable && pl->cg_exec && pl->cg_key.same_graph(s)) {
     pl->last_trim = pl->graph_trim, pl->last_fused = pl->graph_fused;
+    pl->last_start = pl->graph_start, pl->last_r0_once = pl->graph_r0_once;
     HIP_TRY(hipGraphLaunch(pl->cg_exec, st));
   } else {
     if (graphable && pl->cg_exec) drop_cg_graph(pl);
@@ -429,6 +470,7 @@
     if (rc == 0) {
       pl->cg_key = s;
       pl->graph_trim = pl->last_trim, pl->graph_fused = pl->last_fused;
+      pl->graph_start = pl->last_start, pl->graph_r0_once = pl->last_r0_once;
       if (hipGraphLaunch(pl->cg_exec, st) != hipSuccess) {
         cg_resync_gen(pl);
         return fail(UNIRES_ERR_HIP, "hipGraphLaunch failed");
@@ -441,6 +483,32 @@
   mark_use(pl, st);
   CHECK_LAUNCH();
   return iters_out ? cg_read_back(pl, max_iter, tol, iters_out, obj_trace, st) : UNIRES_OK;
+}
+
+extern "C" int unires_cg_solve(unires_plan_t *plan, float rho, float lam, const float *b, float *x,
+                               int32_t max_iter, double tol, int32_t stop_mode,
+                               int32_t precond_mode, int32_t *iters_out, double *obj_trace,
+                               void *stream) {
+  return cg_solve(plan, rho, lam, b, x, max_iter, tol, stop_mode, precond_mode, iters_out, obj_trace, stream, nullptr);
+}
+
+extern "C" int unires_plan_rhs_cg_solve(unires_plan_t *plan, const float *const *x_ptrs, const float *atx,
+                                        const float *w_c, const float *z_c, float rho, float lam, float *b, float *x,
+                                        int32_t max_iter, double tol, int32_t stop_mode, int32_t precond_mode,
+                                        int32_t *iters_out, double *obj_trace, void *stream) {
+  if (!plan || !w_c || !z_c || !b || !x) return fail(UNIRES_ERR_NULL, "null argument");
+  if (!atx == !x_ptrs) return fail(UNIRES_ERR_ARG, "give the kept data term or the observations, not both");
+  if (x_ptrs)
+    for (size_t n = 0; n < plan->reps.size(); ++n)
+      if (!x_ptrs[n]) return fail(UNIRES_ERR_NULL, "null observation pointer");
+  if (cg_rhs_in_start(plan, x_ptrs != nullptr, max_iter, tol, precond_mode)) {
+    const CgRhs rhs = {atx, x_ptrs ? x_ptrs[0] : nullptr, w_c, z_c};
+    return cg_solve(plan, rho, lam, b, x, max_iter, tol, stop_mode, precond_mode, iters_out, obj_trace, stream, &rhs);
+  }
+  const int rc = x_ptrs ? unires_rhs_assemble(plan, x_ptrs, w_c, z_c, rho, lam, b, stream)
+                        : unires_rhs_from_atx(plan, atx, w_c, z_c, rho, lam, b, stream);
+  if (rc) return rc;
+  return unires_cg_solve(plan, rho, lam, b, x, max_iter, tol, stop_mode, precond_mode, iters_out, obj_trace, stream);
 }
 
 extern "C" int unires_cg_solve_many(int32_t n, unires_plan_t *const *plans, const float *rho, const float *lam,
@@ -490,3 +558,43 @@
     }
   return UNIRES_OK;
 }
+
+extern "C" int unires_plan_rhs_cg_solve_many(int32_t n, unires_plan_t *const *plans,
+                                             const float *const *const *x_ptrs, const float *const *atx,
+                                             const float *const *w_c, const float *const *z_c, const float *rho,
+                                             const float *lam, float *const *b, float *const *x, int32_t max_iter,
+                                             double tol, int32_t stop_mode, int32_t precond_mode, int32_t *iters_out,
+                                             double *obj_trace, void *const *streams) {
+  if (n < 1 || !plans || !w_c || !z_c || !rho || !lam || !b || !x || !streams)
+    return fail(UNIRES_ERR_NULL, "null argument");
+  if (!atx == !x_ptrs) return fail(UNIRES_ERR_ARG, "give the kept data terms or the observations, not both");
+  bool in_start = true;
+  for (int c = 0; c < n; ++c) {
+    if (!plans[c] || !(atx ? (const void *)atx[c] : (const void *)x_ptrs[c]) || !w_c[c] || !z_c[c] || !b[c] || !x[c])
+      return fail(UNIRES_ERR_NULL, "null argument");
+    for (int d = 0; d < c; ++d)
+      if (plans[d] == plans[c]) return fail(UNIRES_ERR_ARG, "one plan per solve");
+    in_start = in_start && cg_rhs_in_start(plans[c], x_ptrs != nullptr, max_iter, tol, precond_mode);
+  }
+  if (!in_start && (tol != 0.0 || max_iter <= 0)) {
+    for (int c = 0; c < n; ++c) {
+      const int rc = x_ptrs ? unires_rhs_assemble(plans[c], x_ptrs[c], w_c[c], z_c[c], rho[c], lam[c], b[c], streams[c])
+                            : unires_rhs_from_atx(plans[c], atx[c], w_c[c], z_c[c], rho[c], lam[c], b[c], streams[c]);
+      if (rc) return rc;
+    }
+    return unires_cg_solve_many(n, plans, rho, lam, b, x, max_iter, tol, stop_mode, precond_mode, iters_out, obj_trace,
+                                streams);
+  }
+  for (int c = 0; c < n; ++c) {
+    const int rc = unires_plan_rhs_cg_solve(plans[c], x_ptrs ? x_ptrs[c] : nullptr, atx ? atx[c] : nullptr, w_c[c],
+                                            z_c[c], rho[c], lam[c], b[c], x[c], max_iter, tol, stop_mode, precond_mode,
+                                            nullptr, nullptr, streams[c]);
+    if (rc) return rc;
+  }
+  if (iters_out)
+    for (int c = 0; c < n; ++c) {
+      const int rc = cg_read_back(plans[c], max_iter, tol, iters_out + c, nullptr, (hipStream_t)streams[c]);
+      if (rc) return rc;
+    }
+  return UNIRES_OK;
+}
diff --git a/unires_amd/csrc/api_internal.hpp b/unires_amd/csrc/api_internal.hpp
--- a/unires_amd/csrc/api_internal.hpp
+++ b/unires_amd/csrc/api_internal.hpp
@@ -141,9 +141,12 @@
   int chunk = 0;
   const float *M = nullptr;
   bool fft = false;
+  const float *rhs_w = nullptr, *rhs_z = nullptr, *rhs_add = nullptr, *rhs_x = nullptr;
+  float *rhs_b = nullptr;
   bool same_graph(const CgSolve &o) const {
     return b == o.b && x == o.x && rho == o.rho && lam == o.lam && max_iter == o.max_iter && stop == o.stop &&
-           pre == o.pre && ring == o.ring && chunk == o.chunk && tol == o.tol;
+           pre == o.pre && ring == o.ring && chunk == o.chunk && tol == o.tol && rhs_w == o.rhs_w && rhs_z == o.rhs_z &&
+           rhs_add == o.rhs_add && rhs_x == o.rhs_x;
   }
 };
 
@@ -182,6 +185,7 @@
   int ring_req = 0;
   int last_ring = 1;
   int last_trim = 0, last_fused = 0, graph_trim = 0, graph_fused = 0, chunk_fused = 0;
+  int last_start = 0, last_r0_once = 0, graph_start = 0, graph_r0_once = 0;
   unires::FftPre fft;
   float prec_rho = 0.f, prec_lam = 0.f;
   int prec_mode = UNIRES_PRECOND_IDENTITY;
@@ -211,5 +215,6 @@
 };
 int matvec(unires_plan *pl, float rho, float lam, const float *p, float *q, double *part, const int *done,
            hipStream_t st, const float *objb = nullptr, StartResidual *res = nullptr);
-
-}
+void rhs_data_term(unires_plan *pl, const float *const *x_ptrs, float *out, bool accumulate, hipStream_t st);
+
+}
diff --git a/unires_amd/csrc/api_operator.hip b/unires_amd/csrc/api_operator.hip
--- a/unires_amd/csrc/api_operator.hip
+++ b/unires_amd/csrc/api_operator.hip
@@ -395,6 +395,11 @@
   return UNIRES_OK;
 }
 
+void unires::rhs_data_term(unires_plan *pl, const float *const *x_ptrs, float *out, bool accumulate, hipStream_t st) {
+  for (size_t n = 0; n < pl->reps.size(); ++n)
+    at_accumulate(pl, pl->reps[n], x_ptrs[n], out, pl->reps[n].tau, accumulate || n > 0, st, true);
+}
+
 extern "C" int unires_rhs_assemble(unires_plan_t *plan, const float *const *x_ptrs,
                                    const float *w_c, const float *z_c, float rho, float lam,
                                    float *b, void *stream) {
@@ -404,8 +409,7 @@
   hipStream_t st = (hipStream_t)stream;
   mark_use(plan, st);
   launch_div(w_c, z_c, 1.f, -rho, plan->dy, plan->vx, -lam, nullptr, b, st, plan->diff);
-  for (size_t n = 0; n < plan->reps.size(); ++n)
-    at_accumulate(plan, plan->reps[n], x_ptrs[n], b, plan->reps[n].tau, true, st, true);
+  rhs_data_term(plan, x_ptrs, b, true, st);
   CHECK_LAUNCH();
   return UNIRES_OK;
 }
diff --git a/unires_amd/csrc/api_plan.hip b/unires_amd/csrc/api_plan.hip
--- a/unires_amd/csrc/api_plan.hip
+++ b/unires_amd/csrc/api_plan.hip
@@ -474,6 +474,13 @@
   if (!plan) return fail(UNIRES_ERR_NULL, "null argument");
   if (trimmed) *trimmed = plan->last_trim;
   if (start_fused) *start_fused = plan->last_fused;
+  return UNIRES_OK;
+}
+
+extern "C" int unires_plan_cg_start(unires_plan_t *plan, int32_t *start, int32_t *r0_once) {
+  if (!plan) return fail(UNIRES_ERR_NULL, "null argument");
+  if (start) *start = plan->last_start;
+  if (r0_once) *r0_once = plan->last_r0_once;
   return UNIRES_OK;
 }
 
diff --git a/unires_amd/csrc/cg.hip b/unires_amd/csrc/cg.hip
--- a/unires_amd/csrc/cg.hip
+++ b/unires_amd/csrc/cg.hip
@@ -108,7 +108,7 @@
 template <bool XUPD>
 __global__ void __launch_bounds__(kBlock)
     k_update_xr(const CgState *__restrict__ st, const float *__restrict__ p,
-                const float *__restrict__ ap, float *__restrict__ x, float *__restrict__ r,
+                const float *__restrict__ ap, float *__restrict__ x, const float *r_in, float *r_out,
                 const float *__restrict__ b, size_t n, double *__restrict__ part_rr,
                 double *__restrict__ part_obj, const float *__restrict__ M) {
   if (st->done) return;
@@ -117,7 +117,7 @@
   double rr = 0.0, ob = 0.0;
   for (size_t i = tid0; i < n4; i += stride) {
     const float4 va = ld4(ap, i);
-    float4 vx = make_float4(0.f, 0.f, 0.f, 0.f), vr = ld4(r, i);
+    float4 vx = make_float4(0.f, 0.f, 0.f, 0.f), vr = ld4(r_in, i);
     if (XUPD) {
       const float4 vp = ld4(p, i);
       vx = ld4(x, i);
@@ -131,7 +131,7 @@
     vr.y = __fsub_rn(vr.y, __fmul_rn(alpha, va.y));
     vr.z = __fsub_rn(vr.z, __fmul_rn(alpha, va.z));
     vr.w = __fsub_rn(vr.w, __fmul_rn(alpha, va.w));
-    st4(r, i, vr);
+    st4(r_out, i, vr);
     const float4 vz = zval4(vr, M, i);
     rr += (double)__fmul_rn(vr.x, vz.x) + (double)__fmul_rn(vr.y, vz.y) +
           (double)__fmul_rn(vr.z, vz.z) + (double)__fmul_rn(vr.w, vz.w);
@@ -149,8 +149,8 @@
       vx = __fadd_rn(x[i], __fmul_rn(alpha, p[i]));
       x[i] = vx;
     }
-    const float vr = __fsub_rn(r[i], __fmul_rn(alpha, ap[i]));
-    r[i] = vr;
+    const float vr = __fsub_rn(r_in[i], __fmul_rn(alpha, ap[i]));
+    r_out[i] = vr;
     rr += (double)__fmul_rn(vr, zval1(vr, M, i));
     if (XUPD && part_obj) ob += (double)__fmul_rn(vx, __fadd_rn(b[i], vr));
   }
@@ -501,14 +501,14 @@
                 hipStream_t st) {
   hipLaunchKernelGGL(k_dot, dim3(vec_blocks(n)), dim3(kBlock), 0, st, a, b, n, part, done);
 }
-void launch_update_xr(const CgState *s, const float *p, const float *ap, float *x, float *r,
+void launch_update_xr(const CgState *s, const float *p, const float *ap, float *x, const float *r_in, float *r_out,
                       const float *b, size_t n, double *part_rr, double *part_obj,
                       const float *M, hipStream_t st) {
   if (x)
-    hipLaunchKernelGGL(k_update_xr<true>, dim3(vec_blocks(n)), dim3(kBlock), 0, st, s, p, ap, x, r, b,
+    hipLaunchKernelGGL(k_update_xr<true>, dim3(vec_blocks(n)), dim3(kBlock), 0, st, s, p, ap, x, r_in, r_out, b,
                        n, part_rr, part_obj, M);
   else
-    hipLaunchKernelGGL(k_update_xr<false>, dim3(vec_blocks(n)), dim3(kBlock), 0, st, s, p, ap, x, r,
+    hipLaunchKernelGGL(k_update_xr<false>, dim3(vec_blocks(n)), dim3(kBlock), 0, st, s, p, ap, x, r_in, r_out,
                        b, n, part_rr, part_obj, M);
 }
 void launch_update_p(const CgState *s, const float *r, float *p, size_t n, const float *M, float *x,
diff --git a/unires_amd/csrc/cg.hpp b/unires_amd/csrc/cg.hpp
--- a/unires_amd/csrc/cg.hpp
+++ b/unires_amd/csrc/cg.hpp
@@ -32,7 +32,7 @@
                           hipStream_t st);
 void launch_dot(const float *a, const float *b, size_t n, double *part, const int *done,
                 hipStream_t st);
-void launch_update_xr(const CgState *s, const float *p, const float *ap, float *x, float *r,
+void launch_update_xr(const CgState *s, const float *p, const float *ap, float *x, const float *r_in, float *r_out,
                       const float *b, size_t n, double *part_rr, double *part_obj, const float *M,
                       hipStream_t st);
 void launch_update_p(const CgState *s, const float *r, float *p, size_t n, const float *M, float *x,
diff --git a/unires_amd/csrc/stencil.hip b/unires_amd/csrc/stencil.hip
--- a/unires_amd/csrc/stencil.hip
+++ b/unires_amd/csrc/stencil.hip
@@ -501,4 +501,122 @@
   return 0;
 }
 
-}
+struct RhsArgs {
+  const float *ua, *ub;
+  float ca, cb, sx, sy, sz, scale;
+  const float *add, *q, *M;
+  float *r, *p, *b;
+  double *partials;
+  unsigned n4, nz4, ny, nx;
+};
+
+template <bool UB>
+__device__ __forceinline__ float rhs_comb(const RhsArgs &A, float a, float b) {
+#pragma clang fp contract(off)
+  const float u = A.ca * a;
+  return UB ? fmaf(A.cb, b, u) : u;
+}
+template <bool UB>
+__device__ __forceinline__ void rhs_comb4(const RhsArgs &A, f4 a, f4 b, float u[4]) {
+  u[0] = rhs_comb<UB>(A, a.x, b.x), u[1] = rhs_comb<UB>(A, a.y, b.y);
+  u[2] = rhs_comb<UB>(A, a.z, b.z), u[3] = rhs_comb<UB>(A, a.w, b.w);
+}
+
+template <int W, bool UB, int ADD, bool JAC>
+__global__ void __launch_bounds__(kBlock) k_rhs_residual(RhsArgs A) {
+#pragma clang fp contract(off)
+  constexpr bool kLo = W != kDiffBackward, kHi = W != kDiffForward;
+  const size_t n4 = A.n4;
+  const size_t stride = (size_t)gridDim.x * blockDim.x;
+  const size_t sxv = (size_t)A.ny * A.nz4, syv = A.nz4;
+  const f4 *ax = reinterpret_cast<const f4 *>(A.ua), *ay = ax + n4, *az = ay + n4;
+  const f4 *bx = reinterpret_cast<const f4 *>(UB ? A.ub : A.ua), *by = bx + n4, *bz = by + n4;
+  const float *az1 = reinterpret_cast<const float *>(az), *bz1 = reinterpret_cast<const float *>(bz);
+  const unsigned nz = 4u * A.nz4;
+  const f4 zero = f4{0.f, 0.f, 0.f, 0.f};
+  double rr = 0.0;
+  for (size_t i = (size_t)blockIdx.x * blockDim.x + threadIdx.x; i < n4; i += stride) {
+    const unsigned v = (unsigned)i, line = v / A.nz4, k0 = 4u * (v - line * A.nz4);
+    const unsigned x = line / A.ny, j = line - x * A.ny;
+    const bool lx = x > 0u, hx = x + 1u < A.nx, ly = j > 0u, hy = j + 1u < A.ny;
+    const size_t ixl = kLo && lx ? i - sxv : i, ixh = kHi && hx ? i + sxv : i;
+    const size_t iyl = kLo && ly ? i - syv : i, iyh = kHi && hy ? i + syv : i;
+    const size_t izb = k0 > 0u ? 4 * i - 1 : 4 * i, iza = k0 + 4u < nz ? 4 * i + 4 : 4 * i;
+    const f4 axl = ax[ixl], axh = ax[ixh], ayl = ay[iyl], ayh = ay[iyh], azc = az[i];
+    const f4 bxl = UB ? bx[ixl] : zero, bxh = UB ? bx[ixh] : zero, byl = UB ? by[iyl] : zero, byh = UB ? by[iyh] : zero;
+    const f4 bzc = UB ? bz[i] : zero;
+    const float azb = kLo ? az1[izb] : 0.f, aza = kHi ? az1[iza] : 0.f;
+    const float bzb = kLo && UB ? bz1[izb] : 0.f, bza = kHi && UB ? bz1[iza] : 0.f;
+    const f4 vq = reinterpret_cast<const f4 *>(A.q)[i];
+    const f4 va = ADD != 0 ? reinterpret_cast<const f4 *>(A.add)[i] : zero;
+    const f4 vm = JAC ? reinterpret_cast<const f4 *>(A.M)[i] : zero;
+    float xl4[4], xh4[4], yl4[4], yh4[4], zs[6];
+    rhs_comb4<UB>(A, axl, bxl, xl4), rhs_comb4<UB>(A, axh, bxh, xh4);
+    rhs_comb4<UB>(A, ayl, byl, yl4), rhs_comb4<UB>(A, ayh, byh, yh4);
+    rhs_comb4<UB>(A, azc, bzc, zs + 1);
+    zs[0] = rhs_comb<UB>(A, azb, bzb), zs[5] = rhs_comb<UB>(A, aza, bza);
+    const bool xl_ok = !kLo || lx, xh_ok = !kHi || hx, yl_ok = !kLo || ly, yh_ok = !kHi || hy;
+    const float q4[4] = {vq.x, vq.y, vq.z, vq.w}, a4[4] = {va.x, va.y, va.z, va.w}, m4[4] = {vm.x, vm.y, vm.z, vm.w};
+    float b4[4], r4[4], z4[4];
+#pragma unroll
+    for (int e = 0; e < 4; ++e) {
+      const unsigned k = k0 + (unsigned)e;
+      const bool zl_ok = !kLo || k > 0u, zh_ok = !kHi || k + 1u < nz;
+      const float zl = kLo ? zs[e] : zs[e + 1], zh = kHi ? zs[e + 2] : zs[e + 1];
+      const float dx = (xl_ok ? xl4[e] : 0.f) - (xh_ok ? xh4[e] : 0.f);
+      const float dy = (yl_ok ? yl4[e] : 0.f) - (yh_ok ? yh4[e] : 0.f);
+      const float dz = (zl_ok ? zl : 0.f) - (zh_ok ? zh : 0.f);
+      float t = A.sy * dy;
+      t = fmaf(A.sx, dx, t);
+      t = fmaf(A.sz, dz, t);
+      b4[e] = ADD == 2 ? a4[e] + fmaf(A.scale, t, 0.f) : fmaf(A.scale, t, a4[e]);
+      r4[e] = b4[e] - q4[e];
+      z4[e] = JAC ? r4[e] / m4[e] : r4[e];
+    }
+    if (A.b) reinterpret_cast<f4 *>(A.b)[i] = f4{b4[0], b4[1], b4[2], b4[3]};
+    if (A.r) reinterpret_cast<f4 *>(A.r)[i] = f4{r4[0], r4[1], r4[2], r4[3]};
+    reinterpret_cast<f4 *>(A.p)[i] = f4{z4[0], z4[1], z4[2], z4[3]};
+    rr += (double)(r4[0] * z4[0]) + (double)(r4[1] * z4[1]) + (double)(r4[2] * z4[2]) + (double)(r4[3] * z4[3]);
+  }
+  const double tot = block_sum(rr);
+  if (threadIdx.x == 0) A.partials[blockIdx.x] = tot;
+}
+
+bool rhs_residual_serves(Dim3i d, std::initializer_list<const void *> ptrs) {
+  const size_t n = d.numel();
+  if (d.z % 4 != 0 || n >= (1ull << 31) || n == 0) return false;
+  for (const void *ptr : ptrs)
+    if ((uintptr_t)ptr & 15u) return false;
+  return true;
+}
+
+int launch_rhs_residual(int which, const float *ua, const float *ub, float ca, float cb, Dim3i d, const float vx[3],
+                        float scale, const float *add, bool add_after, const float *q, const float *M, float *r,
+                        float *p, float *b, double *partials, int blocks, hipStream_t st) {
+  const size_t n = d.numel();
+  if (!rhs_residual_serves(d, {ua, ub, add, q, M, r, p, b})) return 1;
+  const float h = diff_grad_scale(which);
+  RhsArgs A;
+  A.ua = ua, A.ub = ub, A.ca = ca, A.cb = cb;
+  A.sx = (1.f / vx[0]) * h, A.sy = (1.f / vx[1]) * h, A.sz = (1.f / vx[2]) * h, A.scale = scale;
+  A.add = add, A.q = q, A.M = M, A.r = r, A.p = p, A.b = b, A.partials = partials;
+  A.n4 = (unsigned)(n / 4), A.nz4 = (unsigned)(d.z / 4), A.ny = (unsigned)d.y, A.nx = (unsigned)d.x;
+  const auto flag = [](bool v, auto &&f) { v ? f(std::true_type()) : f(std::false_type()); };
+  const auto add_mode = [&](auto &&f) {
+    if (!add) f(std::integral_constant<int, 0>());
+    else if (!add_after) f(std::integral_constant<int, 1>());
+    else f(std::integral_constant<int, 2>());
+  };
+  by_diff(which, [&](auto W) {
+    flag(ub != nullptr, [&](auto UB) {
+      add_mode([&](auto ADD) {
+        flag(M != nullptr, [&](auto JAC) {
+          hipLaunchKernelGGL((k_rhs_residual<W(), UB(), ADD(), JAC()>), dim3(blocks), dim3(kBlock), 0, st, A);
+        });
+      });
+    });
+  });
+  return 0;
+}
+
+}
diff --git a/unires_amd/csrc/stencil.hpp b/unires_amd/csrc/stencil.hpp
--- a/unires_amd/csrc/stencil.hpp
+++ b/unires_amd/csrc/stencil.hpp
@@ -1,4 +1,6 @@
 #pragma once
+#include <initializer_list>
+
 #include "common.hpp"
 
 namespace unires {
@@ -10,6 +12,10 @@
 void launch_grad(const float *src, Dim3i d, const float vx[3], float *dst3, hipStream_t st, int which = kDiffForward);
 void launch_div(const float *ua, const float *ub, float ca, float cb, Dim3i d, const float vx[3],
                 float scale, const float *add, float *dst, hipStream_t st, int which = kDiffForward);
+bool rhs_residual_serves(Dim3i d, std::initializer_list<const void *> ptrs);
+int launch_rhs_residual(int which, const float *ua, const float *ub, float ca, float cb, Dim3i d, const float vx[3],
+                        float scale, const float *add, bool add_after, const float *q, const float *M, float *r,
+                        float *p, float *b, double *partials, int blocks, hipStream_t st);
 int dtd_num_blocks(Dim3i d);
 void launch_dtd(const float *src, Dim3i d, const float vx[3], float a, float c, float *dst,
                 double *partials, const float *objb, const int *done, hipStream_t st, int which = kDiffForward,
```

Result: no change. 5292 cg_iters/s, median of 3 (+0.5%).
